# ctu-vras/monoforce

Measured on AMD Instinct MI355X. Metric: rollout-steps/sec (batch x horizon) on 256x256 terrain, higher is better.
Workload: dtype f32; 1 GPU; c3: B=1024/GPU x T=500 x N=4 contact points, 256x256 grid (res 0.05 m), one shared terrain+friction map (the same on every rank), integrator=odeint-euler (reference default), forward+backward; BASE...; rollouts_per_gpu=1024, rollouts_total=1024, horizon=500, contact_points=4, parallelism=rollout-sharded x1

## Files before the change

include/monoforce_hip.h:

```cpp
#ifndef MONOFORCE_HIP_H
#define MONOFORCE_HIP_H

#include <stddef.h>
#include <stdint.h>

#ifdef __cplusplus
extern "C" {
#endif

enum {
  MF_OK = 0,
  MF_ERR_INVALID = 1,
  MF_ERR_UNSUPPORTED = 2,
  MF_ERR_LAUNCH = 3
};

enum {
  MF_INTEG_DYNAMICS = 0,
  MF_INTEG_ODEINT_EULER = 1
};

enum {
  MF_LAYOUT_BATCH_MAJOR = 0,
  MF_LAYOUT_TIME_MAJOR = 1
};

enum {
  MF_MATH_EXACT = 0,
  MF_MATH_FAST = 1
};

enum { MF_LANES_COMPONENT = 16 };

typedef struct MfRolloutDesc {
  int32_t B;
  int32_t T;
  int32_t N;
  int32_t H, W;
  int32_t n_tracks;
  int32_t integrator;
  int32_t layout;
  int32_t map_shared;
  int32_t block;
  int32_t skip_snap;
  int32_t points_per_lane;
  int32_t math_mode;
  int32_t force_stride;
  int32_t grad_copies;
  int32_t has_joints;
  int32_t pose_stride;
  int32_t cost_project;
  int32_t default_state;
  int32_t controls_stride_b, controls_stride_t;
  double mass, gravity, stiffness, damping, omega_max;
  double grid_res, d_max;
  double dt;
  double robot_size_y;
  double Iinv[9];
  double joint_xyz[12];
} MfRolloutDesc;

#define MF_LOSS_VALUE_IN_BACKWARD 1
typedef struct MfRolloutLoss {
  int32_t T2;
  int32_t flags;
  const void* gt;
  const int32_t* near;
  const void* w;
  const int32_t* row_stamp;
  const void* row_w;
  void* partial;
  uint32_t* ticket;
  void* loss;
  const void* gloss;
  const void* Xs;
} MfRolloutLoss;

typedef struct MfRolloutFwdBufs {
  const void* z;
  const void* mu;
  const void* controls;
  const void* ts;
  const void* points;
  const int32_t* part;
  void* x0;
  const void* xd0;
  const void* R0;
  const void* w0;
  void* Xs;
  void* Xds;
  void* Rs;
  void* Omegas;
  void* Fs;
  void* Ff;
  void* Xraw;
  const void* joint_angles;
  void* cost_rows;
  void* path_cost;
  void* zmu_scratch;
  const void* zmu;
  void* rec;
  const MfRolloutLoss* loss;
} MfRolloutFwdBufs;

int mf_rollout_loss_fusable(const MfRolloutDesc* desc);

int mf_rollout_bwd_window(const MfRolloutDesc* desc);

long long mf_rollout_record_bytes(const MfRolloutDesc* desc);
int mf_rollout_fwd_stages_zmu(const MfRolloutDesc* desc);
long long mf_rollout_record_bytes_f64(const MfRolloutDesc* desc);

int mf_rollout_force_stride(const MfRolloutDesc* desc);
int mf_rollout_fwd_f32(const MfRolloutDesc* desc, const MfRolloutFwdBufs* bufs, void* hip_stream);
int mf_rollout_fwd_f64(const MfRolloutDesc* desc, const MfRolloutFwdBufs* bufs, void* hip_stream);

int mf_rollout_default_state_f32(int32_t B, int32_t T, const float* controls, float* x0, float* xd0, float* R0, float* w0, void* hip_stream);
int mf_rollout_default_state_f64(int32_t B, int32_t T, const double* controls, double* x0, double* xd0, double* R0, double* w0, void* hip_stream);

typedef struct MfRolloutBwdBufs {
  const void* z;
  const void* mu;
  const void* controls;
  const void* ts;
  const void* points;
  const int32_t* part;
  const void* x_init;
  const void* xd0;
  const void* R0;
  const void* w0;
  const void* Xraw;
  const void* Xds;
  const void* Rs;
  const void* Omegas;
  const void* gXs;
  const void* gXds;
  const void* gRs;
  const void* gOmegas;
  const void* gFs;
  const void* gFf;
  const void* zeros;
  void* gz;
  void* gmu;
  void* gcontrols;
  void* gx0;
  void* gxd0;
  void* gR0;
  void* gw0;
  const void* joint_angles;
  void* gjoint_angles;
  const void* rec;
  const MfRolloutLoss* loss;
  void* zmu_scratch;
  const void* zmu;
} MfRolloutBwdBufs;

int mf_rollout_bwd_wants_gcontrols(const MfRolloutDesc* desc);
int mf_rollout_bwd_f32(const MfRolloutDesc* desc, const MfRolloutBwdBufs* bufs, void* hip_stream);
int mf_rollout_bwd_f64(const MfRolloutDesc* desc, const MfRolloutBwdBufs* bufs, void* hip_stream);

typedef struct MfSplatDesc {
  int32_t B;
  int32_t n_per_sample;
  int32_t C;
  int32_t nx, ny, nz;
  float off[3];
  float dx[3];
  int32_t lift_D;
  int32_t lift_hw;
} MfSplatDesc;

size_t mf_bev_splat_workspace_bytes(const MfSplatDesc* desc);
int mf_bev_splat_prepare(const MfSplatDesc* desc, const float* geom , void* workspace, void* hip_stream);
int mf_bev_splat_prepare_cameras(const MfSplatDesc* desc, const float* frustum, int32_t pts_per_cam, const float* cams,
                                 void* workspace, void* hip_stream);
int mf_bev_splat_prepare_rig(const MfSplatDesc* desc, const float* frustum, int32_t pts_per_cam, const float* rots, const float* trans,
                             const float* intrins, const float* post_rots, const float* post_trans, void* workspace, void* hip_stream);
int mf_bev_splat_fwd_f32(const MfSplatDesc* desc, const float* x, const void* workspace, float* out, void* hip_stream);
int mf_bev_splat_fwd_f64(const MfSplatDesc* desc, const double* x, const void* workspace, double* out, void* hip_stream);
int mf_bev_splat_bwd_f32(const MfSplatDesc* desc, const float* gout, const void* workspace, float* gx, void* hip_stream);
int mf_bev_splat_bwd_f64(const MfSplatDesc* desc, const double* gout, const void* workspace, double* gx, void* hip_stream);

int mf_bev_lift_splat_fwd_f32(const MfSplatDesc* desc, const float* depth, const float* ctx, const void* workspace, float* out, void* hip_stream);
int mf_bev_lift_splat_fwd_f64(const MfSplatDesc* desc, const double* depth, const double* ctx, const void* workspace, double* out, void* hip_stream);
int mf_bev_lift_splat_bwd_f32(const MfSplatDesc* desc, const float* depth, const float* ctx, const void* workspace, const float* gout,
                              float* rows_scratch, float* g_depth, float* g_ctx, void* hip_stream);
int mf_bev_lift_splat_bwd_f64(const MfSplatDesc* desc, const double* depth, const double* ctx, const void* workspace, const double* gout,
                              double* rows_scratch, double* g_depth, double* g_ctx, void* hip_stream);

typedef struct MfLossDesc {
  int32_t B, T1, T2;
  int32_t reserved;
  int64_t x_stride_b, x_stride_t;
  double gamma;
} MfLossDesc;
int mf_physics_loss_fwd_f32(const MfLossDesc* desc, const float* Xs, const float* Xgt, const float* gt_ts, const int32_t* nearest, float* partial, void* hip_stream);
int mf_physics_loss_fwd_f64(const MfLossDesc* desc, const double* Xs, const double* Xgt, const double* gt_ts, const int32_t* nearest, double* partial, void* hip_stream);
int mf_physics_loss_bwd_f32(const MfLossDesc* desc, const float* Xs, const float* Xgt, const float* gt_ts, const int32_t* nearest, const float* gloss, float* gXs, void* hip_stream);
int mf_physics_loss_bwd_f64(const MfLossDesc* desc, const double* Xs, const double* Xgt, const double* gt_ts, const int32_t* nearest, const double* gloss, double* gXs, void* hip_stream);
int mf_nearest_steps_f32(int32_t B, int32_t T1, int32_t T2, const float* pred_ts, long long pred_stride_b, const float* gt_ts, long long gt_stride_b, int32_t* nearest, void* hip_stream);
int mf_nearest_steps_f64(int32_t B, int32_t T1, int32_t T2, const double* pred_ts, long long pred_stride_b, const double* gt_ts, long long gt_stride_b, int32_t* nearest, void* hip_stream);
int mf_physics_loss_value_f32(const MfLossDesc* desc, const float* Xs, const float* Xgt, const float* gt_ts, const int32_t* nearest, float* partial, uint32_t* ticket, float* loss, float* zero_fill, long long zero_count, void* hip_stream);
int mf_physics_loss_value_f64(const MfLossDesc* desc, const double* Xs, const double* Xgt, const double* gt_ts, const int32_t* nearest, double* partial, uint32_t* ticket, double* loss, double* zero_fill, long long zero_count, void* hip_stream);
int mf_reduce_grad_copies_f32(float* pool, int n_maps, int copies, long long n, float* out, void* hip_stream);
int mf_reduce_grad_copies_f64(double* pool, int n_maps, int copies, long long n, double* out, void* hip_stream);

typedef struct MfStageDesc {
  int32_t B, H, W, k;
} MfStageDesc;
int mf_terrain_stage_fwd_f32(const MfStageDesc* desc, const float* geom, const float* diff, const float* friction, float* terrain,
                             float* z, float* mu, float* zmu, void* hip_stream);
int mf_terrain_stage_bwd_f32(const MfStageDesc* desc, const float* g_terrain, const float* gz, const float* gmu, float* g_geom,
                             float* g_diff, float* g_friction, void* hip_stream);

typedef struct MfHeightmapDesc {
  int32_t n_points, nx, ny;
  float d_max, h_min, h_max;
  float r_min;
  float inv_res;
} MfHeightmapDesc;
int mf_estimate_heightmap_f32(const MfHeightmapDesc* desc, const float* points, const float* x_bins, const float* y_bins,
                              int32_t* scratch, float* hm, void* hip_stream);

typedef struct MfInterpDesc {
  int32_t B, N, H, W;
  int32_t map_shared;
  int32_t math_mode;
  double grid_res, d_max;
} MfInterpDesc;
int mf_interpolate_grid_f32(const MfInterpDesc* desc, const float* grid, const float* xq, const float* yq, float* z_out, float* n_out,
                            int32_t* cells_out, float* frac_out, void* hip_stream);
int mf_interpolate_grid_f64(const MfInterpDesc* desc, const double* grid, const double* xq, const double* yq, double* z_out, double* n_out,
                            int32_t* cells_out, double* frac_out, void* hip_stream);

typedef struct MfMppiDesc {
  int32_t B, T;
  int32_t keep_nominal, reserved;
  int64_t row_stride_b, row_stride_t;
  int64_t x_stride_b;
  float sigma[2], lo[2], hi[2];
  float w_incl, w_force, w_goal, lambda;
} MfMppiDesc;
int mf_mppi_perturb_f32(const MfMppiDesc* desc, const float* nominal , const float* noise ,
                        float* controls , void* hip_stream);
int mf_path_costs_f32(const MfMppiDesc* desc, const float* cost_rows, const float* force_cost, const float* x_last, const float* goal,
                      float* costs, float* terms, void* hip_stream);
long long mf_mppi_scratch_bytes(const MfMppiDesc* desc);
int mf_mppi_update_f32(const MfMppiDesc* desc, const float* costs, const float* controls, const float* nominal_in, float* weights,
                       float* nominal_out, int32_t* best, int32_t* n_valid, void* scratch, long long scratch_bytes, void* hip_stream);

const char* mf_last_error(void);
const char* mf_last_launch(void);
const char* mf_version(void);
int mf_sizeof(const char* struct_name);

#ifdef __cplusplus
}
#endif
#endif
```

monoforce_amd/_lib.py:

```python
import ctypes as C
import os
import threading

_HERE = os.path.dirname(os.path.abspath(__file__))
LIB_PATH = os.path.join(_HERE, 'csrc', 'libmonoforce_hip.so')

MF_INTEG_DYNAMICS, MF_INTEG_ODEINT_EULER = 0, 1
MF_LAYOUT_BATCH_MAJOR, MF_LAYOUT_TIME_MAJOR = 0, 1
MF_LOSS_VALUE_IN_BACKWARD = 1
MF_MATH_EXACT, MF_MATH_FAST = 0, 1
MF_LANES_COMPONENT = 16


class MfRolloutDesc(C.Structure):
    _fields_ = [('B', C.c_int32), ('T', C.c_int32), ('N', C.c_int32), ('H', C.c_int32), ('W', C.c_int32),
                ('n_tracks', C.c_int32), ('integrator', C.c_int32), ('layout', C.c_int32), ('map_shared', C.c_int32),
                ('block', C.c_int32), ('skip_snap', C.c_int32), ('points_per_lane', C.c_int32), ('math_mode', C.c_int32), ('force_stride', C.c_int32), ('grad_copies', C.c_int32), ('has_joints', C.c_int32), ('pose_stride', C.c_int32), ('cost_project', C.c_int32), ('default_state', C.c_int32), ('controls_stride_b', C.c_int32), ('controls_stride_t', C.c_int32),
                ('mass', C.c_double), ('gravity', C.c_double), ('stiffness', C.c_double), ('damping', C.c_double),
                ('omega_max', C.c_double), ('grid_res', C.c_double), ('d_max', C.c_double), ('dt', C.c_double),
                ('robot_size_y', C.c_double), ('Iinv', C.c_double * 9), ('joint_xyz', C.c_double * 12)]


class MfRolloutLoss(C.Structure):
    _fields_ = [('T2', C.c_int32), ('flags', C.c_int32)] + [(n, C.c_void_p) for n in ('gt', 'near', 'w', 'row_stamp', 'row_w', 'partial', 'ticket', 'loss', 'gloss', 'Xs')]


class MfRolloutFwdBufs(C.Structure):
    _fields_ = [(n, C.c_void_p) for n in ('z', 'mu', 'controls', 'ts', 'points', 'part', 'x0', 'xd0', 'R0', 'w0',
                                          'Xs', 'Xds', 'Rs', 'Omegas', 'Fs', 'Ff', 'Xraw', 'joint_angles', 'cost_rows', 'path_cost',
                                          'zmu_scratch', 'zmu', 'rec', 'loss')]


class MfRolloutBwdBufs(C.Structure):
    _fields_ = [(n, C.c_void_p) for n in ('z', 'mu', 'controls', 'ts', 'points', 'part', 'x_init', 'xd0', 'R0', 'w0',
                                          'Xraw', 'Xds', 'Rs', 'Omegas',
                                          'gXs', 'gXds', 'gRs', 'gOmegas', 'gFs', 'gFf', 'zeros',
                                          'gz', 'gmu', 'gcontrols', 'gx0', 'gxd0', 'gR0', 'gw0', 'joint_angles', 'gjoint_angles', 'rec', 'loss',
                                          'zmu_scratch', 'zmu')]


class MfLossDesc(C.Structure):
    _fields_ = [('B', C.c_int32), ('T1', C.c_int32), ('T2', C.c_int32), ('reserved', C.c_int32),
                ('x_stride_b', C.c_int64), ('x_stride_t', C.c_int64), ('gamma', C.c_double)]


class MfSplatDesc(C.Structure):
    _fields_ = [('B', C.c_int32), ('n_per_sample', C.c_int32), ('C', C.c_int32),
                ('nx', C.c_int32), ('ny', C.c_int32), ('nz', C.c_int32),
                ('off', C.c_float * 3), ('dx', C.c_float * 3), ('lift_D', C.c_int32), ('lift_hw', C.c_int32)]


class MfStageDesc(C.Structure):
    _fields_ = [('B', C.c_int32), ('H', C.c_int32), ('W', C.c_int32), ('k', C.c_int32)]


class MfInterpDesc(C.Structure):
    _fields_ = [('B', C.c_int32), ('N', C.c_int32), ('H', C.c_int32), ('W', C.c_int32), ('map_shared', C.c_int32), ('math_mode', C.c_int32),
                ('grid_res', C.c_double), ('d_max', C.c_double)]


class MfHeightmapDesc(C.Structure):
    _fields_ = [('n_points', C.c_int32), ('nx', C.c_int32), ('ny', C.c_int32), ('d_max', C.c_float), ('h_min', C.c_float),
                ('h_max', C.c_float), ('r_min', C.c_float), ('inv_res', C.c_float)]


class MfMppiDesc(C.Structure):
    _fields_ = [('B', C.c_int32), ('T', C.c_int32), ('keep_nominal', C.c_int32), ('reserved', C.c_int32),
                ('row_stride_b', C.c_int64), ('row_stride_t', C.c_int64), ('x_stride_b', C.c_int64),
                ('sigma', C.c_float * 2), ('lo', C.c_float * 2), ('hi', C.c_float * 2),
                ('w_incl', C.c_float), ('w_force', C.c_float), ('w_goal', C.c_float), ('lam', C.c_float)]


SYMBOLS = ['mf_rollout_force_stride', 'mf_rollout_fwd_f32', 'mf_rollout_fwd_f64', 'mf_rollout_default_state_f32', 'mf_rollout_default_state_f64', 'mf_rollout_bwd_f32', 'mf_rollout_bwd_f64', 'mf_rollout_bwd_wants_gcontrols', 'mf_rollout_record_bytes', 'mf_rollout_record_bytes_f64', 'mf_rollout_fwd_stages_zmu', 'mf_rollout_loss_fusable', 'mf_rollout_bwd_window', 'mf_bev_splat_workspace_bytes', 'mf_bev_splat_prepare', 'mf_bev_splat_prepare_cameras', 'mf_bev_splat_prepare_rig',
           'mf_bev_splat_fwd_f32', 'mf_bev_splat_fwd_f64', 'mf_bev_splat_bwd_f32', 'mf_bev_splat_bwd_f64',
           'mf_bev_lift_splat_fwd_f32', 'mf_bev_lift_splat_fwd_f64', 'mf_bev_lift_splat_bwd_f32', 'mf_bev_lift_splat_bwd_f64',
           'mf_physics_loss_fwd_f32', 'mf_physics_loss_fwd_f64', 'mf_physics_loss_bwd_f32', 'mf_physics_loss_bwd_f64', 'mf_physics_loss_value_f32', 'mf_physics_loss_value_f64', 'mf_nearest_steps_f32', 'mf_nearest_steps_f64', 'mf_reduce_grad_copies_f32', 'mf_reduce_grad_copies_f64', 'mf_estimate_heightmap_f32', 'mf_interpolate_grid_f32', 'mf_interpolate_grid_f64', 'mf_terrain_stage_fwd_f32', 'mf_terrain_stage_bwd_f32', 'mf_mppi_perturb_f32', 'mf_path_costs_f32', 'mf_mppi_scratch_bytes', 'mf_mppi_update_f32', 'mf_last_error', 'mf_last_launch', 'mf_version', 'mf_sizeof']

_lib = None
_lock = threading.Lock()


def lib():
    global _lib
    if _lib is None:
        with _lock:
            if _lib is None:
                if not os.path.exists(LIB_PATH):
                    raise RuntimeError(
                        f'{LIB_PATH} is missing: build the HIP extension first (make -C monoforce_amd/csrc). '
                        'monoforce_amd has no CPU fallback.')
                import torch
                L = C.CDLL(os.environ.get('MONOFORCE_HIP_LIB', LIB_PATH))
                L.mf_last_error.restype = C.c_char_p
                L.mf_version.restype = C.c_char_p
                L.mf_last_launch.restype = C.c_char_p
                for name in SYMBOLS:
                    fn = getattr(L, name)
                    if name.startswith(('mf_rollout', 'mf_bev', 'mf_physics', 'mf_estimate', 'mf_terrain', 'mf_reduce', 'mf_interpolate', 'mf_nearest', 'mf_mppi', 'mf_path')):
                        fn.restype = C.c_int
                L.mf_bev_splat_workspace_bytes.restype = C.c_size_t
                L.mf_rollout_record_bytes.restype = C.c_longlong
                L.mf_rollout_record_bytes_f64.restype = C.c_longlong
                L.mf_mppi_scratch_bytes.restype = C.c_longlong
                _lib = L
    return _lib


ON_ERROR = []


def check(rc, what):
    if rc != 0:
        for fn in list(ON_ERROR):
            fn()
        raise RuntimeError(f'{what} failed (code {rc}): {lib().mf_last_error().decode()}')


def ptr(t):
    return None if t is None else C.c_void_p(t.data_ptr())


def require_hip_tensor(t, name):
    if not t.is_cuda:
        raise RuntimeError(f'{name} is on {t.device}: monoforce_amd computes on the MI355X HIP path only '
                           '(no CPU fallback); move inputs to "cuda".')
```

monoforce_amd/csrc/physics_loss.hip:

```cpp
#include "mf_common.h"

namespace mf {

__device__ __forceinline__ void atomic_add_s(float* p, float v) { unsafeAtomicAdd(p, v); }
__device__ __forceinline__ void atomic_add_s(double* p, double v) { unsafeAtomicAdd(p, v); }

template <typename S>
__global__ void __launch_bounds__(256) physics_loss_fwd_kernel(const S* __restrict__ Xs, long long sb, long long st,
                                                              const S* __restrict__ Xgt, const S* __restrict__ gt_ts,
                                                              const int* __restrict__ nearest, int B, int T2, S gamma,
                                                              S* __restrict__ partial) {
  __shared__ S wave_sum[4];
  const int i = blockIdx.x * blockDim.x + threadIdx.x;
  S acc = (S)0;
  if (i < B * T2) {
    const int b = i / T2;
    const S w = (S)1 / ((S)1 + gamma * gt_ts[i]);
    const S* x = Xs + b * sb + (long long)nearest[i] * st;
    const S* g = Xgt + (size_t)i * 3;
#pragma unroll
    for (int c = 0; c < 3; ++c) { const S d = x[c] * w - g[c] * w; acc += d * d; }
  }
#pragma unroll
  for (int d = 32; d >= 1; d >>= 1) acc += __shfl_xor(acc, d, 64);
  if ((threadIdx.x & 63) == 0) wave_sum[threadIdx.x >> 6] = acc;
  __syncthreads();
  if (threadIdx.x == 0) partial[blockIdx.x] = (wave_sum[0] + wave_sum[1]) + (wave_sum[2] + wave_sum[3]);
}

template <typename S>
__global__ void __launch_bounds__(256) physics_loss_value_kernel(const S* __restrict__ Xs, long long sb, long long st,
                                                                const S* __restrict__ Xgt, const S* __restrict__ gt_ts,
                                                                const int* __restrict__ nearest, int B, int T2, S gamma,
                                                                S* __restrict__ partial, unsigned* __restrict__ ticket, S inv_count,
                                                                S* __restrict__ loss, S* __restrict__ zero_fill, long long zero_count) {
  __shared__ S wave_sum[4];
  __shared__ bool last;
  const int i = blockIdx.x * blockDim.x + threadIdx.x;
  {
    const long long head = min(zero_count, (long long)(((16u - (unsigned)((uintptr_t)zero_fill & 15u)) & 15u) / sizeof(S)));
    const long long n16 = (zero_count - head) * (long long)sizeof(S) / 16, tail0 = head + n16 * (16 / (long long)sizeof(S));
    int4* z16 = reinterpret_cast<int4*>(zero_fill + head);
    for (long long k = i; k < n16; k += (long long)gridDim.x * blockDim.x) z16[k] = make_int4(0, 0, 0, 0);
    if (i < head) zero_fill[i] = (S)0;
    if (tail0 + i < zero_count) zero_fill[tail0 + i] = (S)0;
  }
  S acc = (S)0;
  if (i < B * T2) {
    const int k = i, b = i / T2;
    const S w = (S)1 / ((S)1 + gamma * gt_ts[k]);
    const S* x = Xs + b * sb + (long long)nearest[k] * st;
    const S* g = Xgt + (size_t)k * 3;
#pragma unroll
    for (int c = 0; c < 3; ++c) { const S d = x[c] * w - g[c] * w; acc += d * d; }
  }
#pragma unroll
  for (int d = 32; d >= 1; d >>= 1) acc += __shfl_xor(acc, d, 64);
  if ((threadIdx.x & 63) == 0) wave_sum[threadIdx.x >> 6] = acc;
  __syncthreads();
  if (threadIdx.x == 0) {
    partial[blockIdx.x] = (wave_sum[0] + wave_sum[1]) + (wave_sum[2] + wave_sum[3]);
    __threadfence();
    last = atomicAdd(ticket, 1u) == gridDim.x - 1;
  }
  __syncthreads();
  if (!last) return;
  __threadfence();
  S tot = (S)0;
  for (unsigned k = threadIdx.x; k < gridDim.x; k += 256) tot += __builtin_nontemporal_load(partial + k);
#pragma unroll
  for (int d = 32; d >= 1; d >>= 1) tot += __shfl_xor(tot, d, 64);
  if ((threadIdx.x & 63) == 0) wave_sum[threadIdx.x >> 6] = tot;
  __syncthreads();
  if (threadIdx.x == 0) {
    loss[0] = ((wave_sum[0] + wave_sum[1]) + (wave_sum[2] + wave_sum[3])) * inv_count;
    *ticket = 0u;
  }
}

template <typename S>
__global__ void __launch_bounds__(256) reduce_grad_copies_kernel(S* __restrict__ pool, int copies, long long n, S* __restrict__ out) {
  const long long i = (long long)blockIdx.x * blockDim.x + threadIdx.x;
  if (i >= n) return;
  S* p = pool + (long long)blockIdx.y * copies * n + i;
  S acc = (S)0;
  for (int c = 0; c < copies; ++c) { acc += p[(long long)c * n]; p[(long long)c * n] = (S)0; }
  out[(long long)blockIdx.y * n + i] = acc;
}

template <typename S>
__global__ void __launch_bounds__(256) physics_loss_bwd_kernel(const S* __restrict__ Xs, long long sb, long long st,
                                                              const S* __restrict__ Xgt, const S* __restrict__ gt_ts,
                                                              const int* __restrict__ nearest, int B, int T2, S gamma,
                                                              const S* __restrict__ gloss, S inv_count, S* __restrict__ gXs) {
  const int t = blockIdx.x * blockDim.x + threadIdx.x;
  if (t >= B * T2) return;
  const bool jm = sb < st;
  const int b = jm ? t % B : t / T2, j = jm ? t / B : t % T2;
  const int i = b * T2 + j;
  const S scale = (S)2 * gloss[0] * inv_count;
  const S w = (S)1 / ((S)1 + gamma * gt_ts[i]);
  const int nr = nearest[i];
  const long long o = b * sb + (long long)nr * st;
  const S* g = Xgt + (size_t)i * 3;
  bool shared = false;
  for (int k = 0; k < T2; ++k) shared |= (k != j) & (nearest[b * T2 + k] == nr);
#pragma unroll
  for (int c = 0; c < 3; ++c) {
    const S v = scale * w * (Xs[o + c] * w - g[c] * w);
    if (shared) atomic_add_s(gXs + o + c, v); else gXs[o + c] = v;
  }
}

template <typename S>
static int loss_fwd(const MfLossDesc* d, const S* Xs, const S* Xgt, const S* gt_ts, const int* nearest, S* partial, hipStream_t st) {
  MF_REQUIRE(d && Xs && Xgt && gt_ts && nearest && partial, MF_ERR_INVALID, "physics_loss_fwd: null argument");
  MF_REQUIRE(d->B > 0 && d->T1 > 0 && d->T2 > 0, MF_ERR_INVALID, "physics_loss_fwd: B, T1, T2 must be positive");
  hipLaunchKernelGGL((physics_loss_fwd_kernel<S>), dim3((d->B * d->T2 + 255) / 256), dim3(256), 0, st, Xs, (long long)d->x_stride_b,
                     (long long)d->x_stride_t, Xgt, gt_ts, nearest, d->B, d->T2, (S)d->gamma, partial);
  hipError_t e = hipGetLastError();
  MF_REQUIRE(e == hipSuccess, MF_ERR_LAUNCH, std::string("physics_loss_fwd launch: ") + hipGetErrorString(e));
  return MF_OK;
}

template <typename S>
static int loss_value(const MfLossDesc* d, const S* Xs, const S* Xgt, const S* gt_ts, const int* nearest, S* partial, unsigned* ticket,
                      S* loss, S* zero_fill, long long zero_count, hipStream_t st) {
  MF_REQUIRE(d && Xs && Xgt && gt_ts && nearest && partial && ticket && loss, MF_ERR_INVALID, "physics_loss_value: null argument");
  MF_REQUIRE(d->B > 0 && d->T1 > 0 && d->T2 > 0, MF_ERR_INVALID, "physics_loss_value: B, T1, T2 must be positive");
  MF_REQUIRE(zero_count >= 0 && (zero_fill || zero_count == 0), MF_ERR_INVALID, "physics_loss_value: zero_count without zero_fill");
  const double count = (double)d->B * d->T2 * 3;
  hipLaunchKernelGGL((physics_loss_value_kernel<S>), dim3((d->B * d->T2 + 255) / 256), dim3(256), 0, st, Xs, (long long)d->x_stride_b,
                     (long long)d->x_stride_t, Xgt, gt_ts, nearest, d->B, d->T2, (S)d->gamma, partial, ticket, (S)(1.0 / count), loss, zero_fill, zero_count);
  hipError_t e = hipGetLastError();
  MF_REQUIRE(e == hipSuccess, MF_ERR_LAUNCH, std::string("physics_loss_value launch: ") + hipGetErrorString(e));
  return MF_OK;
}

template <typename S>
static int reduce_copies(S* pool, int n_maps, int copies, long long n, S* out, hipStream_t st) {
  MF_REQUIRE(pool && out, MF_ERR_INVALID, "reduce_grad_copies: null argument");
  MF_REQUIRE(n_maps > 0 && n_maps < 65536 && copies > 0 && n > 0, MF_ERR_INVALID, "reduce_grad_copies: n_maps, copies, n must be positive");
  hipLaunchKernelGGL((reduce_grad_copies_kernel<S>), dim3((unsigned)((n + 255) / 256), (unsigned)n_maps), dim3(256), 0, st, pool, copies, n, out);
  hipError_t e = hipGetLastError();
  MF_REQUIRE(e == hipSuccess, MF_ERR_LAUNCH, std::string("reduce_grad_copies launch: ") + hipGetErrorString(e));
  return MF_OK;
}

template <typename S>
static int loss_bwd(const MfLossDesc* d, const S* Xs, const S* Xgt, const S* gt_ts, const int* nearest, const S* gloss, S* gXs,
                    hipStream_t st) {
  MF_REQUIRE(d && Xs && Xgt && gt_ts && nearest && gloss && gXs, MF_ERR_INVALID, "physics_loss_bwd: null argument");
  MF_REQUIRE(d->B > 0 && d->T1 > 0 && d->T2 > 0, MF_ERR_INVALID, "physics_loss_bwd: B, T1, T2 must be positive");
  const double count = (double)d->B * d->T2 * 3;
  hipLaunchKernelGGL((physics_loss_bwd_kernel<S>), dim3((d->B * d->T2 + 255) / 256), dim3(256), 0, st, Xs, (long long)d->x_stride_b,
                     (long long)d->x_stride_t, Xgt, gt_ts, nearest, d->B, d->T2, (S)d->gamma, gloss, (S)(1.0 / count), gXs);
  hipError_t e = hipGetLastError();
  MF_REQUIRE(e == hipSuccess, MF_ERR_LAUNCH, std::string("physics_loss_bwd launch: ") + hipGetErrorString(e));
  return MF_OK;
}

}

namespace mf {
template <typename S>
__global__ void __launch_bounds__(256) nearest_steps_kernel(const S* __restrict__ pred_ts, long long pred_sb, const S* __restrict__ gt_ts, long long gt_sb,
                                                           int B, int T1, int T2, int* __restrict__ out) {
  const int i = blockIdx.x * blockDim.x + threadIdx.x;
  if (i >= B * T2) return;
  const int b = i / T2, j = i - b * T2;
  const S g = gt_ts[b * gt_sb + j];
  const S* p = pred_ts + b * pred_sb;
  S best = (S)INFINITY;
  int arg = 0;
  bool any = false;
  int t = 0;
  for (; t + 8 <= T1; t += 8) {
    S v[8];
#pragma unroll
    for (int k = 0; k < 8; ++k) v[k] = p[t + k];
#pragma unroll
    for (int k = 0; k < 8; ++k) {
      const S d = fabs(v[k] - g);
      if (d < best || (!any && d == d)) { best = d; arg = t + k; any = true; }
    }
  }
  for (; t < T1; ++t) {
    const S d = fabs(p[t] - g);
    if (d < best || (!any && d == d)) { best = d; arg = t; any = true; }
  }
  out[i] = arg;
}
template <typename S>
static int nearest_steps(int B, int T1, int T2, const S* pred_ts, long long pred_sb, const S* gt_ts, long long gt_sb, int32_t* out, hipStream_t st) {
  MF_REQUIRE(B > 0 && T1 > 0 && T2 > 0 && pred_ts && gt_ts && out && pred_sb >= 0 && gt_sb >= 0, MF_ERR_INVALID, "nearest_steps: bad argument");
  const long long n = (long long)B * T2;
  MF_REQUIRE(n < (1ll << 31), MF_ERR_UNSUPPORTED, "nearest_steps: B * T2 must be below 2^31");
  hipLaunchKernelGGL((nearest_steps_kernel<S>), dim3((unsigned)((n + 255) / 256)), dim3(256), 0, st, pred_ts, pred_sb, gt_ts, gt_sb, B, T1, T2, out);
  hipError_t e = hipGetLastError();
  MF_REQUIRE(e == hipSuccess, MF_ERR_LAUNCH, std::string("nearest_steps launch: ") + hipGetErrorString(e));
  return MF_OK;
}
}
extern "C" int mf_nearest_steps_f32(int32_t B, int32_t T1, int32_t T2, const float* pred_ts, long long pred_stride_b, const float* gt_ts, long long gt_stride_b,
                                    int32_t* nearest, void* s) { return mf::nearest_steps<float>(B, T1, T2, pred_ts, pred_stride_b, gt_ts, gt_stride_b, nearest, (hipStream_t)s); }
extern "C" int mf_nearest_steps_f64(int32_t B, int32_t T1, int32_t T2, const double* pred_ts, long long pred_stride_b, const double* gt_ts, long long gt_stride_b,
                                    int32_t* nearest, void* s) { return mf::nearest_steps<double>(B, T1, T2, pred_ts, pred_stride_b, gt_ts, gt_stride_b, nearest, (hipStream_t)s); }
extern "C" int mf_physics_loss_fwd_f32(const MfLossDesc* d, const float* Xs, const float* Xgt, const float* gt_ts, const int32_t* nearest,
                                       float* partial, void* s) { return mf::loss_fwd<float>(d, Xs, Xgt, gt_ts, nearest, partial, (hipStream_t)s); }
extern "C" int mf_physics_loss_fwd_f64(const MfLossDesc* d, const double* Xs, const double* Xgt, const double* gt_ts, const int32_t* nearest,
                                       double* partial, void* s) { return mf::loss_fwd<double>(d, Xs, Xgt, gt_ts, nearest, partial, (hipStream_t)s); }
extern "C" int mf_physics_loss_bwd_f32(const MfLossDesc* d, const float* Xs, const float* Xgt, const float* gt_ts, const int32_t* nearest,
                                       const float* gloss, float* gXs, void* s) { return mf::loss_bwd<float>(d, Xs, Xgt, gt_ts, nearest, gloss, gXs, (hipStream_t)s); }
extern "C" int mf_physics_loss_bwd_f64(const MfLossDesc* d, const double* Xs, const double* Xgt, const double* gt_ts, const int32_t* nearest,
                                       const double* gloss, double* gXs, void* s) { return mf::loss_bwd<double>(d, Xs, Xgt, gt_ts, nearest, gloss, gXs, (hipStream_t)s); }
extern "C" int mf_physics_loss_value_f32(const MfLossDesc* d, const float* Xs, const float* Xgt, const float* gt_ts, const int32_t* nearest,
                                         float* partial, uint32_t* ticket, float* loss, float* zero_fill, long long zero_count, void* s) { return mf::loss_value<float>(d, Xs, Xgt, gt_ts, nearest, partial, ticket, loss, zero_fill, zero_count, (hipStream_t)s); }
extern "C" int mf_physics_loss_value_f64(const MfLossDesc* d, const double* Xs, const double* Xgt, const double* gt_ts, const int32_t* nearest,
                                         double* partial, uint32_t* ticket, double* loss, double* zero_fill, long long zero_count, void* s) { return mf::loss_value<double>(d, Xs, Xgt, gt_ts, nearest, partial, ticket, loss, zero_fill, zero_count, (hipStream_t)s); }
extern "C" int mf_reduce_grad_copies_f32(float* pool, int n_maps, int copies, long long n, float* out, void* s) { return mf::reduce_copies<float>(pool, n_maps, copies, n, out, (hipStream_t)s); }
extern "C" int mf_reduce_grad_copies_f64(double* pool, int n_maps, int copies, long long n, double* out, void* s) { return mf::reduce_copies<double>(pool, n_maps, copies, n, out, (hipStream_t)s); }
```

monoforce_amd/csrc/rollout_bwd.hip:

```cpp
#include "rollout_bwd_cp_kernel.h"
#include "rollout_bwd_mw_kernel.h"

namespace mf {
template <typename S>
__global__ void __launch_bounds__(256) interleave_maps_bwd_kernel(const S* __restrict__ z, const S* __restrict__ mu, int n, cp::Pk2<S>* __restrict__ out) {
  const int i = blockIdx.x * blockDim.x + threadIdx.x;
  if (i < n) out[i] = cp::Pk2<S>{z[i], mu[i]};
}

long long mw_record_bytes(const MfRolloutDesc* d, int scalar_bytes);

static bool xs_bwd_off() { static const bool off = getenv("MF_BWD_XS") && atoi(getenv("MF_BWD_XS")) == 0; return off; }
static long long xs_bwd_min_waves() {
  static const long long v = getenv("MF_BWD_XS_MIN_WAVES") ? atoll(getenv("MF_BWD_XS_MIN_WAVES")) : device_simds() / 2;
  return v;
}
static bool xs_bwd_shape(const MfRolloutDesc* d, const LaneMap& m) {
  return !xs_bwd_off() && m.PPL == 1 && m.G <= 64 && (long long)d->B * m.G >= xs_bwd_min_waves() * 64;
}
bool cp_loss_one_wave(const MfRolloutDesc* d, int scalar_bytes) {
  static const bool off = getenv("MF_CP_LOSS_ONE_WAVE") && atoi(getenv("MF_CP_LOSS_ONE_WAVE")) == 0;
  if (off || !d || d->layout != MF_LAYOUT_TIME_MAJOR || d->has_joints || cp_loss_fusable(d)) return false;
  if (scalar_bytes != 4 && d->points_per_lane != MF_LANES_COMPONENT) return false;
  if (cp_record_bytes(d, scalar_bytes) > 0 || ((long long)d->B * 16 + 63) / 64 <= (long long)device_simds()) return false;
  MfRolloutBwdBufs none{};
  return use_component_parallel_bwd(d, &none, scalar_bytes);
}
bool xs_loss_fusable(const MfRolloutDesc* d) {
  static const bool off = getenv("MF_BWD_XS_LOSS") && atoi(getenv("MF_BWD_XS_LOSS")) == 0;
  if (off || !d || d->B <= 0 || d->T <= 0 || d->N <= 0 || d->N > 64 || d->has_joints) return false;
  if (d->math_mode != MF_MATH_FAST || d->layout != MF_LAYOUT_TIME_MAJOR) return false;
  if (d->integrator != MF_INTEG_ODEINT_EULER && d->integrator != MF_INTEG_DYNAMICS) return false;
  if (d->points_per_lane == MF_LANES_COMPONENT || d->points_per_lane == 4) return false;
  MfRolloutBwdBufs none{};
  if (use_component_parallel_bwd(d, &none, 4)) return false;
  if (mw_record_bytes(d, 4) > 0) return false;
  return xs_bwd_shape(d, choose_lane_map(d->B, d->N, d->points_per_lane));
}

static bool xs_win_off() { static const bool off = getenv("MF_BWD_WIN") && atoi(getenv("MF_BWD_WIN")) == 0; return off; }
static bool xs_win_shape(const MfRolloutDesc* d, const LaneMap& m) {
  return !xs_win_off() && d->map_shared && m.G == 4 && d->H == d->W && (d->H & (d->H - 1)) == 0;
}
bool xs_bwd_window(const MfRolloutDesc* d) {
  if (!d || d->B <= 0 || d->N <= 0 || d->N > 4 || d->has_joints || d->math_mode != MF_MATH_FAST) return false;
  if (d->points_per_lane == MF_LANES_COMPONENT || d->points_per_lane == 4) return false;
  MfRolloutBwdBufs none{};
  if (use_component_parallel_bwd(d, &none, 4)) return false;
  const LaneMap m = choose_lane_map(d->B, d->N, d->points_per_lane);
  return xs_bwd_shape(d, m) && xs_win_shape(d, m);
}

template <typename S>
static int rollout_bwd(const MfRolloutDesc* d, const MfRolloutBwdBufs* p, void* stream) {
  MF_REQUIRE(d && p, MF_ERR_INVALID, "rollout_bwd: null descriptor");
  MF_REQUIRE(d->B > 0 && d->N > 0 && d->H > 1 && d->W > 0 && d->T >= 1, MF_ERR_INVALID, "rollout_bwd: B, T, N, H, W must be positive");
  MF_REQUIRE(d->n_tracks == 2 || d->n_tracks == 4, MF_ERR_INVALID, "n_tracks must be 2 or 4");
  MF_REQUIRE(d->integrator == MF_INTEG_DYNAMICS || d->integrator == MF_INTEG_ODEINT_EULER, MF_ERR_INVALID,
             "rollout_bwd: unknown integrator");
  MF_REQUIRE(p->z && p->controls && p->ts && p->points && p->part && p->x_init && p->xd0 && p->R0 && p->w0, MF_ERR_INVALID,
             "rollout_bwd: null input buffer");
  MF_REQUIRE(p->Xraw && p->Xds && p->Rs && p->Omegas, MF_ERR_INVALID, "rollout_bwd: null saved-state buffer");
  MF_REQUIRE(p->gz && p->gxd0 && p->gR0 && p->gw0, MF_ERR_INVALID, "rollout_bwd: null gradient output buffer");
  MF_REQUIRE(d->N <= 512, MF_ERR_UNSUPPORTED, "rollout_bwd: more than 512 contact points");
  MF_REQUIRE(d->H < (1 << 23), MF_ERR_UNSUPPORTED, "rollout_bwd: grid too large (H must be below 2^23)");
  MF_REQUIRE(d->H >= 2, MF_ERR_INVALID, "rollout_bwd: the grid needs at least 2 x 2 cells");
  MF_REQUIRE(d->controls_stride_b == 0 && d->controls_stride_t == 0, MF_ERR_UNSUPPORTED, "rollout_bwd: controls must be contiguous [B][T][2]");
  MF_REQUIRE(d->map_shared || (long long)d->B * d->H * d->W * (long long)sizeof(S) < (1ll << 32), MF_ERR_UNSUPPORTED,
             "rollout_bwd: per-rollout maps of 4 GiB or more in total (use a shared map or split the batch)");
  MF_REQUIRE((long long)(d->grad_copies > 1 ? d->grad_copies : 1) * d->H * d->W * (long long)sizeof(S) < (1ll << 32), MF_ERR_UNSUPPORTED,
             "rollout_bwd: gradient copies of 4 GiB or more in total");
  int block = d->block ? d->block : 64;
  MF_REQUIRE(block == 64 || block == 128 || block == 256, MF_ERR_INVALID, "rollout_bwd: block must be 64, 128 or 256");

  RolloutBwdArgs<S> a;
  a.B = d->B; a.T = d->T; a.N = d->N; a.H = d->H; a.W = d->W;
  a.n_tracks = d->n_tracks; a.layout = d->layout; a.map_shared = d->map_shared; a.skip_snap = d->skip_snap;
  a.grad_copies = d->grad_copies > 1 ? d->grad_copies : 1;
  a.mass = (S)d->mass; a.inv_mass = (S)(1.0 / d->mass); a.inv_res = (S)(1.0 / (double)(S)d->grid_res); a.mg = (S)(d->mass * d->gravity); a.k = (S)d->stiffness; a.damp = (S)d->damping;
  a.omega_max = (S)d->omega_max; a.res = (S)d->grid_res; a.d_max = (S)d->d_max; a.dt = (S)d->dt;
  a.half_ly = (S)(d->robot_size_y / 2.0);
  a.sink = (S)(d->mass * d->gravity / (d->stiffness + 1e-6));
  for (int i = 0; i < 9; ++i) a.Iinv[i] = (S)d->Iinv[i];
  for (int i = 0; i < 12; ++i) a.joint_xyz[i] = (S)d->joint_xyz[i];
  a.joint_angles = (const S*)p->joint_angles;
  a.gjoint = (S*)p->gjoint_angles;
  a.rec = nullptr;
  a.zmu = nullptr;
  a.loss_T2 = 0; a.loss_gt = nullptr; a.loss_row_stamp = nullptr; a.loss_row_w = nullptr; a.loss_gloss = nullptr; a.loss_inv_count = (S)0;
  a.loss_partial = nullptr; a.loss_ticket = nullptr; a.loss_out = nullptr; a.loss_near = nullptr; a.loss_w = nullptr;
  MF_REQUIRE(!p->gjoint_angles || p->joint_angles, MF_ERR_INVALID, "rollout_bwd: gjoint_angles without joint_angles");
  MF_REQUIRE(!d->has_joints == !p->joint_angles, MF_ERR_INVALID, "rollout_bwd: joint_angles must be given exactly when desc->has_joints is set");
  MF_REQUIRE(!p->joint_angles || d->n_tracks == 4, MF_ERR_INVALID, "rollout_bwd: joint angles need the 4 driving parts of robot 'marv'");
  a.z = (const S*)p->z; a.mu = (const S*)p->mu; a.controls = (const S*)p->controls; a.ts = (const S*)p->ts;
  a.points = (const S*)p->points; a.part = p->part;
  a.x_init = (const S*)p->x_init; a.xd0 = (const S*)p->xd0; a.R0 = (const S*)p->R0; a.w0 = (const S*)p->w0;
  a.Xraw = (const S*)p->Xraw; a.Xds = (const S*)p->Xds; a.Rs = (const S*)p->Rs; a.Om = (const S*)p->Omegas;
  if (p->loss) {
    const MfRolloutLoss* L = p->loss;
    const bool loss_cp = (sizeof(S) == 4 || d->points_per_lane == MF_LANES_COMPONENT) && cp_loss_fusable(d) && p->rec && !p->joint_angles;
    const bool loss_xs = !loss_cp && sizeof(S) == 4 && xs_loss_fusable(d) && !p->joint_angles;
    const bool loss_cp1 = !loss_cp && !loss_xs && cp_loss_one_wave(d, (int)sizeof(S)) && !p->joint_angles && !(L->flags & MF_LOSS_VALUE_IN_BACKWARD);
    MF_REQUIRE(!(loss_cp1 || loss_xs) || (L->near && L->w), MF_ERR_INVALID, "rollout_bwd: this fused loss reads MfRolloutLoss.near and .w");
    MF_REQUIRE(loss_cp || loss_xs || loss_cp1, MF_ERR_UNSUPPORTED,
               "rollout_bwd: this launch cannot carry the fused physics loss (mf_rollout_loss_fusable: 1 = the streaming component-parallel backward, "
               "the forward's record required; 2 = the saturated positions-only kernels)");
    MF_REQUIRE((long long)d->B * L->T2 * 3 * (long long)sizeof(S) < (1ll << 32), MF_ERR_UNSUPPORTED, "rollout_bwd: ground truth of 4 GiB or more");
    MF_REQUIRE(!p->gXs && !p->gXds && !p->gRs && !p->gOmegas && !p->gFs && !p->gFf, MF_ERR_INVALID,
               "rollout_bwd: with a fused loss the six upstream gradients must be NULL");
    MF_REQUIRE(L->T2 > 0 && L->gt && L->row_stamp && L->row_w && L->gloss && L->Xs, MF_ERR_INVALID, "rollout_bwd: incomplete MfRolloutLoss");
    a.loss_T2 = L->T2; a.loss_gt = (const S*)L->gt; a.loss_row_stamp = L->row_stamp; a.loss_row_w = (const S*)L->row_w; a.loss_gloss = (const S*)L->gloss;
    a.loss_inv_count = (S)(1.0 / ((double)d->B * L->T2 * 3));
    a.loss_near = L->near; a.loss_w = (const S*)L->w;
    if (L->flags & MF_LOSS_VALUE_IN_BACKWARD) {
      MF_REQUIRE(L->partial && L->ticket && L->loss, MF_ERR_INVALID, "rollout_bwd: MF_LOSS_VALUE_IN_BACKWARD needs MfRolloutLoss.partial / ticket / loss");
      a.loss_partial = (S*)L->partial; a.loss_ticket = L->ticket; a.loss_out = (S*)L->loss;
    }
  }
  const bool any_null = !p->gXs || !p->gXds || !p->gRs || !p->gOmegas || !p->gFs || !p->gFf;
  MF_REQUIRE(!any_null || p->zeros, MF_ERR_INVALID,
             "rollout_bwd: an upstream gradient is NULL but `zeros` (>= max(9, 3) zero scalars) was not provided");
  const S* zr = (const S*)p->zeros;
  a.gXs = p->gXs ? (const S*)p->gXs : zr;       a.sXs = p->gXs ? 3 : 0;
  if (p->loss) { a.gXs = (const S*)p->loss->Xs; a.sXs = 3; }
  a.gXds = p->gXds ? (const S*)p->gXds : zr;    a.sXds = p->gXds ? 3 : 0;
  a.gOm = p->gOmegas ? (const S*)p->gOmegas : zr; a.sOm = p->gOmegas ? 3 : 0;
  a.gRs = p->gRs ? (const S*)p->gRs : zr;       a.sRs = p->gRs ? 9 : 0;
  a.gFs = p->gFs ? (const S*)p->gFs : zr;       a.sFs = p->gFs ? 3 : 0;
  a.gFf = p->gFf ? (const S*)p->gFf : zr;       a.sFf = p->gFf ? 3 : 0;
  a.gz = (S*)p->gz; a.gmu = (S*)p->gmu; a.gcontrols = (S*)p->gcontrols;
  a.gc_sb = 2 * d->T; a.gc_st = 2;
  if (!p->gcontrols) { a.gcontrols = (S*)p->gw0; a.gc_sb = 3; a.gc_st = 0; }
  a.gx0 = (S*)p->gx0; a.gxd0 = (S*)p->gxd0; a.gR0 = (S*)p->gR0; a.gw0 = (S*)p->gw0;

  hipStream_t st = (hipStream_t)stream;
  if (p->joint_angles) {
    const LaneMap mj = choose_lane_map(d->B, d->N, 0);
    if (sizeof(S) == 4 && d->math_mode == MF_MATH_FAST)
      return launch_rollout_bwd_joints_fast_f32(*reinterpret_cast<const RolloutBwdArgs<float>*>(&a), mj, d->integrator, block, st);
    if (sizeof(S) == 4) return launch_rollout_bwd_joints_f32(*reinterpret_cast<const RolloutBwdArgs<float>*>(&a), mj, d->integrator, block, st);
    return launch_rollout_bwd_joints_f64(*reinterpret_cast<const RolloutBwdArgs<double>*>(&a), mj, d->integrator, block, st);
  }
  const bool cp = (sizeof(S) == 4 || d->points_per_lane == MF_LANES_COMPONENT) && use_component_parallel_bwd(d, p, (int)sizeof(S));
  if (cp) {
    a.gcontrols = (S*)p->gcontrols;
    if (p->rec && cp_record_bytes(d, (int)sizeof(S)) > 0) {
      MF_REQUIRE(((uintptr_t)p->rec & 15) == 0, MF_ERR_INVALID, "rollout_bwd: rec must be 16-byte aligned");
      a.rec = (const S*)p->rec;
    }
    const bool xs_only = (p->gXs || p->loss) && !p->gXds && !p->gRs && !p->gOmegas && !p->gFs && !p->gFf;
    if constexpr (sizeof(S) == 4) {
      if ((p->zmu || p->zmu_scratch) && cp_bwd_wants_zmu(d, a.rec != nullptr, p->mu != nullptr)) {
        MF_REQUIRE((((uintptr_t)p->zmu_scratch | (uintptr_t)p->zmu) & 7) == 0, MF_ERR_INVALID, "rollout_bwd: zmu_scratch / zmu must be 8-byte aligned");
        if (p->zmu) a.zmu = (const S*)p->zmu;
        else {
          const int n = d->H * d->W;
          hipLaunchKernelGGL((interleave_maps_bwd_kernel<S>), dim3((n + 255) / 256), dim3(256), 0, st, a.z, a.mu, n, (cp::Pk2<S>*)p->zmu_scratch);
          a.zmu = (const S*)p->zmu_scratch;
        }
      }
      return launch_rollout_bwd_cp_f32(a, d->integrator, xs_only, st);
    }
    else return launch_rollout_bwd_cp_f64(a, d->integrator, xs_only, st);
  }
  const LaneMap m = choose_lane_map(d->B, d->N, d->points_per_lane == MF_LANES_COMPONENT ? 0 : d->points_per_lane);
  if ((sizeof(S) == 4 || d->points_per_lane == MF_LANES_COMPONENT) && use_multiwave_bwd(d, p)) {
    MF_REQUIRE(((uintptr_t)p->rec & (4 * sizeof(S) - 1)) == 0, MF_ERR_INVALID, "rollout_bwd: rec must be aligned to its quads");
    a.rec = (const S*)p->rec;
    a.gcontrols = (S*)p->gcontrols;
    const bool xs_only = !p->gXds && !p->gRs && !p->gOmegas && !p->gFs && !p->gFf;
    if constexpr (sizeof(S) == 4) return launch_rollout_bwd_mw_f32(a, m.G, d->integrator, xs_only, st);
    else return launch_rollout_bwd_mw_f64(a, m.G, d->integrator, xs_only, st);
  }
  if (sizeof(S) == 4 && d->math_mode == MF_MATH_FAST) {
    const RolloutBwdArgs<float>& af = *reinterpret_cast<const RolloutBwdArgs<float>*>(&a);
    static const bool xs_zmu_off = getenv("MF_BWD_XS_ZMU") && atoi(getenv("MF_BWD_XS_ZMU")) == 0;
    const bool xs_only = (p->gXs || p->loss) && !p->gXds && !p->gRs && !p->gOmegas && !p->gFs && !p->gFf;
    const bool fused = p->loss != nullptr;
    if (xs_only && xs_bwd_shape(d, m)) {
      RolloutBwdArgs<float> ax = af;
      bool zmu = false;
      if (!xs_zmu_off && d->map_shared && p->mu && (p->zmu || p->zmu_scratch) && (long long)d->H * d->W * 8 < (1ll << 31)) {
        MF_REQUIRE((((uintptr_t)p->zmu_scratch | (uintptr_t)p->zmu) & 7) == 0, MF_ERR_INVALID, "rollout_bwd: zmu_scratch / zmu must be 8-byte aligned");
        if (p->zmu) ax.zmu = (const float*)p->zmu;
        else {
          const int n = d->H * d->W;
          hipLaunchKernelGGL((interleave_maps_bwd_kernel<float>), dim3((n + 255) / 256), dim3(256), 0, st, ax.z, ax.mu, n, (cp::Pk2<float>*)p->zmu_scratch);
          ax.zmu = (const float*)p->zmu_scratch;
        }
        zmu = true;
      }
      if (xs_win_shape(d, m)) {
        const long long waves = ((long long)d->B * m.G + 63) / 64;
        const bool two = waves >= 2ll * device_simds();
        if (fused) return launch_rollout_bwd_xs_win_loss_fast_f32(ax, m, d->integrator, two ? 512 : 256, zmu, two, st);
        return launch_rollout_bwd_xs_win_fast_f32(ax, m, d->integrator, two ? 512 : 256, zmu, two, st);
      }
      if (fused) return launch_rollout_bwd_xs_loss_fast_f32(ax, m, d->integrator, block, zmu, st);
      return launch_rollout_bwd_xs_fast_f32(ax, m, d->integrator, block, zmu, st);
    }
    MF_REQUIRE(!fused, MF_ERR_UNSUPPORTED, "rollout_bwd: this launch cannot carry the fused physics loss (mf_rollout_loss_fusable)");
    static const bool xs_ppl_off = getenv("MF_BWD_XS_PPL") && atoi(getenv("MF_BWD_XS_PPL")) == 0;
    if (!xs_ppl_off && !xs_bwd_off() && xs_only && !fused && m.G == 64 && (m.PPL == 2 || m.PPL == 4 || m.PPL == 8) && (long long)d->B >= xs_bwd_min_waves())
      return launch_rollout_bwd_xs_ppl_fast_f32(af, m, d->integrator, block, st);
    if ((long long)d->B * m.G >= 3ll * device_cus() / 4 * 64) return launch_rollout_bwd_carry_fast_f32(af, m, d->integrator, block, st);
    return launch_rollout_bwd_fast_f32(af, m, d->integrator, block, st);
  }
  MF_REQUIRE(!p->loss, MF_ERR_UNSUPPORTED, "rollout_bwd: this launch cannot carry the fused physics loss (mf_rollout_loss_fusable)");
  return launch_rollout_bwd<S, false>(a, m, d->integrator, block, st);
}

}

extern "C" int mf_rollout_loss_fusable(const MfRolloutDesc* d) {
  return mf::cp_loss_fusable(d) ? 1 : (mf::xs_loss_fusable(d) ? 2 : (mf::cp_loss_one_wave(d, 4) ? 3 : 0));
}
extern "C" int mf_rollout_bwd_window(const MfRolloutDesc* d) { return mf::xs_bwd_window(d) ? 1 : 0; }
extern "C" int mf_rollout_bwd_f32(const MfRolloutDesc* d, const MfRolloutBwdBufs* p, void* s) {
  return mf::rollout_bwd<float>(d, p, s);
}
extern "C" int mf_rollout_bwd_f64(const MfRolloutDesc* d, const MfRolloutBwdBufs* p, void* s) {
  return mf::rollout_bwd<double>(d, p, s);
}
```

monoforce_amd/csrc/rollout_bwd_cp_fast.hip:

```cpp
#include "rollout_bwd_cp_kernel.h"
#include "rollout_fwd_cp_kernel.h"

namespace mf {

static long long cp_bwd_max_waves() {
  static const long long v = getenv("MF_CP_BWD_MAX_WAVES") ? atoll(getenv("MF_CP_BWD_MAX_WAVES")) : -1;
  return v >= 0 ? v : 2 * device_simds();
}

static bool cp_bwd_covers(const MfRolloutDesc* d, bool joints, int scalar_bytes = 4) {
  if (d->math_mode != MF_MATH_FAST || d->N > 4 || joints) return false;
  if (d->points_per_lane != 0 && d->points_per_lane != MF_LANES_COMPONENT) return false;
  const long long waves = ((long long)d->B + 3) / 4;
  if (d->points_per_lane == 0 && waves > cp_bwd_max_waves()) return false;
  const long long row = (long long)d->N * 3 > 9 ? (long long)d->N * 3 : 9;
  if ((long long)d->T * d->B * row * scalar_bytes >= (1ll << 32)) return false;
  return true;
}
bool use_component_parallel_bwd(const MfRolloutDesc* d, const MfRolloutBwdBufs* p, int scalar_bytes) { return cp_bwd_covers(d, p->joint_angles != nullptr, scalar_bytes); }

long long cp_record_bytes(const MfRolloutDesc* d, int scalar_bytes) {
  static const long long max_waves_env = getenv("MF_CP_RECORD_MAX_WAVES") ? atoll(getenv("MF_CP_RECORD_MAX_WAVES")) : -1;
  const long long max_waves = max_waves_env >= 0 ? max_waves_env : device_simds();
  if (!d || d->B <= 0 || d->T <= 0) return 0;
  MfRolloutFwdBufs f{};
  static const bool dyn = getenv("MF_CP_RECORD_DYNAMICS") && atoi(getenv("MF_CP_RECORD_DYNAMICS")) != 0;
  static const bool one_wave = getenv("MF_CP_BWD_MODE") && atoi(getenv("MF_CP_BWD_MODE")) == kCpSaved;
  if (d->has_joints) return 0;
  if (!use_component_parallel(d, &f, scalar_bytes) || !cp_bwd_covers(d, false, scalar_bytes)) return 0;
  const long long waves = ((long long)d->B + 3) / 4;
  if (waves > max_waves) return 0;
  if (d->integrator != MF_INTEG_ODEINT_EULER && !dyn && (one_wave || waves > (long long)cp_stream_max_grid(d->integrator))) return 0;
  const long long bytes = (long long)d->T * d->B * 16 * 4 * scalar_bytes;
  if (bytes >= (1ll << 32)) return 0;
  return bytes;
}

bool cp_loss_fusable(const MfRolloutDesc* d) {
  static const bool one_wave = getenv("MF_CP_BWD_MODE") && atoi(getenv("MF_CP_BWD_MODE")) == kCpSaved;
  if (!d || d->layout != MF_LAYOUT_TIME_MAJOR || one_wave) return false;
  if (d->integrator != MF_INTEG_ODEINT_EULER && d->integrator != MF_INTEG_DYNAMICS) return false;
  if (cp_record_bytes(d, 4) <= 0) return false;
  const long long grid = ((long long)d->B * 16 + 63) / 64;
  return grid <= (long long)cp_stream_max_grid(d->integrator);
}
bool cp_bwd_wants_zmu(const MfRolloutDesc* d, bool has_rec, bool has_mu) {
  static const bool off = getenv("MF_CP_BWD_ZMU") && atoi(getenv("MF_CP_BWD_ZMU")) == 0;
  static const int forced = getenv("MF_CP_BWD_MODE") ? atoi(getenv("MF_CP_BWD_MODE")) : -1;
  if (off || !d || !d->map_shared || !has_rec || !has_mu || d->integrator != MF_INTEG_ODEINT_EULER || d->math_mode != MF_MATH_FAST) return false;
  if ((long long)d->H * d->W * 8 >= (1ll << 31)) return false;
  const long long grid = ((long long)d->B * 16 + 63) / 64;
  return forced == kCpSaved || grid > (long long)cp_stream_max_grid(d->integrator);
}
bool cp_loss_in_forward(const MfRolloutDesc* d) { return cp_loss_fusable(d) && d->integrator == MF_INTEG_ODEINT_EULER; }

}
extern "C" int mf_rollout_bwd_wants_gcontrols(const MfRolloutDesc* d) { (void)d; return 0; }
namespace mf { long long mw_record_bytes(const MfRolloutDesc* d, int scalar_bytes); }
extern "C" long long mf_rollout_record_bytes(const MfRolloutDesc* d) {
  const long long cp = mf::cp_record_bytes(d, 4);
  return cp > 0 ? cp : mf::mw_record_bytes(d, 4);
}
extern "C" long long mf_rollout_record_bytes_f64(const MfRolloutDesc* d) {
  if (!d || d->points_per_lane != MF_LANES_COMPONENT) return 0;
  const long long cp = mf::cp_record_bytes(d, 8);
  return cp > 0 ? cp : mf::mw_record_bytes(d, 8);
}
namespace mf {

int launch_rollout_bwd_cp_f32(const RolloutBwdArgs<float>& a, int integ, bool xs_only, hipStream_t st) {
  if (integ == MF_INTEG_DYNAMICS) return launch_rollout_bwd_cp_dynamics_f32(a, xs_only, st);
  return launch_rollout_bwd_cp_variant<float, MF_INTEG_ODEINT_EULER>(a, xs_only, st);
}

}
```

monoforce_amd/csrc/rollout_bwd_cp_kernel.h:

```cpp
#pragma once
#include "rollout_bwd_kernel.h"
#include "rollout_cp_common.h"
#include <type_traits>

namespace mf {

enum { kCpEarly = 0, kCpLate = 1, kCpSaved = 2, kCpStream = 3 };
#ifdef MF_STREAM_PROFILE
extern __device__ unsigned long long mf_stream_prof[32];
#define MF_PROF_T(v) const unsigned long long v = __builtin_readcyclecounter()
#define MF_PROF_RT(v) const unsigned long long v = __builtin_amdgcn_s_memrealtime()
#define MF_PROF_ACC(name) unsigned long long name = 0
#define MF_PROF_SUM(name, t0) name += __builtin_readcyclecounter() - (t0)
#define MF_PROF_OUT(slot, val) do { if (lane == 0) atomicAdd(&mf_stream_prof[slot], (unsigned long long)(val)); } while (0)
#define MF_PROF_ADD(slot, t0) MF_PROF_OUT(slot, __builtin_readcyclecounter() - (t0))
#define MF_PROF_MAX(slot, val) do { if (lane == 0) atomicMax(&mf_stream_prof[slot], (unsigned long long)(val)); } while (0)
#define MF_PROF_DRAIN() asm volatile("s_waitcnt vmcnt(0) lgkmcnt(0)" ::: "memory")
#else
#define MF_PROF_T(v)
#define MF_PROF_RT(v)
#define MF_PROF_ACC(name)
#define MF_PROF_SUM(name, t0)
#define MF_PROF_OUT(slot, val)
#define MF_PROF_ADD(slot, t0)
// ... 112 lines not shown
  const S* const o_gt = ONE1 ? a.loss_gt + ((size_t)b * (size_t)a.loss_T2) * 3u + (unsigned)cc : nullptr;
  int o_zero = 0;
  int o_j = 0, o_near_cur = 0, o_near_prev = 0;
  S o_w_cur = zero, o_w_prev = zero;
  if constexpr (ONE1) {
    asm volatile("v_mov_b32 %0, 0" : "=v"(o_zero));
    o_j = a.loss_T2 - 1 + o_zero;
    o_near_cur = o_near[o_j]; o_near_prev = o_near[max(o_j - 1, 0)];
    o_w_cur = o_w[o_j]; o_w_prev = o_w[max(o_j - 1, 0)];
  }
  auto load_upstream = [&](int orow, UpIn& u) {
    const unsigned uo = __builtin_amdgcn_readfirstlane((unsigned)orow);
    if constexpr (ONE1) {
      const bool dec = (o_near_cur > (int)uo) & (o_j >= 0);
      o_j -= dec ? 1 : 0;
      o_near_cur = dec ? o_near_prev : o_near_cur;
      o_w_cur = dec ? o_w_prev : o_w_cur;
      const int jp = max(o_j - 1, 0);
      o_near_prev = o_near[jp]; o_w_prev = o_w[jp];
      u.lw = ((o_near_cur == (int)uo) & (o_j >= 0)) ? o_w_cur : -one;
      u.lg = o_gt[(size_t)(unsigned)max(o_j, 0) * 3u];
    }
    u.gXs = bload1<S>(rgXs, u_xs, uo * sg_xs);
    if constexpr (!XS_ONLY) {
      u.gXds = bload1<S>(rgXds, u_xds, uo * sg_xds); u.gOm = bload1<S>(rgOm, u_om, uo * sg_om);
      bload3(rgRs, u_r, uo * sg_r, &u.gR0, &u.gR1, &u.gR2);
      u.gFs = bload1<S>(rgFs, u_fs, uo * sg_fs); u.gFf = bload1<S>(rgFf, u_ff, uo * sg_ff);
    }
  };
  const S first = p == 0 ? one : zero;
  auto add_upstream_masked = [&](const UpIn& u) {
    lx += u.gXs;
    lR2 = mf_fma(u.gXs, a.sink, lR2);
    if constexpr (!XS_ONLY) {
      lxd += u.gXds;
      lR0 += u.gR0; lR1 += u.gR1; lR2 += u.gR2;
      lw += u.gOm;
    }
  };
  auto add_upstream_state = [&](const UpIn& u) {
    UpIn m = u;
    S gXs_row = u.gXs;
    if constexpr (ONE1) {
      const Msk smask = u.lw > zero ? ~(Msk)0 : (Msk)0;
      gXs_row = bfi(smask, cp_loss_grad(one1_scale, u.gXs, u.lg, u.lw), zero);
    }
    m.gXs = first * gXs_row;
    if constexpr (!XS_ONLY) { m.gXds = first * u.gXds; m.gR0 = first * u.gR0; m.gR1 = first * u.gR1; m.gR2 = first * u.gR2; m.gOm = first * u.gOm; }
    add_upstream_masked(m);
  };

  if constexpr (GCTRL && ODE) bstore2(rGctrl, v_ctrl, (unsigned)(a.T - 1) * kC, zero, zero);

  unsigned acc_idx = 0u, st_idx = 0u;
  S acc_z = zero, acc_m = zero, st_z = zero, st_m = zero;
  bool st_pending = false;
  auto emit = [&](unsigned idx, S vz, S vm) {
    if constexpr (WIN) {
      if (win_emit(win, win_flat0, win_shift, (unsigned)(a.H - 1), idx, vz, vm, want_gmu)) return;
    }
#ifdef MF_STREAM_NO_ATOMIC
    asm volatile("" :: "v"(vz), "v"(vm), "v"(idx));
    return;
#endif
    atomic_add(at32(gzmap, goff + idx), vz);
    if (want_gmu) atomic_add(at32(gmumap, goff + idx), vm);
  };
  auto flush_stash = [&]() {
    if (st_pending) emit(st_idx, st_z, st_m);
    st_pending = false;
  };

  unsigned gctrl_pending = (unsigned)(a.T - 1) * kC;
  S gv_pending = zero, gwc_pending = zero;

  struct Rec {
    S x, xd, cv, cw, r, pc, fr, mc;
    S R0, R1, R2, w, r1, r2, w1, w2, vp, e, il, coln2, tv, h;
    S wq, wa, wb, zc, mcv, mub, nrm, inl, cj, inv_csum, A, F0, F1, Fr, Nn, cmdv, s, sn, stv, Gf, f1, f2, wraw;
    int idx;
  };
  auto recompute_gather = [&](const StateIn& st, Rec& k) {
    k.x = st.x; k.xd = st.xd; k.w = st.w; k.cv = st.cv; k.cw = st.cw;
    k.R0 = st.R0; k.R1 = st.R1; k.R2 = st.R2;
    k.h = ODE ? st.t1 - st.t0 : a.dt;
    k.r = cp_body_r(P0, P1, P2, st.R0, st.R1, st.R2);
    k.pc = k.r + st.x;
    const S lim = S(262144.0);
    const S uq = M::cell_coord(k.pc, a.d_max, a.res, a.inv_res);
    const int ui = (int)M::clamp(uq, -lim, lim);
    k.fr = uq - (S)ui;
    const int base = dppi<kB1>(ui) + __mul24(a.H, dppi<kB0>(ui));
    k.idx = min(max(base + cell_off, 0), last);
    k.zc = ld32(zmap, moff + (unsigned)k.idx);
    k.mc = ld32(mumap, moff + (unsigned)k.idx);
  };
  auto recompute = [&](Rec& k) {
    const S xd = k.xd, w = k.w, r = k.r, pc = k.pc, fr = k.fr;
    k.wa = mf_fma(wa_s, dpp<kB0>(fr), wa_o); k.wb = mf_fma(wb_s, dpp<kB1>(fr), wb_o);
    k.wq = k.wa * k.wb;
    k.r1 = dpp<kRot1>(r); k.r2 = dpp<kRot2>(r);
    k.w1 = dpp<kRot1>(w); k.w2 = dpp<kRot2>(w);
    k.vp = cp_vel(xd, w, r);
    k.coln2 = dot3(k.R0, k.R0);
    k.il = M::inv_len(k.coln2);
    k.e = k.R0 * k.il;
    k.tv = cp_track(tv_v, tv_w, k.cv, k.cw);
    const S zq = dot4(k.wq, k.zc);
    k.mcv = has_mu ? k.mc : one;
    k.mub = dot4(k.wq, k.mcv);
    const S dz = k.zc - dpp<kB0>(k.zc);
    const S u = mf_fma(dpp<kN12>(dz), n_mul, n_add);
    k.inl = M::inv_len(dot3(u, u));
    k.nrm = u * k.inl;
    const S dh = dpp<kB2>(pc) - zq;
    S cj = M::sigmoid_m10(dh);
    k.cj = act ? cj : zero;
    k.inv_csum = M::div(one, sum_points(k.cj));
    const S vn = dot3(k.vp, k.nrm);
    k.A = cp_normal_force(a.k, dh, a.damp, vn);
    k.F0 = -(k.A * k.nrm);
    k.F1 = cp_spring(k.A, k.nrm, k.cj, k.inv_csum);
    k.Fr = M::clamp(k.F1, -mg, mg);
    k.Nn = M::sqrt(dot3(k.Fr, k.Fr));
    k.cmdv = cp_cmd(k.tv, k.e, k.vp);
    k.s = k.mub * k.cmdv;
    k.sn = dot3(k.s, k.nrm);
    k.stv = cp_tangent(k.s, k.sn, k.nrm);
    k.Gf = k.Nn * k.stv;
    const S Ff = M::clamp(k.Gf, -mg, mg);
    const S f = k.Fr + Ff;
    k.f1 = dpp<kRot1>(f); k.f2 = dpp<kRot2>(f);
    const S Tsum = sum_points(unrot(cross_pre(r, f)));
    k.wraw = cp_wraw(I0, I1, I2, Tsum);
  };

  auto vjp = [&](int n, const Rec& k, const UpIn& up) {
    const S h = k.h, w1 = k.w1, w2 = k.w2, r1 = k.r1, r2 = k.r2, nrm = k.nrm, cj = k.cj, inv_csum = k.inv_csum;
    S gFr_up = zero, gFf_up = zero, gxdd, gwd;
    if constexpr (ODE) {
      if constexpr (!XS_ONLY) {
        laFs += act ? up.gFs : zero;
        laFf += act ? up.gFf : zero;
        gFr_up = h * laFs; gFf_up = h * laFf;
      }
      gxdd = h * sum_points(lxd); gwd = h * sum_points(lw);
      lxd = mf_fma(h, lx, lxd);
      const S g0 = h * lR0, g1 = h * lR1, g2 = h * lR2;
      const S g01 = dpp<kRot1>(g0), g02 = dpp<kRot2>(g0), g11 = dpp<kRot1>(g1), g12 = dpp<kRot2>(g1), g21 = dpp<kRot1>(g2), g22 = dpp<kRot2>(g2);
      lw += (dpp<kRot1>(k.R0) * g02 - dpp<kRot2>(k.R0) * g01) + (dpp<kRot1>(k.R1) * g12 - dpp<kRot2>(k.R1) * g11) + (dpp<kRot1>(k.R2) * g22 - dpp<kRot2>(k.R2) * g21);
      lR0 += g01 * w2 - g02 * w1;
      lR1 += g11 * w2 - g12 * w1;
      lR2 += g21 * w2 - g22 * w1;
    } else {
      if constexpr (!XS_ONLY) { gFr_up = act ? up.gFs : zero; gFf_up = act ? up.gFf : zero; }
      const S wd = M::clamp(k.wraw, -a.omega_max, a.omega_max);
      const S wn = mf_fma(wd, h, k.w);
      const S th2 = dot3(wn, wn);
      const S idn = M::inv_len(th2);
      const S kv = wn * idn;
      const S th = M::sqrt(th2);
      S sn_, oc;
      M::sincos_small(th * h, &sn_, &oc);
      const S kk = dot3(kv, kv);
      const S kv1 = dpp<kRot1>(kv), kv2 = dpp<kRot2>(kv);
      const S ok = oc * kv;
      const S m0 = mf_fma(ok, kv, mf_fma(-oc, kk, one)), m1 = mf_fma(ok, kv1, -(sn_ * kv2)), m2 = mf_fma(ok, kv2, sn_ * kv1);
      const S q0 = dpp<kB0>(kv), q1 = dpp<kB1>(kv), q2 = dpp<kB2>(kv);
      const S Lk = lR0 * q0 + lR1 * q1 + lR2 * q2, Rk = k.R0 * q0 + k.R1 * q1 + k.R2 * q2;
      const S Gk0 = dot3(k.R0, Lk), Gk1 = dot3(k.R1, Lk), Gk2 = dot3(k.R2, Lk);
      const S Gt0 = dot3(Rk, lR0), Gt1 = dot3(Rk, lR1), Gt2 = dot3(Rk, lR2);
      const S trG = sum3(k.R0 * lR0 + k.R1 * lR1 + k.R2 * lR2);
      const S a0 = sum3(k.R1 * lR2 - k.R2 * lR1), a1 = sum3(k.R2 * lR0 - k.R0 * lR2), a2 = sum3(k.R0 * lR1 - k.R1 * lR0);
      const S ga = -(q0 * a0 + q1 * a1 + q2 * a2);
      const S gb = (q0 * Gk0 + q1 * Gk1 + q2 * Gk2) - kk * trG;
      S gth = ga * h * (one - oc) + gb * h * sn_;
      const S ac = mask_or(mask_or(mask_or(zero, a0, lane0), a1, lane1), a2, lane2);
      const S sc = mask_or(mask_or(mask_or(zero, Gk0 + Gt0, lane0), Gk1 + Gt1, lane1), Gk2 + Gt2, lane2);
      const S gk = -(sn_ * ac) - oc * (S(2.0) * trG * kv - sc);
      const S gkw = dot3(gk, wn);
      const S idn2 = th2 >= S(1e-12) ? idn * idn : zero;
      gth = mf_fma(-gkw, idn2, gth);
      const S ith = th2 > zero ? M::div(one, th) : zero;
      lw += mf_fma(gth * ith, wn, gk * idn);
      gwd = h * sum_points(lw);
      lxd = mf_fma(h, lx, lxd);
      gxdd = h * sum_points(lxd);
      const S n0 = lR0 * dpp<kB0>(m0) + lR1 * dpp<kB0>(m1) + lR2 * dpp<kB0>(m2);
      const S n1 = lR0 * dpp<kB1>(m2) + lR1 * dpp<kB1>(m0) + lR2 * dpp<kB1>(m1);
      const S n2 = lR0 * dpp<kB2>(m1) + lR1 * dpp<kB2>(m2) + lR2 * dpp<kB2>(m0);
      lR0 = n0; lR1 = n1; lR2 = n2;
    }
    const S mwd = inside(k.wraw, -a.omega_max, a.omega_max) ? gwd : zero;
    const S gtau = J0 * dpp<kB0>(mwd) + J1 * dpp<kB1>(mwd) + J2 * dpp<kB2>(mwd);
    const S gsum = gxdd * a.inv_mass;
    const S gt1 = dpp<kRot1>(gtau), gt2 = dpp<kRot2>(gtau);
    const S gf = gt1 * r2 - gt2 * r1;
    S gr = k.f1 * gt2 - k.f2 * gt1;
    S gFr = gFr_up + gsum + gf;
    const S gFf_ = gFf_up + gsum + gf;
    const S gG = inside(k.Gf, -mg, mg) ? gFf_ : zero;
    const S gNn = dot3(gG, k.stv);
    const S gst = k.Nn * gG;
    const S gsn = -dot3(gst, nrm);
    S gn = gsn * k.s - k.sn * gst;
    const S gslip = gst + gsn * nrm;
    const S gmuq = dot3(gslip, k.cmdv);
    const S gcmd = k.mub * gslip;
    S gvp = -gcmd;
    const S ge_p = k.tv * gcmd;
    S gv_p = zero, gwc_p = zero;
    if constexpr (GCTRL) {
      const S gtv = dot3(gcmd, k.e);
      gv_p = tv_v * gtv; gwc_p = tv_w * gtv;
    }
    gFr = mf_fma(k.Nn > zero ? gNn * M::div(one, k.Nn) : zero, k.Fr, gFr);
    const S gF1 = inside(k.F1, -mg, mg) ? gFr : zero;
    const S dF = dot3(gF1, k.F0);
    const S gc_p = dF * inv_csum;
    const S gS = sum_points(-(dF * cj) * inv_csum * inv_csum);
    const S gF0 = gF1 * cj * inv_csum;
    const S gA = -dot3(gF0, nrm);
    gn = mf_fma(-k.A, gF0, gn);
    const S gdh_p = a.k * gA;
    const S gvn = a.damp * gA;
    gvp = mf_fma(gvn, nrm, gvp);
    gn = mf_fma(gvn, k.vp, gn);
    const S gcw = gc_p + gS;
    const S gdh = gdh_p + gcw * (-S(10.0)) * cj * (one - cj);
    const S gzq = -gdh;
    const S dotn = dot3(gn, nrm);
    const S gg = -((gn - dotn * nrm) * k.inl) * a.inv_res;
    const S ggp = dpp<0x51>(gg);
    const S nz = mf_fma(gzq, k.wq, cgA * gg + cgB * ggp);
    const S nm = gmuq * k.wq;
    {
      const unsigned ni = (unsigned)k.idx;
      const bool same = !act | (ni == acc_idx);
      st_pending = !same;
      st_idx = acc_idx; st_z = acc_z; st_m = acc_m;
      acc_idx = act ? ni : acc_idx;
      acc_z = same ? acc_z + nz : nz;
      acc_m = same ? acc_m + nm : nm;
    }
    const S vq = gzq * k.zc + gmuq * k.mcv;
    const S gpx = dot4(vq, wa_s * k.wb), gpy = dot4(vq, wb_s * k.wa);
    const S gp = mask_or(mask_or(mask_or(zero, gpx * a.inv_res, lane0), gpy * a.inv_res, lane1), gdh, lane2);
    const S gvp1 = dpp<kRot1>(gvp), gvp2 = dpp<kRot2>(gvp);
    gr += gvp1 * w2 - gvp2 * w1;
    const S gw_p = r1 * gvp2 - r2 * gvp1;
    const S qa = gp + gr;
    lx += gp; lxd += gvp; lw += gw_p;
    lR0 = mf_fma(qa, P0, lR0); lR1 = mf_fma(qa, P1, lR1); lR2 = mf_fma(qa, P2, lR2);
    const S ge = ge_p;
    S gv = zero, gwc = zero;
    if constexpr (GCTRL) { gv = sum_points(gv_p); gwc = sum_points(gwc_p); }
    {
      const S dote = dot3(ge, k.e) * (k.coln2 >= S(1e-12) ? one : zero);
      lR0 = mf_fma(ge - dote * k.e, k.il, lR0);
    }
    gctrl_pending = __builtin_amdgcn_readfirstlane((unsigned)n * kC); gv_pending = gv; gwc_pending = gwc;
  };

  auto body = [&](int n, const Rec& rec, Rec& rec_next, const StateIn& s_prev, StateIn& s_pp, const UpIn& up, UpIn& up_next) {
    add_upstream_state(up);
    load_state(max(n - 2, 0), s_pp);
    load_upstream(ODE ? n : max(n - 1, 0), up_next);
    recompute_gather(s_prev, rec_next);
    if constexpr (!LATE) recompute(rec_next);
    flush_stash();
    if constexpr (GCTRL) bstore2(rGctrl, v_ctrl, gctrl_pending, gv_pending, gwc_pending);
    vjp(n, rec, up);
    if constexpr (LATE) {
      asm("" : "+v"(rec_next.zc), "+v"(rec_next.mc) : "v"(lR0));
      recompute(rec_next);
    }
  };

  auto snap_cell = [&](int& idx, S& wq, S& dx, S& dy) {
    const S Ra = a.R0[b * 9 + cc * 3 + 0], Rb = a.R0[b * 9 + cc * 3 + 1], Rc = a.R0[b * 9 + cc * 3 + 2];
    const S x0c = a.x_init[b * 3 + cc];
    const S pc = (P0 * Ra + P1 * Rb + P2 * Rc) + x0c;
    const S lim = S(262144.0);
    const S uq = M::cell_coord(pc, a.d_max, a.res, a.inv_res);
    const int ui = (int)M::clamp(uq, -lim, lim);
    const S fr = uq - (S)ui;
    const int base = dppi<kB1>(ui) + __mul24(a.H, dppi<kB0>(ui));
    idx = min(max(base + cell_off, 0), last);
    const S wa = mf_fma(wa_s, dpp<kB0>(fr), wa_o), wb = mf_fma(wb_s, dpp<kB1>(fr), wb_o);
    const S zc = ld32(zmap, moff + (unsigned)idx);
    wq = wa * wb;
    dx = dot4(zc, wa_s * wb); dy = dot4(zc, wb_s * wa);
  };
  int snap_idx = 0;
  S snap_wq = zero, snap_dx = zero, snap_dy = zero;

  StateIn sA, sB;
  UpIn uA, uB;
  Rec recA, recB;
  int n = n_steps - 1;
  if constexpr (SAVED) {
    typedef S f4v __attribute__((ext_vector_type(4)));
    struct Saved { f4v q; S zc, mc; int idx; };
    const char* const prec = reinterpret_cast<const char*>(a.rec) + (size_t)tid * kRecBytesPerLane<S>;
    const unsigned rec_step = (unsigned)a.B * 16u * kRecBytesPerLane<S>;
    auto load_saved = [&](int m, Saved& v) {
      v.q = __builtin_nontemporal_load(reinterpret_cast<const f4v*>(prec + (size_t)__builtin_amdgcn_readfirstlane((unsigned)m) * (size_t)rec_step));
    };
    auto gather_cells = [&](Saved& v) {
      const S lim = S(262144.0);
      const int ui = (int)M::clamp(v.q.x, -lim, lim);
      const int base = dppi<kB1>(ui) + __mul24(a.H, dppi<kB0>(ui));
      v.idx = min(max(base + cell_off, 0), last);
#ifdef MF_STREAM_NO_GATHER
      v.zc = S(0.1) * (S)q; v.mc = S(0.8);
      return;
#endif
      if constexpr (ZMU) {
        const Pk2<S> zm = *reinterpret_cast<const Pk2<S>*>(reinterpret_cast<const char*>(a.zmu) + (size_t)((unsigned)v.idx * (unsigned)(2 * sizeof(S))));
        v.zc = zm.a; v.mc = zm.b;
        return;
      }
      v.zc = ld32(zmap, moff + (unsigned)v.idx);
      v.mc = ld32(mumap, moff + (unsigned)v.idx);
    };
    auto rebuild = [&](const StateIn& st, const Saved& v, Rec& k) {
      k.R0 = st.R0; k.R1 = st.R1; k.R2 = st.R2; k.w = st.w;
      k.h = ODE ? st.t1 - st.t0 : a.dt;
      const S r = cp_body_r(P0, P1, P2, st.R0, st.R1, st.R2);
      k.r1 = dpp<kRot1>(r); k.r2 = dpp<kRot2>(r);
      k.w1 = dpp<kRot1>(st.w); k.w2 = dpp<kRot2>(st.w);
      k.vp = cp_vel(st.xd, st.w, r);
      const S lim = S(262144.0);
      const S uq = v.q.x;
      const S fr = uq - (S)(int)M::clamp(uq, -lim, lim);
      k.wa = mf_fma(wa_s, dpp<kB0>(fr), wa_o); k.wb = mf_fma(wb_s, dpp<kB1>(fr), wb_o);
      k.wq = k.wa * k.wb;
      k.cj = v.q.y; k.wraw = v.q.z; k.A = v.q.w;
      k.idx = v.idx; k.zc = v.zc; k.mcv = has_mu ? v.mc : one;
      k.mub = dot4(k.wq, k.mcv);
      const S dz = v.zc - dpp<kB0>(v.zc);
      const S u = mf_fma(dpp<kN12>(dz), n_mul, n_add);
      k.inl = M::inv_len(dot3(u, u));
      k.nrm = u * k.inl;
      k.inv_csum = M::div(one, sum_points(k.cj));
      k.coln2 = dot3(st.R0, st.R0);
      k.il = M::inv_len(k.coln2);
      k.e = st.R0 * k.il;
      k.tv = cp_track(tv_v, tv_w, st.cv, st.cw);
      k.F0 = -(k.A * k.nrm);
      k.F1 = cp_spring(k.A, k.nrm, k.cj, k.inv_csum);
      k.Fr = M::clamp(k.F1, -mg, mg);
      k.Nn = M::sqrt(dot3(k.Fr, k.Fr));
      k.cmdv = cp_cmd(k.tv, k.e, k.vp);
      k.s = k.mub * k.cmdv;
      k.sn = dot3(k.s, k.nrm);
      k.stv = cp_tangent(k.s, k.sn, k.nrm);
      k.Gf = k.Nn * k.stv;
      const S f = k.Fr + M::clamp(k.Gf, -mg, mg);
      k.f1 = dpp<kRot1>(f); k.f2 = dpp<kRot2>(f);
    };
    const bool loss_on = STREAM && a.loss_gt != nullptr;
    const Msk loss_mask = loss_on ? ~(Msk)0 : (Msk)0;
    const S loss_scale = loss_on ? S(2.0) * a.loss_gloss[0] * a.loss_inv_count : zero;
    const S* const loss_gt_lane = loss_on ? a.loss_gt + ((size_t)b * (size_t)a.loss_T2) * 3u + (unsigned)cc : a.z;
    const int* const l_row_stamp = loss_on ? a.loss_row_stamp : reinterpret_cast<const int*>(a.ts);
    const S* const l_row_w = loss_on ? a.loss_row_w : a.ts;
    const int l_T2m1 = loss_on ? a.loss_T2 - 1 : 0;
    if constexpr (STREAM) {
      const unsigned un = (unsigned)max(n, 0);
      unsigned o3 = v3 + un * s3, o9 = v9 + un * s9, oc = v_ctrl + un * kC, orc = un * rec_step;
      constexpr unsigned kUp = ODE ? 1u : 0u;
      unsigned og_xs = u_xs + (un + kUp) * sg_xs, og_xds = u_xds + (un + kUp) * sg_xds, og_om = u_om + (un + kUp) * sg_om;
      unsigned og_r = u_r + (un + kUp) * sg_r, og_fs = u_fs + (un + kUp) * sg_fs, og_ff = u_ff + (un + kUp) * sg_ff;
      int ti = max(n, 0);
      auto request_state = [&](StateIn& d, Saved& v) {
        d.x = zero;
#ifdef MF_STREAM_NO_FETCH
        d.xd = S(0.1); d.w = S(0.01); d.R0 = cc == 0 ? one : zero; d.R1 = cc == 1 ? one : zero; d.R2 = cc == 2 ? one : zero; d.cv = S(0.5); d.cw = S(0.1);
        d.t1 = S(0.01); d.t0 = zero; v.q = f4v{S(100.3), S(0.2), S(0.1), S(50.0)};
        return;
#endif
        if constexpr (ODE) {
          d.xd = bload1<S>(rXds, o3, 0u); d.w = bload1<S>(rOm, o3, 0u);
          bload3(rRs, o9, 0u, &d.R0, &d.R1, &d.R2);
          d.t1 = a.ts[ti + 1]; d.t0 = a.ts[ti];
        } else {
          const bool init = ti == 0;
          const unsigned p3 = init ? o3 : o3 - s3, p9 = init ? o9 : o9 - s9;
          const S xd = bload1<S>(rXds, p3, 0u), w = bload1<S>(rOm, p3, 0u);
          S R0, R1, R2;
          bload3(rRs, p9, 0u, &R0, &R1, &R2);
          d.xd = init ? ini.xd : xd; d.w = init ? ini.w : w;
          d.R0 = init ? ini.R0 : R0; d.R1 = init ? ini.R1 : R1; d.R2 = init ? ini.R2 : R2;
          d.x = bload1<S>(rOm, o3, 0u);
          d.t1 = a.dt; d.t0 = zero;
        }
        bload2(rCtrl, oc, 0u, &d.cv, &d.cw);
        v.q = __builtin_nontemporal_load(reinterpret_cast<const f4v*>(prec + (size_t)orc));
      };
      auto request_up = [&](UpIn& u) {
#ifdef MF_STREAM_NO_FETCH
        u.gXs = S(0.001);
        if constexpr (!XS_ONLY) { u.gXds = u.gOm = u.gR0 = u.gR1 = u.gR2 = u.gFs = u.gFf = S(0.001); }
        return;
#endif
        u.gXs = bload1<S>(rgXs, og_xs, 0u);
        if constexpr (!XS_ONLY) {
          u.gXds = bload1<S>(rgXds, og_xds, 0u); u.gOm = bload1<S>(rgOm, og_om, 0u);
          bload3(rgRs, og_r, 0u, &u.gR0, &u.gR1, &u.gR2);
          u.gFs = bload1<S>(rgFs, og_fs, 0u); u.gFf = bload1<S>(rgFf, og_ff, 0u);
        }
      };
      auto step_back_up = [&]() {
        og_xs -= sg_xs;
        if constexpr (!XS_ONLY) { og_xds -= sg_xds; og_om -= sg_om; og_r -= sg_r; og_fs -= sg_fs; og_ff -= sg_ff; }
      };
      constexpr int kSlots = SLOTS, kPlanesD = ODE ? 0 : 6, kPlanes = (XS_ONLY ? 10 : 12) + kPlanesD;
      constexpr bool kPow2 = (kSlots & (kSlots - 1)) == 0;
      __shared__ f4v ring[kSlots * kPlanes * 64];
      __shared__ int flags[4];
      typedef __attribute__((address_space(3))) volatile int LdsCounter;
      LdsCounter* vflags = (LdsCounter*)flags;
      if (threadIdx.x == 0) { flags[0] = 0; flags[1] = 0; flags[2] = 0; flags[3] = 0; }
      __syncthreads();
      const bool loss_val = loss_on && a.loss_out != nullptr;
      __shared__ S l_part[3 * 16];
      auto loss_share = [&](S acc) {
        if (!loss_val) return;
        const int wv = (int)(threadIdx.x >> 6);
        if (lane < 16) l_part[wv * 16 + lane] = zero;
        if (p == 0 && q < 3) l_part[wv * 16 + (lane >> 4) * 4 + q] = acc;
        asm volatile("" ::: "memory");
        if (lane == 0) __hip_atomic_fetch_add(&flags[2], 1, __ATOMIC_RELAXED, __HIP_MEMORY_SCOPE_WORKGROUP);
      };
      auto loss_value_finish = [&]() {
        if (!loss_val) return;
        while (__builtin_amdgcn_readfirstlane(vflags[2]) != 3) __builtin_amdgcn_s_sleep(1);
        asm volatile("" ::: "memory");
        unsigned last_wg = 0u;
        if (lane == 0) {
          S tot = zero;
#pragma unroll
          for (int r = 0; r < 4; ++r)
#pragma unroll
            for (int v = 0; v < 3; ++v) tot += (l_part[v * 16 + r * 4 + 0] + l_part[v * 16 + r * 4 + 1]) + l_part[v * 16 + r * 4 + 2];
          __builtin_nontemporal_store(tot, a.loss_partial + blockIdx.x);
          __threadfence();
          last_wg = atomicAdd(a.loss_ticket, 1u) == gridDim.x - 1 ? 1u : 0u;
        }
        last_wg = __builtin_amdgcn_readfirstlane(last_wg);
        if (last_wg) {
          __threadfence();
          const int n_act = min(64, (a.B - (int)blockIdx.x * 4) * 16);
          S tot = zero;
          for (unsigned k0 = (unsigned)lane; k0 < gridDim.x; k0 += 8u * (unsigned)n_act) {
            S v[8];
#pragma unroll
            for (int i = 0; i < 8; ++i) {
              const unsigned k2 = k0 + (unsigned)(i * n_act);
              v[i] = __builtin_nontemporal_load(a.loss_partial + min(k2, gridDim.x - 1u));
              v[i] = k2 < gridDim.x ? v[i] : zero;
            }
#pragma unroll
            for (int i = 0; i < 8; ++i) tot += v[i];
          }
          S sum = zero;
#pragma unroll
          for (int k2 = 0; k2 < 64; ++k2) sum += k2 < n_act ? mf_readlane(tot, k2) : zero;
          if (lane == 0) {
            a.loss_out[0] = sum * a.loss_inv_count;
            *a.loss_ticket = 0u;
          }
        }
      };
      __shared__ S snap_c[4 * 64];
      auto snap_prepare = [&]() {
        if (!a.skip_snap) {
          S wq, dx, dy;
          int idx;
          snap_cell(idx, wq, dx, dy);
          snap_c[lane] = idx_as(zero, idx); snap_c[64 + lane] = wq; snap_c[128 + lane] = dx; snap_c[192 + lane] = dy;
        }
        asm volatile("" ::: "memory");
        vflags[3] = 1;
      };
      if (threadIdx.x >= 64) {
        static_assert(kSlots % BATCH == 0 && (BATCH == 2 || BATCH == 3), "a batch must not wrap around the ring");
        struct Slot { StateIn st; Saved sv; UpIn up; S lg, lw; int sj; };
        unsigned zero_lane = 0u;
        asm("" : "+v"(zero_lane));
        const int fk = __builtin_amdgcn_readfirstlane((int)(threadIdx.x >> 6)) - 1;
        int m = n;
        S l_acc = zero;
        auto fetch = [&](Slot& r) {
          request_state(r.st, r.sv);
          request_up(r.up);
          r.sj = ld32(l_row_stamp, (unsigned)ti + kUp + zero_lane);
          r.lw = ld32(l_row_w, (unsigned)ti + kUp + zero_lane);
          r.lg = zero;
          o3 -= s3; o9 -= s9; oc -= kC; orc -= rec_step; --ti;
          step_back_up();
          --m;
        };
        constexpr unsigned kB = (unsigned)BATCH;
        auto skip3 = [&]() {
          o3 -= kB * s3; o9 -= kB * s9; oc -= kB * kC; orc -= kB * rec_step; ti -= BATCH; m -= BATCH;
          og_xs -= kB * sg_xs;
          if constexpr (!XS_ONLY) { og_xds -= kB * sg_xds; og_om -= kB * sg_om; og_r -= kB * sg_r; og_fs -= kB * sg_fs; og_ff -= kB * sg_ff; }
        };
        MF_PROF_T(t_fetcher);
        MF_PROF_ACC(acc_room); MF_PROF_ACC(acc_pub);
        auto room = [&](int upto) {
          MF_PROF_T(t0);
          while (upto - __builtin_amdgcn_readfirstlane(vflags[1]) > kSlots) __builtin_amdgcn_s_sleep(2);
          asm volatile("" ::: "memory");
          MF_PROF_SUM(acc_room, t0);
        };
        int pub = 0;
        auto publish_written = [&](int upto) {
          asm volatile("" ::: "memory");
          if (__builtin_amdgcn_readfirstlane(vflags[0]) == pub) { vflags[0] = upto; pub = upto; }
        };
        auto publish = [&](int upto) {
          asm volatile("" ::: "memory");
          MF_PROF_T(t0);
          if (pub != upto) {
            while (__builtin_amdgcn_readfirstlane(vflags[0]) != pub) __builtin_amdgcn_s_sleep(1);
            asm volatile("" ::: "memory");
            vflags[0] = upto; pub = upto;
          }
          MF_PROF_SUM(acc_pub, t0);
        };
        auto put = [&](const Slot& r, unsigned slot, int o) {
            Rec k;
            rebuild(r.st, r.sv, k);
            const S mw = inside(k.wraw, -a.omega_max, a.omega_max) ? one : zero;
            const S mG = inside(k.Gf, -mg, mg) ? one : zero;
            const S mF1 = inside(k.F1, -mg, mg) ? one : zero;
            const S invNn = k.Nn > zero ? M::div(one, k.Nn) : zero;
            const S cmask = k.coln2 >= S(1e-12) ? one : zero;
            const S cs = k.cj * k.inv_csum;
            const f4v p0 = f4v{k.R0, k.R1, k.R2, k.h};
            const f4v p1 = f4v{k.w1, k.w2, k.r1, k.r2};
            const f4v p2 = f4v{k.f1, k.f2, mw, mG * k.stv};
            const f4v p3 = f4v{mG * k.Nn, k.nrm, k.s, k.sn};
            const f4v p4 = f4v{k.cmdv, k.mub, k.tv * k.mub, k.Fr * invNn};
            const f4v p5 = f4v{mF1 * cs, mF1 * k.nrm, k.A, -(a.k * cs)};
            const f4v p6 = f4v{-(a.damp * cs), -(k.A * k.inv_csum), k.A * k.cj * k.inv_csum * k.inv_csum, -S(10.0) * k.cj * (one - k.cj)};
            const f4v p7 = f4v{k.vp, -(k.inl * a.inv_res), k.wq, idx_as(zero, k.idx)};
            const f4v p8 = f4v{k.zc, k.mcv, wa_s * k.wb * a.inv_res, wb_s * k.wa * a.inv_res};
            const Msk smask = r.sj >= 0 ? ~(Msk)0 : (Msk)0;
            const S gXs_row = bfi(loss_mask, bfi(smask, cp_loss_grad(loss_scale, r.up.gXs, r.lg, r.lw), zero), r.up.gXs);
            l_acc += bfi(smask, cp_loss_term(r.up.gXs, r.lg, r.lw), zero);
            const f4v p9 = f4v{k.e, k.il, cmask * k.e * k.il, first * gXs_row};
            f4v d0 = {zero, zero, zero, zero}, d1 = d0, d2 = d0, d3 = d0, d4 = d0, d5 = d0;
            if constexpr (!ODE) {
              const S h = a.dt, wn = r.st.x;
              const S th2 = dot3(wn, wn);
              const S idn = M::inv_len(th2);
              const S kv = wn * idn;
              const S th = M::sqrt(th2);
              S sn_, oc;
              M::sincos_small(th * h, &sn_, &oc);
              const S kk = dot3(kv, kv);
              const S kv1 = dpp<kRot1>(kv), kv2 = dpp<kRot2>(kv);
              const S ok = oc * kv;
              const S m0 = mf_fma(ok, kv, mf_fma(-oc, kk, one)), m1 = mf_fma(ok, kv1, -(sn_ * kv2)), m2 = mf_fma(ok, kv2, sn_ * kv1);
              const S q0 = dpp<kB0>(kv), q1 = dpp<kB1>(kv), q2 = dpp<kB2>(kv);
              const S Rk = k.R0 * q0 + k.R1 * q1 + k.R2 * q2;
              const S idn2 = th2 >= S(1e-12) ? idn * idn : zero;
              const S ith = th2 > zero ? M::div(one, th) : zero;
              d0 = f4v{wn, kv, q0, q1};
              d1 = f4v{q2, Rk, kk, sn_};
              d2 = f4v{oc, h * (one - oc), h * sn_, idn};
              d3 = f4v{idn2, ith, dpp<kB0>(m0), dpp<kB0>(m1)};
              d4 = f4v{dpp<kB0>(m2), dpp<kB1>(m2), dpp<kB1>(m0), dpp<kB1>(m1)};
              d5 = f4v{dpp<kB2>(m1), dpp<kB2>(m2), dpp<kB2>(m0), zero};
            }
            room(o + 1);
            f4v* out = ring + slot * (unsigned)(kPlanes * 64) + lane;
            out[0] = p0; out[64] = p1; out[128] = p2; out[192] = p3; out[256] = p4; out[320] = p5; out[384] = p6; out[448] = p7; out[512] = p8; out[576] = p9;
            if constexpr (!XS_ONLY) {
              out[640] = f4v{first * r.up.gXds, first * r.up.gOm, r.up.gFs, r.up.gFf};
              out[704] = f4v{first * r.up.gR0, first * r.up.gR1, first * r.up.gR2, zero};
            }
            if constexpr (!ODE) {
              constexpr int D0 = (XS_ONLY ? 10 : 12) * 64;
              out[D0] = d0; out[D0 + 64] = d1; out[D0 + 128] = d2; out[D0 + 192] = d3; out[D0 + 256] = d4; out[D0 + 320] = d5;
            }
            publish_written(o + 1);
#ifdef MF_STREAM_PROFILE
            if (o == 0) MF_PROF_ADD(18, t_k0);
#endif
          };
        int ord = BATCH * fk;
        unsigned sbase = kB * (unsigned)fk;
        auto fetch3 = [&](Slot (&s)[BATCH]) {
#pragma unroll
          for (int i = 0; i < BATCH; ++i) fetch(s[i]);
          skip3();
        };
        auto gather1 = [&](Slot& r) {
          gather_cells(r.sv);
          r.lg = loss_gt_lane[(size_t)(unsigned)min(max(r.sj, 0), l_T2m1) * 3u];
        };
        auto gather3 = [&](Slot (&s)[BATCH]) {
#pragma unroll
          for (int i = 0; i < BATCH; ++i) gather1(s[i]);
        };
        auto put3 = [&](const Slot (&s)[BATCH]) {
          pub = ord;
#pragma unroll
          for (int i = 0; i < BATCH; ++i) put(s[i], sbase + (unsigned)i, ord + i);
          publish(ord + BATCH);
          ord += 2 * BATCH;
          if constexpr (kSlots != 2 * BATCH) sbase = sbase + 2u * kB >= (unsigned)kSlots ? sbase + 2u * kB - (unsigned)kSlots : sbase + 2u * kB;
        };
        Slot A[BATCH], B[BATCH], C[BATCH];
        const int n_full = (n + 1) / BATCH;
        int full = (n_full - fk + 1) / 2;
        if (fk == 1) skip3();
        if (full >= 2) {
          fetch3(A); fetch3(B); gather3(A);
          full -= 2;
          while (full >= 3) {
            fetch3(C); gather3(B); put3(A);
            fetch3(A); gather3(C); put3(B);
            fetch3(B); gather3(A); put3(C);
            full -= 3;
          }
          if (full == 0) { gather3(B); put3(A); put3(B); }
          else if (full == 1) { fetch3(C); gather3(B); put3(A); gather3(C); put3(B); put3(C); }
          else { fetch3(C); gather3(B); put3(A); fetch3(A); gather3(C); put3(B); gather3(A); put3(C); put3(A); }
        } else if (full == 1) { fetch3(A); gather3(A); put3(A); }
        if (fk == (n_full & 1)) {
          int o = BATCH * n_full;
          unsigned sl = sbase;
          while (m >= 0) {
            Slot r0;
            fetch(r0);
            gather1(r0);
            pub = o;
            put(r0, sl, o);
            publish(o + 1);
            ++sl; ++o;
          }
        }
        MF_PROF_ADD(2 + 4 * fk, t_fetcher);
        MF_PROF_OUT(0 + 4 * fk, acc_room); MF_PROF_OUT(1 + 4 * fk, acc_pub);
        loss_share(l_acc);
        if (fk == 0) {
          MF_PROF_T(t_lf);
          loss_value_finish();
          MF_PROF_DRAIN();
          MF_PROF_ADD(21, t_lf);
#ifdef MF_STREAM_PROFILE
          MF_PROF_MAX(17, __builtin_readcyclecounter() - t_lf);
          MF_PROF_MAX(14, __builtin_amdgcn_s_memrealtime());
#endif
        } else {
          snap_prepare();
        }
        return;
      }
        int consumed = 0, seen = 0;
        unsigned rslot = 0u;
        UpIn uZ;
        load_upstream(0, uZ);
        S l_row0 = zero;
        if (loss_on && ODE) {
          const S g0 = loss_gt_lane[(size_t)max(a.loss_row_stamp[0], 0) * 3u], w0 = a.loss_row_w[0];
          const bool stamped = a.loss_row_stamp[0] >= 0;
          l_row0 = stamped ? cp_loss_term(uZ.gXs, g0, w0) : zero;
          uZ.gXs = stamped ? cp_loss_grad(loss_scale, uZ.gXs, g0, w0) : zero;
        }
        loss_share(l_row0);
        struct Coef {
          S R0, R1, R2, h, w1, w2, r1, r2, f1, f2, mw;
          S stvG, NnG, nrm, s, sn;
          S cmdv, mub, tvm, FrN;
          S csm, nm1, A, kcs;
          S dcs, Aic, Acc, dcj;
          S vp, inlr, wq, zc, mcv, wsb, wsa;
          S e, il, eci;
          int idx;
          S wn, kv, q0, q1, q2, Rk, kk, sn_, oc, cga, cgb, idn, idn2, ith;
          S M00, M01, M02, M10, M11, M12, M20, M21, M22;
        };
        MF_PROF_T(t_compute);
        MF_PROF_ACC(acc_wait);
#ifdef MF_STREAM_PROFILE
        unsigned long long acc_wait_early = 0, acc_wait_late = 0, n_waited = 0;
#endif
        auto ensure = [&](int k) {
          MF_PROF_T(t0);
          int have = __builtin_amdgcn_readfirstlane(seen);
          while (have < consumed + k) have = __builtin_amdgcn_readfirstlane(vflags[0]);
          asm volatile("" ::: "memory");
          MF_PROF_SUM(acc_wait, t0);
#ifdef MF_STREAM_PROFILE
          const unsigned long long dt = __builtin_readcyclecounter() - t0;
          if (consumed < 30) acc_wait_early += dt;
          if (consumed >= n_steps - 30) acc_wait_late += dt;
          n_waited += __builtin_amdgcn_readfirstlane(seen) < consumed + k ? 1u : 0u;
#endif
        };
        auto grab = [&](Coef& c, UpIn& up) {
          const f4v* o = ring + (kPow2 ? (unsigned)(consumed & (kSlots - 1)) : rslot) * (unsigned)(kPlanes * 64) + lane;
          if constexpr (!kPow2) rslot = rslot + 1u == (unsigned)kSlots ? 0u : rslot + 1u;
          const f4v c0 = o[0], c1 = o[64], c2 = o[128], c3 = o[192], c4 = o[256], c5 = o[320], c6 = o[384], c7 = o[448], c8 = o[512], c9 = o[576];
          const S idx_bits = c7.w;
          c.R0 = c0.x; c.R1 = c0.y; c.R2 = c0.z; c.h = c0.w;
          c.w1 = c1.x; c.w2 = c1.y; c.r1 = c1.z; c.r2 = c1.w;
          c.f1 = c2.x; c.f2 = c2.y; c.mw = c2.z; c.stvG = c2.w;
          c.NnG = c3.x; c.nrm = c3.y; c.s = c3.z; c.sn = c3.w;
          c.cmdv = c4.x; c.mub = c4.y; c.tvm = c4.z; c.FrN = c4.w;
          c.csm = c5.x; c.nm1 = c5.y; c.A = c5.z; c.kcs = c5.w;
          c.dcs = c6.x; c.Aic = c6.y; c.Acc = c6.z; c.dcj = c6.w;
          c.vp = c7.x; c.inlr = c7.y; c.wq = c7.z; c.idx = idx_of(idx_bits);
          c.zc = c8.x; c.mcv = c8.y; c.wsb = c8.z; c.wsa = c8.w;
          c.e = c9.x; c.il = c9.y; c.eci = c9.z; up.gXs = c9.w;
          if constexpr (!XS_ONLY) {
            const f4v g0 = o[640];
            const S* g1 = reinterpret_cast<const S*>(o + 704);
            up.gXds = g0.x; up.gOm = g0.y; up.gFs = g0.z; up.gFf = g0.w; up.gR0 = g1[0]; up.gR1 = g1[1]; up.gR2 = g1[2];
          }
          if constexpr (!ODE) {
            constexpr int D0 = (XS_ONLY ? 10 : 12) * 64;
            const f4v e0 = o[D0], e1 = o[D0 + 64], e2 = o[D0 + 128], e3 = o[D0 + 192], e4 = o[D0 + 256];
            const S* e5 = reinterpret_cast<const S*>(o + D0 + 320);
            c.wn = e0.x; c.kv = e0.y; c.q0 = e0.z; c.q1 = e0.w;
            c.q2 = e1.x; c.Rk = e1.y; c.kk = e1.z; c.sn_ = e1.w;
            c.oc = e2.x; c.cga = e2.y; c.cgb = e2.z; c.idn = e2.w;
            c.idn2 = e3.x; c.ith = e3.y; c.M00 = e3.z; c.M01 = e3.w;
            c.M02 = e4.x; c.M10 = e4.y; c.M11 = e4.z; c.M12 = e4.w;
            c.M20 = e5[0]; c.M21 = e5[1]; c.M22 = e5[2];
          }
          ++consumed;
        };
        auto release = [&]() {
          seen = vflags[0];
          asm volatile("" ::: "memory");
          vflags[1] = consumed;
        };
        auto take = [&](Coef& c, UpIn& up) { ensure(1); grab(c, up); release(); };
        auto chain = [&](int n, const Coef& c, const UpIn& up) {
          const S h = c.h;
          S gFr_up = zero, gFf_up = zero, gxdd, gwd;
          if constexpr (ODE) {
          if constexpr (!XS_ONLY) {
            laFs += act ? up.gFs : zero;
            laFf += act ? up.gFf : zero;
            gFr_up = h * laFs; gFf_up = h * laFf;
          }
          gxdd = h * sum_points(lxd); gwd = h * sum_points(lw);
          lxd = mf_fma(h, lx, lxd);
          const S g0 = h * lR0, g1 = h * lR1, g2 = h * lR2;
          const S g01 = dpp<kRot1>(g0), g02 = dpp<kRot2>(g0), g11 = dpp<kRot1>(g1), g12 = dpp<kRot2>(g1), g21 = dpp<kRot1>(g2), g22 = dpp<kRot2>(g2);
          lw += (dpp<kRot1>(c.R0) * g02 - dpp<kRot2>(c.R0) * g01) + (dpp<kRot1>(c.R1) * g12 - dpp<kRot2>(c.R1) * g11) + (dpp<kRot1>(c.R2) * g22 - dpp<kRot2>(c.R2) * g21);
          lR0 += g01 * c.w2 - g02 * c.w1;
          lR1 += g11 * c.w2 - g12 * c.w1;
          lR2 += g21 * c.w2 - g22 * c.w1;
          } else {
            if constexpr (!XS_ONLY) { gFr_up = act ? up.gFs : zero; gFf_up = act ? up.gFf : zero; }
            const S Lk = lR0 * c.q0 + lR1 * c.q1 + lR2 * c.q2;
            const S Gk0 = dot3(c.R0, Lk), Gk1 = dot3(c.R1, Lk), Gk2 = dot3(c.R2, Lk);
            const S Gt0 = dot3(c.Rk, lR0), Gt1 = dot3(c.Rk, lR1), Gt2 = dot3(c.Rk, lR2);
            const S trG = sum3(c.R0 * lR0 + c.R1 * lR1 + c.R2 * lR2);
            const S a0 = sum3(c.R1 * lR2 - c.R2 * lR1), a1 = sum3(c.R2 * lR0 - c.R0 * lR2), a2 = sum3(c.R0 * lR1 - c.R1 * lR0);
            const S ga = -(c.q0 * a0 + c.q1 * a1 + c.q2 * a2);
            const S gb = (c.q0 * Gk0 + c.q1 * Gk1 + c.q2 * Gk2) - c.kk * trG;
            S gth = ga * c.cga + gb * c.cgb;
            const S ac = mask_or(mask_or(mask_or(zero, a0, lane0), a1, lane1), a2, lane2);
            const S sc = mask_or(mask_or(mask_or(zero, Gk0 + Gt0, lane0), Gk1 + Gt1, lane1), Gk2 + Gt2, lane2);
            const S gk = -(c.sn_ * ac) - c.oc * (S(2.0) * trG * c.kv - sc);
            const S gkw = dot3(gk, c.wn);
            gth = mf_fma(-gkw, c.idn2, gth);
            lw += mf_fma(gth * c.ith, c.wn, gk * c.idn);
            gwd = h * sum_points(lw);
            lxd = mf_fma(h, lx, lxd);
            gxdd = h * sum_points(lxd);
            const S n0 = lR0 * c.M00 + lR1 * c.M01 + lR2 * c.M02;
            const S n1 = lR0 * c.M10 + lR1 * c.M11 + lR2 * c.M12;
            const S n2 = lR0 * c.M20 + lR1 * c.M21 + lR2 * c.M22;
            lR0 = n0; lR1 = n1; lR2 = n2;
          }
          const S mwd = c.mw * gwd;
          const S gtau = J0 * dpp<kB0>(mwd) + J1 * dpp<kB1>(mwd) + J2 * dpp<kB2>(mwd);
          const S gt1 = dpp<kRot1>(gtau), gt2 = dpp<kRot2>(gtau);
          const S gq = mf_fma(gxdd, a.inv_mass, gt1 * c.r2 - gt2 * c.r1);
          S gr = c.f1 * gt2 - c.f2 * gt1;
          S gFr = gFr_up + gq;
          const S gFf_ = gFf_up + gq;
          const S gNn = dot3(gFf_, c.stvG);
          const S gst = c.NnG * gFf_;
          const S gsn = -dot3(gst, c.nrm);
          S gn = gsn * c.s - c.sn * gst;
          const S gslip = mf_fma(gsn, c.nrm, gst);
          const S gmuq = dot3(gslip, c.cmdv);
          const S gcmd = c.mub * gslip;
          S gvp = -gcmd;
          const S ge_p = c.tvm * gslip;
          S gv_p = zero, gwc_p = zero;
          if constexpr (GCTRL) {
            const S gtv = dot3(gcmd, c.e);
            gv_p = tv_v * gtv; gwc_p = tv_w * gtv;
          }
          gFr = mf_fma(gNn, c.FrN, gFr);
          const S gF0 = gFr * c.csm;
          const S d1 = dot3(gFr, c.nm1);
          gn = mf_fma(-c.A, gF0, gn);
          const S gvn = c.dcs * d1;
          gvp = mf_fma(gvn, c.nrm, gvp);
          gn = mf_fma(gvn, c.vp, gn);
          const S gcw = mf_fma(c.Aic, d1, sum_points(c.Acc * d1));
          const S gdh = mf_fma(gcw, c.dcj, c.kcs * d1);
          const S gzq = -gdh;
          const S dotn = dot3(gn, c.nrm);
          const S gg = (gn - dotn * c.nrm) * c.inlr;
          const S ggp = dpp<0x51>(gg);
          const S nz = mf_fma(gzq, c.wq, cgA * gg + cgB * ggp);
          const S nm = gmuq * c.wq;
          {
            const unsigned ni = (unsigned)c.idx;
            const bool same = !act | (ni == acc_idx);
            st_pending = !same;
            st_idx = acc_idx; st_z = acc_z; st_m = acc_m;
            acc_idx = act ? ni : acc_idx;
            acc_z = same ? acc_z + nz : nz;
            acc_m = same ? acc_m + nm : nm;
          }
          const S vq = gzq * c.zc + gmuq * c.mcv;
          const S gpx = dot4(vq, c.wsb), gpy = dot4(vq, c.wsa);
          const S gp = mask_or(mask_or(mask_or(zero, gpx, lane0), gpy, lane1), gdh, lane2);
          const S gvp1 = dpp<kRot1>(gvp), gvp2 = dpp<kRot2>(gvp);
          gr += gvp1 * c.w2 - gvp2 * c.w1;
          const S gw_p = c.r1 * gvp2 - c.r2 * gvp1;
          const S qa = gp + gr;
          lx += gp; lxd += gvp; lw += gw_p;
          lR0 = mf_fma(qa, P0, lR0); lR1 = mf_fma(qa, P1, lR1); lR2 = mf_fma(qa, P2, lR2);
          S gv = zero, gwc = zero;
          if constexpr (GCTRL) { gv = sum_points(gv_p); gwc = sum_points(gwc_p); }
          lR0 = mf_fma(-dot3(ge_p, c.e), c.eci, mf_fma(ge_p, c.il, lR0));
          gctrl_pending = __builtin_amdgcn_readfirstlane((unsigned)n * kC); gv_pending = gv; gwc_pending = gwc;
        };
        auto crunch = [&](int n, const Coef& c, const UpIn& up, Coef& c_next, UpIn& up_next, auto more, auto paired) {
          add_upstream_masked(up);
          if constexpr (decltype(paired)::value == 1) grab(c_next, up_next);
          else if constexpr (decltype(paired)::value == 2) { grab(c_next, up_next); release(); }
          else if constexpr (decltype(more)::value) take(c_next, up_next);
          flush_stash();
          if constexpr (GCTRL) bstore2(rGctrl, v_ctrl, gctrl_pending, gv_pending, gwc_pending);
#ifdef MF_STREAM_NO_VJP
          asm volatile("" :: "v"(c.R0), "v"(c.w1), "v"(c.f1), "v"(c.NnG), "v"(c.cmdv), "v"(c.csm), "v"(c.dcs), "v"(c.vp), "v"(c.zc), "v"(c.e));
#else
          chain(n, c, up);
#endif
        };
        using std::true_type;
        using std::false_type;
        Coef cA, cB;
        if (n_steps > 0) {
          take(cA, uA);
          MF_PROF_ADD(3, t_k0); MF_PROF_OUT(19, acc_wait);
          using single = std::integral_constant<int, 0>;
          for (; n >= 2; n -= 2) {
            ensure(2);
            crunch(n, cA, uA, cB, uB, true_type{}, std::integral_constant<int, 1>{});
            crunch(n - 1, cB, uB, cA, uA, true_type{}, std::integral_constant<int, 2>{});
          }
          if (n == 1) { crunch(1, cA, uA, cB, uB, true_type{}, single{}); crunch(0, cB, uB, cA, uA, false_type{}, single{}); }
          else crunch(0, cA, uA, cB, uB, false_type{}, single{});
        }
        MF_PROF_ADD(9, t_compute);
        MF_PROF_OUT(8, acc_wait);
#ifdef MF_STREAM_PROFILE
        MF_PROF_OUT(22, acc_wait_early); MF_PROF_OUT(23, n_waited); MF_PROF_OUT(24, acc_wait_late);
#endif
        MF_PROF_ADD(20, t_k0);
        MF_PROF_DRAIN();
        MF_PROF_T(t_sw);
        if (!a.skip_snap) {
          while (__builtin_amdgcn_readfirstlane(vflags[3]) == 0) __builtin_amdgcn_s_sleep(1);
          asm volatile("" ::: "memory");
          snap_idx = idx_of(snap_c[lane]); snap_wq = snap_c[64 + lane]; snap_dx = snap_c[128 + lane]; snap_dy = snap_c[192 + lane];
        }
        MF_PROF_DRAIN();
        MF_PROF_ADD(7, t_sw);
        uA = uZ; uB = uZ;
    } else {
      struct Raw { StateIn st; Saved sv; };
      Raw S_[3];
      Rec K_[3];
      UpIn U_[3];
      auto up_row = [&](int m) { return ODE ? max(m + 1, 0) : max(m, 0); };
      auto run = [&](auto rtag, int n) {
        constexpr int R = decltype(rtag)::value, R1 = (R + 1) % 3, R2 = (R + 2) % 3;
        add_upstream_state(U_[R]);
        gather_cells(S_[R1].sv);
#ifndef MF_SAVED_NO_STATE
        load_state(max(n - 3, 0), S_[R].st);
#endif
#ifndef MF_SAVED_NO_REC
        load_saved(max(n - 3, 0), S_[R].sv);
#endif
#ifndef MF_SAVED_NO_UP
        load_upstream(min(up_row(n - 2), a.T - 1), U_[R2]);
#endif
#ifndef MF_SAVED_NO_ATOMIC
        flush_stash();
#endif
        if constexpr (GCTRL) bstore2(rGctrl, v_ctrl, gctrl_pending, gv_pending, gwc_pending);
#ifndef MF_SAVED_NO_VJP
        vjp(n, K_[R], U_[R]);
#endif
#ifndef MF_SAVED_NO_VJP
        asm("" : "+v"(S_[R1].sv.zc), "+v"(S_[R1].sv.mc) : "v"(lR0));
#endif
#ifndef MF_SAVED_NO_REBUILD
        rebuild(S_[R1].st, S_[R1].sv, K_[R1]);
#endif
      };
      const int n0 = max(n, 0);
      load_state(n0, S_[0].st);
      load_saved(n0, S_[0].sv);
      load_upstream(min(up_row(n0), a.T - 1), U_[0]);
      load_state(max(n0 - 1, 0), S_[1].st);
      load_saved(max(n0 - 1, 0), S_[1].sv);
      load_upstream(min(up_row(n0 - 1), a.T - 1), U_[1]);
      load_state(max(n0 - 2, 0), S_[2].st);
      load_saved(max(n0 - 2, 0), S_[2].sv);
      gather_cells(S_[0].sv);
      rebuild(S_[0].st, S_[0].sv, K_[0]);
      __builtin_amdgcn_s_waitcnt(0);
      using std::integral_constant;
      int i = 0;
      for (; i + 2 < n_steps; i += 3) {
        run(integral_constant<int, 0>{}, n0 - i);
        run(integral_constant<int, 1>{}, n0 - i - 1);
        run(integral_constant<int, 2>{}, n0 - i - 2);
      }
      if (i < n_steps) run(integral_constant<int, 0>{}, n0 - i);
      if (i + 1 < n_steps) run(integral_constant<int, 1>{}, n0 - i - 1);
      {
        const int r0 = (n0 + 1) % 3;
        uA = r0 == 0 ? U_[0] : (r0 == 1 ? U_[1] : U_[2]);
        uB = uA;
      }
      n = -1;
    }
  } else {
  load_state(max(n, 0), sA);
  load_upstream(min(max(n, 0) + (ODE ? 1 : 0), a.T - 1), uA);
  load_state(max(n - 1, 0), sB);
  recompute_gather(sA, recA);
  recompute(recA);
  __builtin_amdgcn_s_waitcnt(0);
  for (; n >= 1; n -= 2) {
    body(n, recA, recB, sB, sA, uA, uB);
    body(n - 1, recB, recA, sA, sB, uB, uA);
  }
  if (n == 0) body(0, recA, recB, sB, sA, uA, uB);
  }
  MF_PROF_T(t_e0);
  UpIn up = (n_steps & 1) ? uB : uA;
  flush_stash();
  if constexpr (GCTRL) bstore2(rGctrl, v_ctrl, gctrl_pending, gv_pending, gwc_pending);
  if (act) emit(acc_idx, acc_z, acc_m);
  if constexpr (ODE) {
    if (n_steps == 0) load_upstream(0, up);
    add_upstream_state(up);
  }
  lx = sum_points(lx); lxd = sum_points(lxd); lw = sum_points(lw);
  lR0 = sum_points(lR0); lR1 = sum_points(lR1); lR2 = sum_points(lR2);
  MF_PROF_DRAIN();
  MF_PROF_ADD(10, t_e0);
  MF_PROF_T(t_s0);

  S gx0 = lx;
  if (!a.skip_snap) {
    if constexpr (!STREAM) snap_cell(snap_idx, snap_wq, snap_dx, snap_dy);
    const S g = dpp<kB2>(lx) / (S)a.N;
    if (act) atomic_add(at32(gzmap, goff + (unsigned)snap_idx), g * snap_wq);
    const S gpx = snap_dx * g * a.inv_res, gpy = snap_dy * g * a.inv_res;
    S gpxy = q == 0 ? gpx : (q == 1 ? gpy : zero);
    gpxy = act ? gpxy : zero;
    gx0 = (q < 2 ? lx : zero) + sum_points(gpxy);
    lR0 += sum_points(gpxy * P0); lR1 += sum_points(gpxy * P1); lR2 += sum_points(gpxy * P2);
  }
  if (p == 0) {
    if (a.gx0) a.gx0[b * 3 + cc] = gx0;
    a.gxd0[b * 3 + cc] = lxd;
    a.gw0[b * 3 + cc] = lw;
    a.gR0[b * 9 + cc * 3 + 0] = lR0; a.gR0[b * 9 + cc * 3 + 1] = lR1; a.gR0[b * 9 + cc * 3 + 2] = lR2;
  }
#ifdef MF_STREAM_PROFILE
  if constexpr (STREAM) {
    MF_PROF_DRAIN();
    MF_PROF_ADD(11, t_s0);
    MF_PROF_RT(rt_end);
    MF_PROF_ADD(12, t_k0);
    MF_PROF_MAX(13, __builtin_readcyclecounter() - t_k0);
    MF_PROF_MAX(14, rt_end); MF_PROF_MAX(15, ~rt_k0); MF_PROF_OUT(16, rt_end - rt_k0);
  }
#endif
  if constexpr (WIN) {
    __syncthreads();
    win_close(a, win, wx0, wy0);
  }
}

bool use_component_parallel_bwd(const MfRolloutDesc* d, const MfRolloutBwdBufs* p, int scalar_bytes = 4);
long long cp_record_bytes(const MfRolloutDesc* d, int scalar_bytes);
bool cp_loss_fusable(const MfRolloutDesc* d);
bool cp_bwd_wants_zmu(const MfRolloutDesc* d, bool has_rec, bool has_mu);
int launch_rollout_bwd_cp_f32(const RolloutBwdArgs<float>& a, int integ, bool xs_only, hipStream_t st);
int launch_rollout_bwd_cp_dynamics_f32(const RolloutBwdArgs<float>& a, bool xs_only, hipStream_t st);
void launch_rollout_bwd_cp_stream_f32(const RolloutBwdArgs<float>& a, bool xs_only, unsigned grid, hipStream_t st);
void launch_rollout_bwd_cp_stream_dynamics_f32(const RolloutBwdArgs<float>& a, bool xs_only, unsigned grid, hipStream_t st);

inline unsigned cp_stream_max_grid(int integ = MF_INTEG_ODEINT_EULER) {
  static const int env = getenv("MF_CP_STREAM_MAX_GRID") ? atoi(getenv("MF_CP_STREAM_MAX_GRID")) : -1;
  const unsigned cus = (unsigned)device_cus();
  const unsigned v = env >= 0 ? (unsigned)env : 2u * cus;
  return integ == MF_INTEG_ODEINT_EULER ? v : (v < cus ? v : cus);
}

void launch_rollout_bwd_cp_stream_f64(const RolloutBwdArgs<double>& a, bool xs_only, unsigned grid, hipStream_t st);
int launch_rollout_bwd_cp_f64(const RolloutBwdArgs<double>& a, int integ, bool xs_only, hipStream_t st);
inline void launch_rollout_bwd_cp_stream_any(const RolloutBwdArgs<float>& a, int integ, bool xs_only, unsigned grid, hipStream_t st) {
  if (integ == MF_INTEG_ODEINT_EULER) launch_rollout_bwd_cp_stream_f32(a, xs_only, grid, st); else launch_rollout_bwd_cp_stream_dynamics_f32(a, xs_only, grid, st);
}
inline void launch_rollout_bwd_cp_stream_any(const RolloutBwdArgs<double>& a, int, bool xs_only, unsigned grid, hipStream_t st) {
  launch_rollout_bwd_cp_stream_f64(a, xs_only, grid, st);
}
template <typename S>
inline unsigned cp_stream_max_grid_of(int integ) {
  if (sizeof(S) == 8) return integ == MF_INTEG_ODEINT_EULER ? cp_stream_max_grid(integ) : 0u;
  return cp_stream_max_grid(integ);
}
template <typename S, int INTEG>
int launch_rollout_bwd_cp_variant(const RolloutBwdArgs<S>& a, bool xs_only, hipStream_t st) {
  const long long threads = (long long)a.B * 16;
  const unsigned grid = (unsigned)((threads + 63) / 64);
  const unsigned block = wave_unit_block(grid), wgs = (unsigned)((threads + block - 1) / block);
  const bool gc = a.gcontrols != nullptr;
  static const int forced = getenv("MF_CP_BWD_MODE") ? atoi(getenv("MF_CP_BWD_MODE")) : -1;
  const int saved_mode = grid <= cp_stream_max_grid_of<S>(INTEG) && forced != kCpSaved ? kCpStream : kCpSaved;
  const int mode = a.rec ? saved_mode : (forced >= 0 && forced < kCpSaved ? forced : ((long long)grid <= device_simds() ? kCpLate : kCpEarly));
#define MF_BCP(XS_, GC_, M_) MF_KLAUNCH((rollout_bwd_cp_kernel<S, INTEG, XS_, GC_, M_>), dim3(wgs), dim3(block), 0, st, a)
  constexpr bool kZmu = std::is_same<S, float>::value && INTEG == MF_INTEG_ODEINT_EULER;
#define MF_BCP_Z(XS_, GC_) do { if constexpr (kZmu) { if (a.zmu) { MF_KLAUNCH((rollout_bwd_cp_kernel<S, INTEG, XS_, GC_, kCpSaved, 6, 3, kZmu>), dim3(wgs), dim3(block), 0, st, a); break; } } MF_BCP(XS_, GC_, kCpSaved); } while (0)
  static const bool win_off = getenv("MF_BWD_WIN") && atoi(getenv("MF_BWD_WIN")) == 0;
  constexpr bool kWin = std::is_same<S, float>::value;
  const bool win = kWin && !win_off && mode == kCpEarly && a.map_shared && a.H == a.W && (a.H & (a.H - 1)) == 0 && threads % 512 == 0;
#define MF_BCP_W(XS_, GC_) do { if constexpr (kWin) { if (win) { MF_KLAUNCH((rollout_bwd_cp_kernel<S, INTEG, XS_, GC_, kCpEarly, 6, 3, false, kWin>), dim3((unsigned)(threads / 512)), dim3(512), 0, st, a); break; } } MF_BCP(XS_, GC_, kCpEarly); } while (0)
#define MF_BCP_L(XS_, GC_) do { if (mode == kCpStream) launch_rollout_bwd_cp_stream_any(a, INTEG, xs_only, grid, st); else if (mode == kCpSaved) MF_BCP_Z(XS_, GC_); else if (mode == kCpLate) MF_BCP(XS_, GC_, kCpLate); else MF_BCP_W(XS_, GC_); } while (0)
  bool one1_done = false;
  if constexpr (std::is_same<S, float>::value) {
    if (xs_only && a.loss_gt != nullptr && mode != kCpStream) {
      MF_REQUIRE(mode == kCpEarly, MF_ERR_UNSUPPORTED, "rollout_bwd: only the early-recompute one-wave form carries a fused loss");
      one1_done = true;
#define MF_BCP1(GC_, M_, Z_, W_, G_, B_) MF_KLAUNCH((rollout_bwd_cp_kernel<S, INTEG, true, GC_, M_, 6, 3, Z_, W_, true>), dim3(G_), dim3(B_), 0, st, a)
#define MF_BCP1_L(GC_) do {                                                                                                   \
        if (win) MF_BCP1(GC_, kCpEarly, false, kWin, (unsigned)(threads / 512), 512);                                    \
        else MF_BCP1(GC_, kCpEarly, false, false, wgs, block);                                                                \
      } while (0)
      if (gc) MF_BCP1_L(true); else MF_BCP1_L(false);
#undef MF_BCP1_L
#undef MF_BCP1
    }
  }
  if (!one1_done) {
    MF_REQUIRE(a.loss_gt == nullptr || mode == kCpStream, MF_ERR_UNSUPPORTED, "rollout_bwd: the one-wave fused physics loss exists for float32 positions-only launches");
    if (xs_only) { if (gc) MF_BCP_L(true, true); else MF_BCP_L(true, false); }
    else         { if (gc) MF_BCP_L(false, true); else MF_BCP_L(false, false); }
  }
#undef MF_BCP_L
#undef MF_BCP_W
#undef MF_BCP_Z
#undef MF_BCP
  hipError_t e = hipGetLastError();
  MF_REQUIRE(e == hipSuccess, MF_ERR_LAUNCH, std::string("rollout_bwd (component-parallel) launch: ") + hipGetErrorString(e));
  return MF_OK;
}

}
```

monoforce_amd/csrc/rollout_bwd_kernel.h:

```cpp
#pragma once
#include "rollout_fwd_kernel.h"

namespace mf {

template <typename S>
struct RolloutBwdArgs {
  int B, T, N, H, W, n_tracks, layout, map_shared, skip_snap, grad_copies;
  S mass, inv_mass, mg, k, damp, omega_max, res, inv_res, d_max, dt, half_ly, sink;
  S Iinv[9];
  const S *z, *mu, *controls, *ts, *points;
  const int* part;
  const S *x_init, *xd0, *R0, *w0;
  const S *Xraw, *Xds, *Rs, *Om;
  const S *gXs, *gXds, *gRs, *gOm, *gFs, *gFf;
  int sXs, sXds, sRs, sOm, sFs, sFf;
  S *gz, *gmu, *gcontrols, *gx0, *gxd0, *gR0, *gw0;
  const S* joint_angles;
  S joint_xyz[12];
  S* gjoint;
  const S* rec;
  const S* zmu;
  int loss_T2;
  const S* loss_gt;
  const int* loss_row_stamp;
  const S* loss_row_w;
  const S* loss_gloss;
  S loss_inv_count;
  S* loss_partial;
  unsigned* loss_ticket;
  S* loss_out;
  const int* loss_near;
  const S* loss_w;
  int gc_sb, gc_st;
};

#ifdef MF_NO_ATOMICS
__device__ __forceinline__ void atomic_add(float* p, float v) { if (v == 1.2345e-30f) *p = v; }
#else
__device__ __forceinline__ void atomic_add(float* p, float v) { unsafeAtomicAdd(p, v); }
#endif
__device__ __forceinline__ void atomic_add(double* p, double v) { unsafeAtomicAdd(p, v); }

__device__ __forceinline__ void lds_add(float* p, float v) {
  __builtin_amdgcn_ds_faddf((__attribute__((address_space(3))) float*)p, v, __ATOMIC_RELAXED, __HIP_MEMORY_SCOPE_WORKGROUP, false);
}
__device__ __forceinline__ void lds_add(double* p, double v) { unsafeAtomicAdd(p, v); }
template <typename S>
__device__ __forceinline__ bool inside(S v, S lo, S hi) { return v >= lo && v <= hi; }
template <typename S>
__device__ __forceinline__ S* at32(S* base, unsigned elem) {
  return reinterpret_cast<S*>(reinterpret_cast<char*>(base) + (size_t)(elem * (unsigned)sizeof(S)));
}

#define MF_CROSS(o, a, b)                    \
  do {                                       \
    (o)[0] = (a)[1] * (b)[2] - (a)[2] * (b)[1]; \
    (o)[1] = (a)[2] * (b)[0] - (a)[0] * (b)[2]; \
    (o)[2] = (a)[0] * (b)[1] - (a)[1] * (b)[0]; \
  } while (0)

constexpr int kWinW = 128;
template <typename S, bool FAST>
__device__ __forceinline__ void win_open(const RolloutBwdArgs<S>& a, S* win, int b0, int* wx0, int* wy0) {
  b0 = min(b0, a.B - 1);
  const int cx = (int)mf_clamp(Mth<S, FAST>::cell_coord(a.x_init[b0 * 3 + 0], a.d_max, a.res, a.inv_res), (S)-262144.0, (S)262144.0);
  const int cy = (int)mf_clamp(Mth<S, FAST>::cell_coord(a.x_init[b0 * 3 + 1], a.d_max, a.res, a.inv_res), (S)-262144.0, (S)262144.0);
  *wx0 = __builtin_amdgcn_readfirstlane(max(min(cx - kWinW / 2, a.H - kWinW), 0));
  *wy0 = __builtin_amdgcn_readfirstlane(max(min(cy - kWinW / 2, a.H - kWinW), 0));
  typedef float f4 __attribute__((ext_vector_type(4)));
  for (int i = threadIdx.x; i < 2 * kWinW * kWinW / 4; i += blockDim.x) reinterpret_cast<f4*>(win)[i] = f4{0.f, 0.f, 0.f, 0.f};
}
template <typename S>
__device__ __forceinline__ bool win_emit(S* win, unsigned win_flat0, unsigned win_shift, unsigned h_mask, unsigned idx, S vz, S vm, bool want_gmu) {
  const unsigned d = idx - win_flat0, rx = d >> win_shift, ry = d & h_mask;
  if ((rx < (unsigned)kWinW) & (ry < (unsigned)kWinW)) {
    S* wz = win + (rx * kWinW + ry);
    lds_add(wz, vz);
    if (want_gmu) lds_add(wz + kWinW * kWinW, vm);
    return true;
  }
  return false;
}
template <typename S>
__device__ __forceinline__ void win_close(const RolloutBwdArgs<S>& a, const S* win, int wx0, int wy0) {
  const unsigned HW = (unsigned)a.H * (unsigned)a.W;
  const unsigned coff = (a.map_shared ? (unsigned)(blockIdx.x % a.grad_copies) : 0u) * HW;
  const bool want_gmu = a.gmu != nullptr && a.mu != nullptr;
  for (int i = threadIdx.x; i < kWinW * kWinW; i += blockDim.x) {
    const int ix = wx0 + i / kWinW, iy = wy0 + i % kWinW;
    if (ix < a.H && iy < a.H) {
      const unsigned cell = (unsigned)iy + (unsigned)a.H * (unsigned)ix;
      const S vz = win[i];
      if (vz != (S)0) atomic_add(at32(a.gz, coff + cell), vz);
      if (want_gmu) {
        const S vm = win[kWinW * kWinW + i];
        if (vm != (S)0) atomic_add(at32(a.gmu, coff + cell), vm);
      }
    }
  }
}
template <typename S>
__device__ __forceinline__ S xs_loss_grad(S scale, S xs, S g, S w) {
#pragma clang fp contract(off)
  return scale * w * (xs * w - g * w);
}
template <typename S>
__device__ __forceinline__ S xs_loss_term(S xs, S g, S w) {
#pragma clang fp contract(off)
  const S d = xs * w - g * w;
  return d * d;
}
template <typename S>
__device__ __forceinline__ void xs_loss_value_finish(const RolloutBwdArgs<S>& a, S acc) {
  if (a.loss_out == nullptr) return;
  __shared__ S wave_sum[8];
  __shared__ unsigned last_wg;
  const int nw = (int)((blockDim.x + 63) >> 6), lane = (int)(threadIdx.x & 63), wv = (int)(threadIdx.x >> 6);
#pragma unroll
  for (int d = 32; d >= 1; d >>= 1) acc += __shfl_xor(acc, d, 64);
  if (lane == 0) wave_sum[wv] = acc;
  __syncthreads();
  if (threadIdx.x == 0) {
    S tot = (S)0;
    for (int k = 0; k < nw; ++k) tot += wave_sum[k];
    __builtin_nontemporal_store(tot, a.loss_partial + blockIdx.x);
    __threadfence();
    last_wg = atomicAdd(a.loss_ticket, 1u) == gridDim.x - 1 ? 1u : 0u;
  }
  __syncthreads();
  if (!last_wg) return;
  __threadfence();
  S tot = (S)0;
  for (unsigned k = threadIdx.x; k < gridDim.x; k += blockDim.x) tot += __builtin_nontemporal_load(a.loss_partial + k);
#pragma unroll
  for (int d = 32; d >= 1; d >>= 1) tot += __shfl_xor(tot, d, 64);
  __syncthreads();
  if (lane == 0) wave_sum[wv] = tot;
  __syncthreads();
  if (threadIdx.x == 0) {
    S sum = (S)0;
    for (int k = 0; k < nw; ++k) sum += wave_sum[k];
    a.loss_out[0] = sum * a.loss_inv_count;
    *a.loss_ticket = 0u;
  }
}
template <typename S, int G, int PPL, int INTEG, bool FAST, bool JOINTS, bool CARRY, bool XS_ONLY, bool ZMU, bool WIN, bool LOSS = false>
__device__ __forceinline__ void rollout_bwd_body(const RolloutBwdArgs<S>& a, S* win, const unsigned win_flat0, const unsigned win_shift, S* l_acc = nullptr) {
  using M = Mth<S, FAST>;
  const int tid = blockIdx.x * blockDim.x + threadIdx.x;
  const int b = tid / G;
  const int gl = tid % G;
  if (b >= a.B) return;
  const S one = (S)1, zero = (S)0;
  const int HW = a.H * a.W, last = HW - 1;
  __shared__ S gs_lds[G > 64 ? 2 * (G / 64) * kGroupSumMaxValues : 1];
  GroupSum<G, S> gs;
  gs.lds = gs_lds;
  const unsigned moff = a.map_shared ? 0u : (unsigned)b * (unsigned)HW;
  const S* zmap = a.z;
  const bool has_mu = a.mu != nullptr;
  const S* mumap = has_mu ? a.mu : a.z;
  const unsigned goff = a.map_shared ? (unsigned)(b % a.grad_copies) * (unsigned)HW : (unsigned)b * (unsigned)HW;
  S* gzmap = a.gz;
  const bool want_gmu = a.gmu != nullptr && has_mu;
  S* gmumap = want_gmu ? a.gmu : a.gz;

  S P[PPL][3];
  S P0[PPL][3];
  S Iv[9];
  int part[PPL];
  bool act[PPL];
#pragma unroll
  for (int j = 0; j < PPL; ++j) {
    int i = gl * PPL + j;
    act[j] = i < a.N;
    int ii = act[j] ? i : 0;
    P[j][0] = P0[j][0] = a.points[ii * 3 + 0];
    P[j][1] = P0[j][1] = a.points[ii * 3 + 1];
    P[j][2] = P0[j][2] = a.points[ii * 3 + 2];
    part[j] = act[j] ? a.part[ii] : -1;
  }
#pragma unroll
  for (int c = 0; c < 9; ++c) Iv[c] = a.Iinv[c];

  const size_t row_stride = (a.layout == MF_LAYOUT_TIME_MAJOR) ? (size_t)a.B : 1;
  const size_t row0 = (a.layout == MF_LAYOUT_TIME_MAJOR) ? (size_t)b : (size_t)b * a.T;
  const S* ctrl = a.controls + (size_t)b * a.T * 2;
  S* gctrl = a.gcontrols + (size_t)b * (size_t)a.gc_sb;

  constexpr bool UNSUM = XS_ONLY && G <= 64 && !JOINTS;
  const S up_lane = (!UNSUM || gl == 0) ? one : zero;
  S lx[3] = {zero, zero, zero}, lxd[3] = {zero, zero, zero}, lw[3] = {zero, zero, zero}, lR[9];
#pragma unroll
  for (int c = 0; c < 9; ++c) lR[c] = zero;
  S laFs[PPL][3], laFf[PPL][3];
#pragma unroll
  for (int j = 0; j < PPL; ++j)
#pragma unroll
    for (int c = 0; c < 3; ++c) laFs[j][c] = laFf[j][c] = zero;

  struct StateIn {
    S x[3], xd[3], R[9], w[3];
    S cv, cw, t0, t1;
  };
  struct UpIn {
    S gXs[3], gXds[3], gRs[9], gOm[3];
    S gFs[PPL][3], gFf[PPL][3];
    S lg[3], lw;
    bool stamped;
  };
  static_assert(!LOSS || XS_ONLY, "the fused physics loss is a positions-only upstream");
  const S loss_scale = LOSS ? (S)2 * a.loss_gloss[0] * a.loss_inv_count : zero;
  const S* const loss_gt_b = LOSS ? a.loss_gt + (size_t)b * (size_t)a.loss_T2 * 3u : nullptr;
  S l_val = zero;
  int l_opaque_zero = 0;
  if constexpr (LOSS) asm volatile("v_mov_b32 %0, 0" : "=v"(l_opaque_zero));
  int l_j = LOSS ? a.loss_T2 - 1 + l_opaque_zero : 0;
  int l_row = LOSS ? a.loss_near[l_j] : -1;
  S l_w = LOSS ? a.loss_w[l_j] : zero;
  const S* l_gt = LOSS ? loss_gt_b + (size_t)(unsigned)l_j * 3u : nullptr;
  const int* const l_near_tab = LOSS ? a.loss_near : nullptr;
  const S* const l_w_tab = LOSS ? a.loss_w : nullptr;
  const int n_steps = (INTEG == MF_INTEG_ODEINT_EULER) ? a.T - 1 : a.T;
  struct Ptrs {
    const S *x, *xd, *w, *R, *c, *t, *g1, *g2, *g3, *g4;
    const S* f1[PPL];
    const S* f2[PPL];
    int trow;
  };
  auto make_ptrs = [&](int m, Ptrs& p) {
    const size_t in_row = row0 + (size_t)(INTEG == MF_INTEG_ODEINT_EULER ? m : m - 1) * row_stride;
    const size_t out_row = row0 + (size_t)(INTEG == MF_INTEG_ODEINT_EULER ? min(m + 1, a.T - 1) : m) * row_stride;
    p.x = a.Xraw + in_row * 3; p.xd = a.Xds + in_row * 3; p.w = a.Om + in_row * 3; p.R = a.Rs + in_row * 9;
    p.c = ctrl + (size_t)m * 2; p.t = a.ts + m;
    p.g1 = a.gXs + out_row * a.sXs; p.g2 = a.gXds + out_row * a.sXds; p.g3 = a.gOm + out_row * a.sOm; p.g4 = a.gRs + out_row * a.sRs;
    p.trow = INTEG == MF_INTEG_ODEINT_EULER ? min(m + 1, a.T - 1) : m;
#pragma unroll
    for (int j = 0; j < PPL; ++j) {
      const size_t pt = out_row * a.N + min(gl * PPL + j, a.N - 1);
      p.f1[j] = a.gFs + pt * a.sFs; p.f2[j] = a.gFf + pt * a.sFf;
    }
  };
  const size_t d3 = row_stride * 3, d9 = row_stride * 9;
  const size_t dg1 = row_stride * a.sXs, dg2 = row_stride * a.sXds, dg3 = row_stride * a.sOm, dg4 = row_stride * a.sRs;
  const size_t df1 = row_stride * a.N * a.sFs, df2 = row_stride * a.N * a.sFf;
  auto step_back = [&](Ptrs& p, size_t k) {
    p.x -= k * d3; p.xd -= k * d3; p.w -= k * d3; p.R -= k * d9; p.c -= k * 2; p.t -= k;
    p.g1 -= k * dg1; p.g2 -= k * dg2; p.g3 -= k * dg3; p.g4 -= k * dg4;
    p.trow -= (int)k;
#pragma unroll
    for (int j = 0; j < PPL; ++j) { p.f1[j] -= k * df1; p.f2[j] -= k * df2; }
  };
  auto load_state = [&](const Ptrs& p, int m, StateIn& s) {
    const bool init = (INTEG == MF_INTEG_DYNAMICS) && m == 0;
    const S* sx = init ? a.x_init + b * 3 : p.x;
    const S* sxd = init ? a.xd0 + b * 3 : p.xd;
    const S* sw = init ? a.w0 + b * 3 : p.w;
    const S* sR = init ? a.R0 + b * 9 : p.R;
#pragma unroll
    for (int c = 0; c < 3; ++c) { s.x[c] = sx[c]; s.xd[c] = sxd[c]; s.w[c] = sw[c]; }
#pragma unroll
    for (int c = 0; c < 9; ++c) s.R[c] = sR[c];
    s.cv = p.c[0]; s.cw = p.c[1];
    s.t0 = p.t[0]; s.t1 = p.t[m + 1 < a.T ? 1 : 0];
  };
  auto load_upstream = [&](const Ptrs& p, UpIn& u) {
#pragma unroll
    for (int c = 0; c < 3; ++c) u.gXs[c] = p.g1[c];
    if constexpr (LOSS) {
      u.stamped = (p.trow == l_row) & (l_j >= 0);
      u.lw = l_w;
#pragma unroll
      for (int c = 0; c < 3; ++c) u.lg[c] = l_gt[c];
      l_j -= u.stamped ? 1 : 0;
      l_gt -= (u.stamped & (l_j >= 0)) ? 3 : 0;
      const unsigned jn = (unsigned)max(l_j, 0);
      l_row = l_near_tab[jn];
      l_w = l_w_tab[jn];
    }
    if constexpr (!XS_ONLY) {
#pragma unroll
      for (int c = 0; c < 3; ++c) { u.gXds[c] = p.g2[c]; u.gOm[c] = p.g3[c]; }
#pragma unroll
      for (int c = 0; c < 9; ++c) u.gRs[c] = p.g4[c];
#pragma unroll
      for (int j = 0; j < PPL; ++j)
#pragma unroll
        for (int c = 0; c < 3; ++c) { u.gFs[j][c] = p.f1[j][c]; u.gFf[j][c] = p.f2[j][c]; }
    }
  };
  auto add_upstream_state = [&](const UpIn& u) {
    S g[3] = {u.gXs[0], u.gXs[1], u.gXs[2]};
    if constexpr (LOSS) {
#pragma unroll
      for (int c = 0; c < 3; ++c) g[c] = u.stamped ? xs_loss_grad(loss_scale, u.gXs[c], u.lg[c], u.lw) : zero;
      const S e2 = xs_loss_term(u.gXs[0], u.lg[0], u.lw) + xs_loss_term(u.gXs[1], u.lg[1], u.lw) + xs_loss_term(u.gXs[2], u.lg[2], u.lw);
      l_val += (u.stamped & (gl == 0)) ? e2 : zero;
    }
    if constexpr (UNSUM) {
      const S ms = up_lane * a.sink;
      lx[0] += up_lane * g[0]; lx[1] += up_lane * g[1]; lx[2] += up_lane * g[2];
      lR[2] += g[0] * ms; lR[5] += g[1] * ms; lR[8] += g[2] * ms;
    } else {
    lx[0] += g[0]; lx[1] += g[1]; lx[2] += g[2];
    lR[2] += g[0] * a.sink; lR[5] += g[1] * a.sink; lR[8] += g[2] * a.sink;
    }
    if constexpr (!XS_ONLY) {
      lxd[0] += u.gXds[0]; lxd[1] += u.gXds[1]; lxd[2] += u.gXds[2];
#pragma unroll
      for (int c = 0; c < 9; ++c) lR[c] += u.gRs[c];
      lw[0] += u.gOm[0]; lw[1] += u.gOm[1]; lw[2] += u.gOm[2];
    }
  };

  if (INTEG == MF_INTEG_ODEINT_EULER) {
    if (gl == 0) { gctrl[(a.T - 1) * a.gc_st + 0] = zero; gctrl[(a.T - 1) * a.gc_st + 1] = zero; }
  }

  unsigned acc_idx[PPL][4], st_idx[PPL][4];
  S acc_z[PPL][4], acc_m[PPL][4], st_z[PPL][4], st_m[PPL][4];
  bool st_pending[PPL], st_all[PPL];
  constexpr bool carry_over = CARRY;
#pragma unroll
  for (int j = 0; j < PPL; ++j) {
    st_pending[j] = st_all[j] = false;
#pragma unroll
    for (int q = 0; q < 4; ++q) { acc_idx[j][q] = st_idx[j][q] = 0u; acc_z[j][q] = acc_m[j][q] = st_z[j][q] = st_m[j][q] = zero; }
  }
  auto emit = [&](unsigned idx, S vz, S vm) {
    if constexpr (WIN) {
      if (win_emit(win, win_flat0, win_shift, (unsigned)(a.H - 1), idx, vz, vm, want_gmu)) return;
    }
    atomic_add(at32(gzmap, goff + idx), vz);
    if (want_gmu) atomic_add(at32(gmumap, goff + idx), vm);
  };
  auto flush_stash = [&]() {
// ... 642 lines not shown
```

monoforce_amd/dphysics_bwd.py:

```python
import ctypes as C

import torch

from . import _lib, _timing

import os

GRAD_COPIES = int(os.environ.get('MF_GRAD_COPIES', '32'))
WIN_GRAD_COPIES = int(os.environ.get('MF_GRAD_COPIES_WIN', '64'))


def grad_copies_for(B, N):
    floor = GRAD_COPIES if N <= 4 else max(GRAD_COPIES, min(256, max(64, (B * N) // 512)))
    return max(1, min(max(floor, B // 64), 256, B))


class GradPool:

    def __init__(self, n_maps, copies, n, dt, dev):
        self.n_maps, self.copies, self.n = n_maps, copies, n
        self.buf = torch.zeros(n_maps * copies * n + 16, dtype=dt, device=dev)
        self.busy = False
        self.stream = None
        self.pinned = False
        self.done = None

    def acquire(self):
        cur_s = torch.cuda.current_stream(self.buf.device)
        cur = cur_s.cuda_stream
        capturing = torch.cuda.is_current_stream_capturing()
        self.pinned = self.pinned or capturing
        if self.busy or (self.stream is not None and self.stream != cur):
            if self.done is not None and not capturing:
                cur_s.wait_event(self.done)
            self.buf.zero_()
        self.busy, self.stream = True, cur

    def reduce(self, map_shape):
        from .dphysics import _scalar_suffix
        flat = torch.empty(self.n_maps * self.n + 1, dtype=self.buf.dtype, device=self.buf.device)
        out = flat[:-1].view((self.n_maps,) + tuple(map_shape))
        fn = getattr(_lib.lib(), 'mf_reduce_grad_copies_' + _scalar_suffix(self.buf.dtype))
        with torch.cuda.device(self.buf.device):
            _lib.check(fn(_lib.ptr(self.buf), self.n_maps, self.copies, C.c_longlong(self.n), _lib.ptr(out),
                          C.c_void_p(self.stream)), 'mf_reduce_grad_copies')
        if not torch.cuda.is_current_stream_capturing():
            if self.done is None:
                self.done = torch.cuda.Event()
            self.done.record(torch.cuda.current_stream(self.buf.device))
        self.busy = False
        return out


MAX_IDLE_POOLS = 4


def grad_pool(owner, n_maps, copies, n, dt, dev):
    pools = owner.__dict__.setdefault('_grad_pools', {})
    key = (n_maps, copies, n, dt, dev)
    p = pools.pop(key, None)
    if p is None:
        idle = [k for k, q in pools.items() if not q.pinned and not q.busy]
        for k in idle[:max(len(idle) - (MAX_IDLE_POOLS - 1), 0)]:
            del pools[k]
        p = GradPool(n_maps, copies, n, dt, dev)
    pools[key] = p
    p.acquire()
    return p

def rollout_backward(ctx, gXs, gXds, gRs, gOm, gFs, gFf, gloss=None):
    with torch.cuda.device(ctx.saved_tensors[0].device):
        return _rollout_backward_on_device(ctx, gXs, gXds, gRs, gOm, gFs, gFf, gloss)


def _rollout_backward_on_device(ctx, gXs, gXds, gRs, gOm, gFs, gFf, gloss):
    from .dphysics import _scalar_suffix, _stream_ptr
    controls, x_init, xd0, R0, w0, ts, Xraw, Xds, Rs, Om = ctx.saved_tensors
    desc, keep, mod = ctx.desc, ctx.keep, ctx.mod
    dev, dt = controls.device, controls.dtype
    B, T = desc.B, desc.T
    tm = desc.layout == _lib.MF_LAYOUT_TIME_MAJOR

    def up(g):
        if g is None:
            return None
        g = g.to(dt)
        return (g.transpose(0, 1) if tm else g).contiguous()

    ups = [up(g) for g in (gXs, gXds, gRs, gOm, gFs, gFf)]
    z, mu = keep['z'], keep['mu']
    want_gmu = mu is not None and ctx.needs_input_grad[2]
    if desc.map_shared:
        copies = grad_copies_for(B, desc.N)
        if (WIN_GRAD_COPIES and dt == torch.float32 and (gloss is not None or ups[0] is not None) and all(u is None for u in ups[1:])
                and _lib.lib().mf_rollout_bwd_window(C.byref(desc))):
            copies = min(copies, WIN_GRAD_COPIES)
        desc.grad_copies = copies
        n_maps = 2 if want_gmu else 1
        pool = grad_pool(mod, n_maps, copies, z.numel(), dt, dev)
        maps = pool.buf[:n_maps * copies * z.numel()].view((n_maps, copies) + tuple(z.shape))
        gz, gmu, zero_row = maps[0], (maps[1] if want_gmu else None), pool.buf[-16:]
    else:
        maps = None
        gz = torch.zeros_like(z)
        gmu = torch.zeros_like(mu) if want_gmu else None
        zero_row = torch.zeros(16, dtype=dt, device=dev)
    need_gc = ctx.needs_input_grad[3] or bool(_lib.lib().mf_rollout_bwd_wants_gcontrols(C.byref(desc)))
    gcontrols = torch.empty_like(controls) if need_gc else None
    gxd0, gR0, gw0 = torch.empty_like(xd0), torch.empty_like(R0), torch.empty_like(w0)
    gx0 = torch.empty_like(xd0) if ctx.needs_input_grad[4] else None
    ja = getattr(ctx, 'joint_angles', None)
    gja = torch.zeros_like(ja) if ja is not None and ctx.needs_input_grad[10] else None
    bufs = _lib.MfRolloutBwdBufs(
        z=_lib.ptr(z), mu=_lib.ptr(mu), controls=_lib.ptr(controls), ts=_lib.ptr(ts), points=_lib.ptr(keep['points']),
        part=_lib.ptr(mod._part_dev(dev)), x_init=_lib.ptr(x_init), xd0=_lib.ptr(xd0), R0=_lib.ptr(R0), w0=_lib.ptr(w0),
        Xraw=_lib.ptr(Xraw), Xds=_lib.ptr(Xds), Rs=_lib.ptr(Rs), Omegas=_lib.ptr(Om),
        gXs=_lib.ptr(ups[0]), gXds=_lib.ptr(ups[1]), gRs=_lib.ptr(ups[2]), gOmegas=_lib.ptr(ups[3]),
        gFs=_lib.ptr(ups[4]), gFf=_lib.ptr(ups[5]), zeros=_lib.ptr(zero_row),
        gz=_lib.ptr(gz), gmu=_lib.ptr(gmu), gcontrols=_lib.ptr(gcontrols), gx0=_lib.ptr(gx0),
        gxd0=_lib.ptr(gxd0), gR0=_lib.ptr(gR0), gw0=_lib.ptr(gw0), joint_angles=_lib.ptr(ja), gjoint_angles=_lib.ptr(gja),
        rec=_lib.ptr(getattr(ctx, 'rec', None)), zmu_scratch=_lib.ptr(getattr(ctx, 'zmu', (None, None))[0]), zmu=_lib.ptr(getattr(ctx, 'zmu', (None, None))[1]))
    if gloss is not None:
        spec, X_gt, Xs_rows, loss_out = ctx.loss
        gl = gloss.to(dt).reshape(1).contiguous()
        lstruct = _lib.MfRolloutLoss(T2=spec.T2, gt=_lib.ptr(X_gt), near=_lib.ptr(spec.near), w=_lib.ptr(spec.w), row_stamp=_lib.ptr(spec.row_stamp), row_w=_lib.ptr(spec.row_w),
                                     gloss=_lib.ptr(gl), Xs=_lib.ptr(Xs_rows))
        if loss_out is not None:
            lstruct.flags = _lib.MF_LOSS_VALUE_IN_BACKWARD
            lstruct.partial, lstruct.ticket, lstruct.loss = _lib.ptr(loss_out[1]), _lib.ptr(spec.ticket(dev, torch.cuda.current_stream(dev))), _lib.ptr(loss_out[0])
        bufs.loss = C.cast(C.pointer(lstruct), C.c_void_p)
    fn = getattr(_lib.lib(), 'mf_rollout_bwd_' + _scalar_suffix(dt))
    with torch.cuda.device(dev), _timing.timed('rollout_bwd_kernel', dev):
        _lib.check(fn(C.byref(desc), C.byref(bufs), _stream_ptr(dev)), 'mf_rollout_bwd')
    _timing.note_launch('rollout_bwd_kernel')

    if desc.map_shared:
        summed = pool.reduce(z.shape)
        gz, gmu = summed[0], (summed[1] if want_gmu else None)

    def to_input_shape(g, shape, expanded):
        if g is None:
            return None
        Bm = shape[0]
        if g.dim() == 3:
            if Bm == g.shape[0] and not expanded:
                return g
            gs_ = g.sum(0)
            if Bm == 1:
                return gs_.unsqueeze(0)
            g = gs_
        if Bm == 1:
            return g.unsqueeze(0)
        if Bm & (Bm - 1) == 0:
            return (g / Bm).unsqueeze(0).expand(shape)
        full = torch.zeros(shape, dtype=g.dtype, device=g.device)
        full[0] = g
        return full

    return (None, to_input_shape(gz, ctx.z_shape, ctx.z_expanded) if ctx.needs_input_grad[1] else None,
            to_input_shape(gmu, ctx.mu_shape, ctx.mu_expanded), gcontrols if ctx.needs_input_grad[3] else None, gx0,
            gxd0 if ctx.needs_input_grad[5] else None, gR0 if ctx.needs_input_grad[6] else None,
            gw0 if ctx.needs_input_grad[7] else None, None, None, gja)
```

monoforce_amd/ops.py:

```python
import ctypes as C

import torch

from . import _lib, _timing
from .dphysics_bwd import grad_copies_for, grad_pool


class _PoolOwner:
    pass


_POOL_OWNER = _PoolOwner()

__all__ = ['rollout', 'splat', 'CONST_NAMES']

CONST_NAMES = ('mass', 'gravity', 'stiffness', 'damping', 'grid_res', 'd_max', 'dt', 'omega_max', 'robot_size_y')

_L = torch.library.Library('monoforce', 'DEF')
_L.define('dphys_rollout_fwd(Tensor z, Tensor? mu, Tensor controls, Tensor x0, Tensor xd0, Tensor R0, Tensor w0, Tensor pts, '
          'Tensor part_id, Tensor Iinv, float[] consts, int integrator, bool save_for_bwd) -> (Tensor, Tensor, Tensor, Tensor, Tensor, Tensor, Tensor, Tensor, Tensor)')
_L.define('dphys_rollout_bwd(Tensor z, Tensor? mu, Tensor controls, Tensor x_init, Tensor xd0, Tensor R0, Tensor w0, Tensor pts, '
          'Tensor part_id, Tensor Iinv, float[] consts, int integrator, Tensor Xraw, Tensor Xds, Tensor Rs, Tensor Om, Tensor rec, '
          'Tensor? gXs, Tensor? gXds, Tensor? gRs, Tensor? gOm, Tensor? gFs, Tensor? gFf) -> (Tensor, Tensor, Tensor, Tensor, Tensor, Tensor, Tensor)')
_L.define('bev_splat_plan(Tensor geom, float[] dx, float[] bx, int[] nx) -> Tensor')
_L.define('bev_splat_fwd(Tensor x, Tensor plan, int B, int n_per_sample, float[] dx, float[] bx, int[] nx) -> Tensor')
_L.define('bev_splat_bwd(Tensor grad, Tensor plan, int B, int n_per_sample, int C, float[] dx, float[] bx, int[] nx) -> Tensor')
_L.define('mppi_perturb(Tensor nominal, Tensor noise, float[] sigma, float[] lo, float[] hi, bool keep_nominal) -> Tensor')
_L.define('path_costs(Tensor cost_rows, Tensor? force_cost, Tensor x_last, Tensor goal, float[] weights) -> (Tensor, Tensor)')
_L.define('mppi_update(Tensor costs, Tensor controls, Tensor nominal, float lam) -> (Tensor, Tensor, Tensor, Tensor)')


def _sfx(dtype):
    if dtype == torch.float32:
        return 'f32'
    if dtype == torch.float64:
        return 'f64'
    raise TypeError(f'monoforce ops compute in float32 or float64, got {dtype}')


def _stream(dev):
    return C.c_void_p(torch.cuda.current_stream(dev).cuda_stream)


def _rollout_desc(z, controls, pts, Iinv, consts, integrator):
    assert len(consts) in (len(CONST_NAMES), len(CONST_NAMES) + 1), f'consts = {CONST_NAMES} (+ traj_sim_time)'
    c = dict(zip(CONST_NAMES, (float(v) for v in consts)))
    B, T = controls.shape[:2]
    assert z.dim() == 3 and z.shape[0] in (1, B), 'z must be [B,H,W] or [1,H,W] (one map shared by all rollouts)'
    d = _lib.MfRolloutDesc(B=B, T=T, N=pts.shape[0], H=z.shape[1], W=z.shape[2], n_tracks=2, integrator=int(integrator),
                           layout=_lib.MF_LAYOUT_TIME_MAJOR, map_shared=int(z.shape[0] == 1), math_mode=_lib.MF_MATH_FAST,
                           mass=c['mass'], gravity=c['gravity'], stiffness=c['stiffness'], damping=c['damping'], omega_max=c['omega_max'],
                           grid_res=c['grid_res'], d_max=c['d_max'], dt=c['dt'], robot_size_y=c['robot_size_y'])
    for i, v in enumerate(Iinv.detach().double().flatten().tolist()):
        d.Iinv[i] = v
    return d


_TS = {}


def _time_grid(consts, T, dt, dev):
    step = float(consts[6])
    t_sim = float(consts[9]) if len(consts) > 9 else T * step
    key = (step, t_sim, T, dt, str(dev))
    if key not in _TS:
        _TS[key] = torch.linspace(0, t_sim, max(int(t_sim / step), T), dtype=dt)[:T].to(dev).contiguous()
    return _TS[key]


def _prep(z, mu, controls, pts, part_id, states=()):
    dt = z.dtype
    B = controls.shape[0]
    assert controls.dim() == 3 and controls.shape[2] == 2, f'controls must be [B,T,2], got {tuple(controls.shape)}'
    assert z.dim() == 3 and z.shape[0] in (1, B), f'z must be [B,H,W] or [1,H,W] (one map shared by all {B} rollouts), got {tuple(z.shape)}'
    if mu is not None:
        assert mu.dim() == 3 and tuple(mu.shape[1:]) == tuple(z.shape[1:]), \
            f'mu shape {tuple(mu.shape)} does not match the {z.shape[1]}x{z.shape[2]} height grid'
        assert mu.shape[0] in (1, B), f'mu batch {mu.shape[0]} is neither 1 (shared map) nor the {B} rollouts of controls'
        if mu.shape[0] != z.shape[0]:
            z, mu = z.expand(B, -1, -1), mu.expand(B, -1, -1)
    for name, t in states:
        assert t.shape[0] == B, f'{name} has {t.shape[0]} rows, controls {B} rollouts'
    assert pts.dim() == 2 and pts.shape[1] == 3 and part_id.shape[0] == pts.shape[0], 'pts must be [N,3] with one part id per point'
    cont = lambda t: None if t is None else t.to(dt).contiguous()
    return cont(z), cont(mu), cont(controls), cont(pts), part_id.to(torch.int32).contiguous()


@torch.library.impl(_L, 'dphys_rollout_fwd', 'CUDA')
def _rollout_fwd(z, mu, controls, x0, xd0, R0, w0, pts, part_id, Iinv, consts, integrator, save_for_bwd):
    dev, dt = z.device, z.dtype
    zc, muc, cc, pc, part = _prep(z, mu, controls, pts, part_id, (('x0', x0), ('xd0', xd0), ('R0', R0), ('w0', w0)))
    d = _rollout_desc(zc, cc, pc, Iinv, consts, integrator)
    if dt == torch.float64:
        d.math_mode = _lib.MF_MATH_EXACT
    B, T, N = d.B, d.T, d.N
    x0 = x0.to(dt).contiguous().clone()
    with torch.cuda.device(dev):
        Np = _lib.lib().mf_rollout_force_stride(C.byref(d))
        nrec = int(_lib.lib().mf_rollout_record_bytes(C.byref(d))) // 4 if (save_for_bwd and dt == torch.float32) else 0
    d.force_stride = Np
    new = lambda *tail: torch.empty(T, B, *tail, dtype=dt, device=dev)
    Xs, Xds, Rs, Om, Fs, Ff = new(3), new(3), new(3, 3), new(3), new(Np, 3), new(Np, 3)
    Xraw = new(3) if save_for_bwd else torch.empty(0, dtype=dt, device=dev)
    rec = torch.empty(nrec, dtype=dt, device=dev)
    ts = _time_grid(consts, T, dt, dev)
    bufs = _lib.MfRolloutFwdBufs(z=_lib.ptr(zc), mu=_lib.ptr(muc), controls=_lib.ptr(cc), ts=_lib.ptr(ts), points=_lib.ptr(pc),
                                 part=_lib.ptr(part), x0=_lib.ptr(x0), xd0=_lib.ptr(xd0.to(dt).contiguous()), R0=_lib.ptr(R0.to(dt).contiguous()),
                                 w0=_lib.ptr(w0.to(dt).contiguous()), Xs=_lib.ptr(Xs), Xds=_lib.ptr(Xds), Rs=_lib.ptr(Rs), Omegas=_lib.ptr(Om),
                                 Fs=_lib.ptr(Fs), Ff=_lib.ptr(Ff), Xraw=_lib.ptr(Xraw) if save_for_bwd else None,
                                 rec=_lib.ptr(rec) if nrec else None)
    with torch.cuda.device(dev), _timing.timed('rollout_fwd_kernel', dev):
        _lib.check(getattr(_lib.lib(), 'mf_rollout_fwd_' + _sfx(dt))(C.byref(d), C.byref(bufs), _stream(dev)), 'mf_rollout_fwd')
    tr = lambda t: t.transpose(0, 1)
    return tr(Xs), tr(Xds), tr(Rs), tr(Om), tr(Fs[:, :, :N]), tr(Ff[:, :, :N]), (tr(Xraw) if save_for_bwd else Xraw), x0, rec


@torch.library.impl(_L, 'dphys_rollout_bwd', 'CUDA')
def _rollout_bwd(z, mu, controls, x_init, xd0, R0, w0, pts, part_id, Iinv, consts, integrator, Xraw, Xds, Rs, Om, rec, gXs, gXds, gRs, gOm, gFs, gFf):
    dev, dt = z.device, z.dtype
    zc, muc, cc, pc, part = _prep(z, mu, controls, pts, part_id, (('x_init', x_init), ('xd0', xd0), ('R0', R0), ('w0', w0)))
    d = _rollout_desc(zc, cc, pc, Iinv, consts, integrator)
    if dt == torch.float64:
        d.math_mode = _lib.MF_MATH_EXACT
    B = d.B
    tm = lambda t: None if t is None else t.to(dt).transpose(0, 1).contiguous()
    saved = [tm(t) for t in (Xraw, Xds, Rs, Om)]
    ups = [tm(t) for t in (gXs, gXds, gRs, gOm, gFs, gFf)]
    if d.map_shared:
        copies = grad_copies_for(B, int(d.N))
        d.grad_copies = copies
        n_maps = 2 if muc is not None else 1
        pool = grad_pool(_POOL_OWNER, n_maps, copies, zc[0].numel(), dt, dev)
        maps = pool.buf[:n_maps * copies * zc[0].numel()].view((n_maps, copies) + tuple(zc.shape[1:]))
        gz, gmu, zero_row = maps[0], (maps[1] if muc is not None else None), pool.buf[-16:]
    else:
        gz, gmu = torch.zeros_like(zc), (torch.zeros_like(muc) if muc is not None else None)
        zero_row = torch.zeros(16, dtype=dt, device=dev)
    gcontrols = torch.empty_like(cc)
    gx0, gxd0, gR0, gw0 = (torch.empty(B, 3, dtype=dt, device=dev), torch.empty(B, 3, dtype=dt, device=dev),
                           torch.empty(B, 3, 3, dtype=dt, device=dev), torch.empty(B, 3, dtype=dt, device=dev))
    ts = _time_grid(consts, d.T, dt, dev)
    bufs = _lib.MfRolloutBwdBufs(
        z=_lib.ptr(zc), mu=_lib.ptr(muc), controls=_lib.ptr(cc), ts=_lib.ptr(ts), points=_lib.ptr(pc), part=_lib.ptr(part),
        x_init=_lib.ptr(x_init.to(dt).contiguous()), xd0=_lib.ptr(xd0.to(dt).contiguous()), R0=_lib.ptr(R0.to(dt).contiguous()),
        w0=_lib.ptr(w0.to(dt).contiguous()), Xraw=_lib.ptr(saved[0]), Xds=_lib.ptr(saved[1]), Rs=_lib.ptr(saved[2]), Omegas=_lib.ptr(saved[3]),
        gXs=_lib.ptr(ups[0]), gXds=_lib.ptr(ups[1]), gRs=_lib.ptr(ups[2]), gOmegas=_lib.ptr(ups[3]), gFs=_lib.ptr(ups[4]), gFf=_lib.ptr(ups[5]),
        zeros=_lib.ptr(zero_row), gz=_lib.ptr(gz), gmu=_lib.ptr(gmu), gcontrols=_lib.ptr(gcontrols), gx0=_lib.ptr(gx0), gxd0=_lib.ptr(gxd0),
        gR0=_lib.ptr(gR0), gw0=_lib.ptr(gw0), rec=_lib.ptr(rec) if rec.numel() else None)
    with torch.cuda.device(dev), _timing.timed('rollout_bwd_kernel', dev):
        _lib.check(getattr(_lib.lib(), 'mf_rollout_bwd_' + _sfx(dt))(C.byref(d), C.byref(bufs), _stream(dev)), 'mf_rollout_bwd')
    if d.map_shared:
        summed = pool.reduce(zc.shape[1:])
        gz = summed[0].unsqueeze(0)
        gmu = summed[1].unsqueeze(0) if muc is not None else None
    if gz.shape[0] != z.shape[0]:
        gz = gz.sum(0, keepdim=True)
    if gmu is not None and gmu.shape[0] != mu.shape[0]:
        gmu = gmu.sum(0, keepdim=True)
    if gmu is None:
        gmu = torch.zeros(0, dtype=dt, device=dev)
    return gz, gmu, gcontrols, gx0, gxd0, gR0, gw0


def _rollout_setup(ctx, inputs, output):
    z, mu, controls, x0, xd0, R0, w0, pts, part_id, Iinv, consts, integrator, save_for_bwd = inputs
    ctx.consts, ctx.integrator, ctx.has_mu = list(consts), integrator, mu is not None
    if not save_for_bwd:
        ctx.ok = False
        return
    ctx.ok = True
    Xs, Xds, Rs, Om, Fs, Ff, Xraw, x0s, rec = output
    ctx.save_for_backward(z, mu, controls, x0s, xd0, R0, w0, pts, part_id, Iinv, Xraw, Xds, Rs, Om, rec)
    ctx.set_materialize_grads(False)


def _rollout_backward(ctx, gXs, gXds, gRs, gOm, gFs, gFf, _gXraw, _gx0s, _grec):
    if not ctx.ok:
        raise RuntimeError('monoforce::dphys_rollout_fwd was called with save_for_bwd=False: no gradient available')
    z, mu, controls, x_init, xd0, R0, w0, pts, part_id, Iinv, Xraw, Xds, Rs, Om, rec = ctx.saved_tensors
    gz, gmu, gc, gx0, gxd0, gR0, gw0 = torch.ops.monoforce.dphys_rollout_bwd(
        z, mu, controls, x_init, xd0, R0, w0, pts, part_id, Iinv, ctx.consts, ctx.integrator, Xraw, Xds, Rs, Om, rec, gXs, gXds, gRs, gOm, gFs, gFf)
    return gz, (gmu if ctx.has_mu else None), gc, gx0, gxd0, gR0, gw0, None, None, None, None, None, None


torch.library.register_autograd('monoforce::dphys_rollout_fwd', _rollout_backward, setup_context=_rollout_setup, lib=_L)


@torch.library.register_fake('monoforce::dphys_rollout_fwd', lib=_L)
def _rollout_fwd_fake(z, mu, controls, x0, xd0, R0, w0, pts, part_id, Iinv, consts, integrator, save_for_bwd):
    B, T = controls.shape[:2]
    N = pts.shape[0]
    e = lambda *s: z.new_empty(s)
    return e(B, T, 3), e(B, T, 3), e(B, T, 3, 3), e(B, T, 3), e(B, T, N, 3), e(B, T, N, 3), (e(B, T, 3) if save_for_bwd else e(0)), e(B, 3), e(0)


@torch.library.register_fake('monoforce::dphys_rollout_bwd', lib=_L)
def _rollout_bwd_fake(z, mu, controls, x_init, xd0, R0, w0, pts, part_id, Iinv, consts, integrator, Xraw, Xds, Rs, Om, rec, gXs, gXds, gRs, gOm, gFs, gFf):
    B = controls.shape[0]
    return (torch.empty_like(z), torch.empty_like(mu) if mu is not None else z.new_empty(0), torch.empty_like(controls), z.new_empty(B, 3),
            z.new_empty(B, 3), z.new_empty(B, 3, 3), z.new_empty(B, 3))


def _splat_desc(B, n_per_sample, Cc, dx, bx, nx):
    off = (torch.tensor(bx, dtype=torch.float32) - torch.tensor(dx, dtype=torch.float32) / 2.).tolist()
    return _lib.MfSplatDesc(B=B, n_per_sample=n_per_sample, C=Cc, nx=int(nx[0]), ny=int(nx[1]), nz=int(nx[2]),
                            off=(C.c_float * 3)(*off), dx=(C.c_float * 3)(*[float(v) for v in dx]))


@torch.library.impl(_L, 'bev_splat_plan', 'CUDA')
def _splat_plan(geom, dx, bx, nx):
    B = geom.shape[0]
    g = geom.detach().to(torch.float32).contiguous().view(-1, 3)
    d = _splat_desc(B, g.shape[0] // B, 1, dx, bx, nx)
    nbytes = _lib.lib().mf_bev_splat_workspace_bytes(C.byref(d))
    if nbytes == 0:
        raise RuntimeError('mf_bev_splat_workspace_bytes: ' + _lib.lib().mf_last_error().decode())
    ws = torch.empty(nbytes, dtype=torch.uint8, device=geom.device)
    with torch.cuda.device(geom.device), _timing.timed('splat_prepare', geom.device):
        _lib.check(_lib.lib().mf_bev_splat_prepare(C.byref(d), _lib.ptr(g), _lib.ptr(ws), _stream(geom.device)), 'mf_bev_splat_prepare')
    return ws


@torch.library.impl(_L, 'bev_splat_fwd', 'CUDA')
def _splat_fwd(x, plan, B, n_per_sample, dx, bx, nx):
    Cc = x.shape[-1]
    xf = x.contiguous().view(-1, Cc)
    assert xf.shape[0] == B * n_per_sample, 'features and plan disagree on the number of points'
    d = _splat_desc(B, n_per_sample, Cc, dx, bx, nx)
    out = torch.empty(B, d.nz * Cc, d.nx, d.ny, dtype=xf.dtype, device=xf.device)
    with torch.cuda.device(xf.device), _timing.timed('splat_fwd_kernel', xf.device):
        _lib.check(getattr(_lib.lib(), 'mf_bev_splat_fwd_' + _sfx(xf.dtype))(C.byref(d), _lib.ptr(xf), _lib.ptr(plan), _lib.ptr(out), _stream(xf.device)),
                   'mf_bev_splat_fwd')
    return out


@torch.library.impl(_L, 'bev_splat_bwd', 'CUDA')
def _splat_bwd(grad, plan, B, n_per_sample, Cc, dx, bx, nx):
    g = grad.contiguous()
    d = _splat_desc(B, n_per_sample, Cc, dx, bx, nx)
    gx = torch.empty(B * n_per_sample, Cc, dtype=g.dtype, device=g.device)
    with torch.cuda.device(g.device), _timing.timed('splat_bwd_kernel', g.device):
        _lib.check(getattr(_lib.lib(), 'mf_bev_splat_bwd_' + _sfx(g.dtype))(C.byref(d), _lib.ptr(g), _lib.ptr(plan), _lib.ptr(gx), _stream(g.device)),
                   'mf_bev_splat_bwd')
    return gx


def _splat_setup(ctx, inputs, output):
    x, plan, B, n_per_sample, dx, bx, nx = inputs
    ctx.save_for_backward(plan)
    ctx.args = (B, n_per_sample, x.shape[-1], list(dx), list(bx), list(nx))
    ctx.x_shape = x.shape


def _splat_backward(ctx, grad):
    plan, = ctx.saved_tensors
    B, n, Cc, dx, bx, nx = ctx.args
    return torch.ops.monoforce.bev_splat_bwd(grad, plan, B, n, Cc, dx, bx, nx).view(ctx.x_shape), None, None, None, None, None, None


torch.library.register_autograd('monoforce::bev_splat_fwd', _splat_backward, setup_context=_splat_setup, lib=_L)


@torch.library.register_fake('monoforce::bev_splat_fwd', lib=_L)
def _splat_fwd_fake(x, plan, B, n_per_sample, dx, bx, nx):
    return x.new_empty(B, int(nx[2]) * x.shape[-1], int(nx[0]), int(nx[1]))


@torch.library.register_fake('monoforce::bev_splat_bwd', lib=_L)
def _splat_bwd_fake(grad, plan, B, n_per_sample, Cc, dx, bx, nx):
    return grad.new_empty(B * n_per_sample, Cc)


def _mppi_desc(B, T, sigma=(0., 0.), lo=(0., 0.), hi=(0., 0.), weights=(0., 0., 0.), lam=1.0, keep_nominal=False):
    f2 = lambda v: (C.c_float * 2)(float(v[0]), float(v[1]))
    return _lib.MfMppiDesc(B=int(B), T=int(T), keep_nominal=int(bool(keep_nominal)), sigma=f2(sigma), lo=f2(lo), hi=f2(hi),
                           w_incl=float(weights[0]), w_force=float(weights[1]), w_goal=float(weights[2]), lam=float(lam))


def _f32(t, name):
    _lib.require_hip_tensor(t, name)
    if t.dtype != torch.float32:
        raise TypeError(f'monoforce MPPI ops compute in float32, {name} is {t.dtype}')
    return t


@torch.library.impl(_L, 'mppi_perturb', 'CUDA')
def _mppi_perturb(nominal, noise, sigma, lo, hi, keep_nominal):
    nom, nz = _f32(nominal, 'nominal').contiguous(), _f32(noise, 'noise').contiguous()
    assert nz.dim() == 3 and nz.shape[2] == 2 and tuple(nom.shape) == (nz.shape[1], 2), \
        f'noise must be [B,T,2] and nominal [T,2], got {tuple(nz.shape)} and {tuple(nom.shape)}'
    d = _mppi_desc(nz.shape[0], nz.shape[1], sigma=sigma, lo=lo, hi=hi, keep_nominal=keep_nominal)
    controls = torch.empty_like(nz)
    with torch.cuda.device(nz.device), _timing.timed('mppi_perturb_kernel', nz.device):
        _lib.check(_lib.lib().mf_mppi_perturb_f32(C.byref(d), _lib.ptr(nom), _lib.ptr(nz), _lib.ptr(controls), _stream(nz.device)), 'mf_mppi_perturb')
    return controls


@torch.library.impl(_L, 'path_costs', 'CUDA')
def _path_costs(cost_rows, force_cost, x_last, goal, weights):
    rows = _f32(cost_rows, 'cost_rows')
    assert rows.dim() == 3 and rows.shape[2] == 4, f'cost_rows must be [B,T,4], got {tuple(rows.shape)}'
    B, T = rows.shape[:2]
    if rows.stride(2) != 1:
        rows = rows.contiguous()
    xl = _f32(x_last, 'x_last')
    assert xl.dim() == 2 and xl.shape[0] == B and xl.shape[1] >= 2, f'x_last must be [B,>=2], got {tuple(xl.shape)}'
    if xl.stride(1) != 1:
        xl = xl.contiguous()
    g = _f32(goal, 'goal').contiguous()
    assert g.numel() == 2, 'goal must hold (x, y)'
    assert len(weights) == 3, 'weights = (inclination, force, goal)'
    fc = None if force_cost is None else _f32(force_cost, 'force_cost').contiguous()
    assert fc is None or fc.numel() == B, 'force_cost must be [B]'
    d = _mppi_desc(B, T, weights=weights)
    d.row_stride_b, d.row_stride_t, d.x_stride_b = rows.stride(0), rows.stride(1), xl.stride(0)
    costs, terms = torch.empty(B, dtype=torch.float32, device=rows.device), torch.empty(B, 3, dtype=torch.float32, device=rows.device)
    with torch.cuda.device(rows.device), _timing.timed('path_costs_kernel', rows.device):
        _lib.check(_lib.lib().mf_path_costs_f32(C.byref(d), _lib.ptr(rows), _lib.ptr(fc), _lib.ptr(xl), _lib.ptr(g), _lib.ptr(costs), _lib.ptr(terms),
                                                _stream(rows.device)), 'mf_path_costs')
    return costs, terms


def mppi_update_into(costs, controls, nominal, lam, out):
    c, u, nom = _f32(costs, 'costs').contiguous(), _f32(controls, 'controls').contiguous(), _f32(nominal, 'nominal')
    assert u.dim() == 3 and u.shape[2] == 2 and c.shape == (u.shape[0],) and tuple(nom.shape) == (u.shape[1], 2), \
        f'costs [B], controls [B,T,2], nominal [T,2] expected, got {tuple(c.shape)}, {tuple(u.shape)}, {tuple(nom.shape)}'
    assert nom.is_contiguous() and out.is_contiguous() and out.shape == nom.shape and out.dtype == torch.float32 and out.device == u.device
    B, T = u.shape[:2]
    dev = u.device
    d = _mppi_desc(B, T, lam=lam)
    nbytes = int(_lib.lib().mf_mppi_scratch_bytes(C.byref(d)))
    if nbytes < 0:
        raise RuntimeError('mf_mppi_scratch_bytes: ' + _lib.lib().mf_last_error().decode())
    scratch = torch.empty(nbytes // 4, dtype=torch.float32, device=dev)
    weights = torch.empty(B, dtype=torch.float32, device=dev)
    flags = torch.empty(2, dtype=torch.int32, device=dev)
    best, n_valid = flags[:1], flags[1:]
    with torch.cuda.device(dev), _timing.timed('mppi_update_kernel', dev):
        _lib.check(_lib.lib().mf_mppi_update_f32(C.byref(d), _lib.ptr(c), _lib.ptr(u), _lib.ptr(nom), _lib.ptr(weights), _lib.ptr(out), _lib.ptr(best),
                                                 _lib.ptr(n_valid), _lib.ptr(scratch), C.c_longlong(nbytes), _stream(dev)), 'mf_mppi_update')
    return out, weights, best, n_valid


@torch.library.impl(_L, 'mppi_update', 'CUDA')
def _mppi_update(costs, controls, nominal, lam):
    nom = _f32(nominal, 'nominal').contiguous()
    return mppi_update_into(costs, controls, nom, lam, torch.empty_like(nom))


@torch.library.register_fake('monoforce::mppi_perturb', lib=_L)
def _mppi_perturb_fake(nominal, noise, sigma, lo, hi, keep_nominal):
    return noise.new_empty(noise.shape)


@torch.library.register_fake('monoforce::path_costs', lib=_L)
def _path_costs_fake(cost_rows, force_cost, x_last, goal, weights):
    B = cost_rows.shape[0]
    return cost_rows.new_empty(B), cost_rows.new_empty(B, 3)


@torch.library.register_fake('monoforce::mppi_update', lib=_L)
def _mppi_update_fake(costs, controls, nominal, lam):
    B = controls.shape[0]
    return (nominal.new_empty(nominal.shape), costs.new_empty(B), costs.new_empty(1, dtype=torch.int32), costs.new_empty(1, dtype=torch.int32))


def rollout(dphysics, z_grid, controls, state, friction=None):
    cfg = dphysics.dphys_cfg
    dev, dt = z_grid.device, z_grid.dtype
    x0, xd0, R0, w0 = state
    consts = [float(cfg.robot_mass), float(cfg.gravity), float(dphysics.stiffness), float(dphysics.damping), float(cfg.grid_res),
              float(cfg.d_max), float(cfg.dt), float(cfg.omega_max), float(cfg.robot_size[1]), float(dphysics._ts_T)]
    pts = dphysics._points_dev(dev, dt)
    Iinv = torch.tensor(dphysics._iinv(dt), dtype=torch.float64).view(3, 3)
    need = torch.is_grad_enabled() and any(t is not None and t.requires_grad for t in (z_grid, friction, controls, x0, xd0, R0, w0))
    outs = torch.ops.monoforce.dphys_rollout_fwd(z_grid, friction, controls, x0, xd0, R0, w0, pts, dphysics._part_dev(dev), Iinv, consts,
                                                 1 if cfg.use_odeint else 0, need)
    with torch.no_grad():
        x0.data[..., 2] = outs[7][..., 2].to(x0.dtype)
    return tuple(outs[:4]), tuple(outs[4:6])


def splat(geom, x, dx, bx, nx):
    B = geom.shape[0]
    dxl, bxl, nxl = [float(v) for v in dx], [float(v) for v in bx], [int(v) for v in nx]
    plan = torch.ops.monoforce.bev_splat_plan(geom, dxl, bxl, nxl)
    n = geom.numel() // 3 // B
    return torch.ops.monoforce.bev_splat_fwd(x, plan, B, n, dxl, bxl, nxl)
```

Baseline: 1.380 billion rollout-steps/s.

## Track touched-cell bounding box in backward and reduce grad copies only inside it

The streaming backward kernel now records the min/max grid cells its contact points touch, reduced per wavefront and committed with global atomics into a small box buffer. The gradient-copy reduction kernel reads this box and only sums and re-zeros the copies inside it, writing zeros elsewhere. The last block resets the box through a ticket counter. The reduction is also vectorized to 16-byte loads with several copies in flight. The aim is to avoid reading and clearing all 32 copies of the full 256x256 map when rollouts cover only part of it. The cost is extra shuffles and atomics in the backward kernel, plus a correctness dependence on the box tracking being complete.

```diff
diff --git a/include/monoforce_hip.h b/include/monoforce_hip.h
--- a/include/monoforce_hip.h
+++ b/include/monoforce_hip.h
@@ -153,9 +153,11 @@
   const MfRolloutLoss* loss;
   void* zmu_scratch;
   const void* zmu;
+  int32_t* gbox;
 } MfRolloutBwdBufs;
 
 int mf_rollout_bwd_wants_gcontrols(const MfRolloutDesc* desc);
+int mf_rollout_bwd_tracks_box(const MfRolloutDesc* desc);
 int mf_rollout_bwd_f32(const MfRolloutDesc* desc, const MfRolloutBwdBufs* bufs, void* hip_stream);
 int mf_rollout_bwd_f64(const MfRolloutDesc* desc, const MfRolloutBwdBufs* bufs, void* hip_stream);
 
@@ -204,6 +206,8 @@
 int mf_physics_loss_value_f64(const MfLossDesc* desc, const double* Xs, const double* Xgt, const double* gt_ts, const int32_t* nearest, double* partial, uint32_t* ticket, double* loss, double* zero_fill, long long zero_count, void* hip_stream);
 int mf_reduce_grad_copies_f32(float* pool, int n_maps, int copies, long long n, float* out, void* hip_stream);
 int mf_reduce_grad_copies_f64(double* pool, int n_maps, int copies, long long n, double* out, void* hip_stream);
+int mf_reduce_grad_copies_box_f32(float* pool, int n_maps, int copies, int H, int W, int32_t* gbox, float* out, void* hip_stream);
+int mf_reduce_grad_copies_box_f64(double* pool, int n_maps, int copies, int H, int W, int32_t* gbox, double* out, void* hip_stream);
 
 typedef struct MfStageDesc {
   int32_t B, H, W, k;
diff --git a/monoforce_amd/_lib.py b/monoforce_amd/_lib.py
--- a/monoforce_amd/_lib.py
+++ b/monoforce_amd/_lib.py
@@ -36,7 +36,7 @@
                                           'Xraw', 'Xds', 'Rs', 'Omegas',
                                           'gXs', 'gXds', 'gRs', 'gOmegas', 'gFs', 'gFf', 'zeros',
                                           'gz', 'gmu', 'gcontrols', 'gx0', 'gxd0', 'gR0', 'gw0', 'joint_angles', 'gjoint_angles', 'rec', 'loss',
-                                          'zmu_scratch', 'zmu')]
+                                          'zmu_scratch', 'zmu', 'gbox')]
 
 
 class MfLossDesc(C.Structure):
@@ -71,10 +71,10 @@
                 ('w_incl', C.c_float), ('w_force', C.c_float), ('w_goal', C.c_float), ('lam', C.c_float)]
 
 
-SYMBOLS = ['mf_rollout_force_stride', 'mf_rollout_fwd_f32', 'mf_rollout_fwd_f64', 'mf_rollout_default_state_f32', 'mf_rollout_default_state_f64', 'mf_rollout_bwd_f32', 'mf_rollout_bwd_f64', 'mf_rollout_bwd_wants_gcontrols', 'mf_rollout_record_bytes', 'mf_rollout_record_bytes_f64', 'mf_rollout_fwd_stages_zmu', 'mf_rollout_loss_fusable', 'mf_rollout_bwd_window', 'mf_bev_splat_workspace_bytes', 'mf_bev_splat_prepare', 'mf_bev_splat_prepare_cameras', 'mf_bev_splat_prepare_rig',
+SYMBOLS = ['mf_rollout_force_stride', 'mf_rollout_fwd_f32', 'mf_rollout_fwd_f64', 'mf_rollout_default_state_f32', 'mf_rollout_default_state_f64', 'mf_rollout_bwd_f32', 'mf_rollout_bwd_f64', 'mf_rollout_bwd_wants_gcontrols', 'mf_rollout_record_bytes', 'mf_rollout_record_bytes_f64', 'mf_rollout_fwd_stages_zmu', 'mf_rollout_loss_fusable', 'mf_rollout_bwd_window', 'mf_rollout_bwd_tracks_box', 'mf_bev_splat_workspace_bytes', 'mf_bev_splat_prepare', 'mf_bev_splat_prepare_cameras', 'mf_bev_splat_prepare_rig',
            'mf_bev_splat_fwd_f32', 'mf_bev_splat_fwd_f64', 'mf_bev_splat_bwd_f32', 'mf_bev_splat_bwd_f64',
            'mf_bev_lift_splat_fwd_f32', 'mf_bev_lift_splat_fwd_f64', 'mf_bev_lift_splat_bwd_f32', 'mf_bev_lift_splat_bwd_f64',
-           'mf_physics_loss_fwd_f32', 'mf_physics_loss_fwd_f64', 'mf_physics_loss_bwd_f32', 'mf_physics_loss_bwd_f64', 'mf_physics_loss_value_f32', 'mf_physics_loss_value_f64', 'mf_nearest_steps_f32', 'mf_nearest_steps_f64', 'mf_reduce_grad_copies_f32', 'mf_reduce_grad_copies_f64', 'mf_estimate_heightmap_f32', 'mf_interpolate_grid_f32', 'mf_interpolate_grid_f64', 'mf_terrain_stage_fwd_f32', 'mf_terrain_stage_bwd_f32', 'mf_mppi_perturb_f32', 'mf_path_costs_f32', 'mf_mppi_scratch_bytes', 'mf_mppi_update_f32', 'mf_last_error', 'mf_last_launch', 'mf_version', 'mf_sizeof']
+           'mf_physics_loss_fwd_f32', 'mf_physics_loss_fwd_f64', 'mf_physics_loss_bwd_f32', 'mf_physics_loss_bwd_f64', 'mf_physics_loss_value_f32', 'mf_physics_loss_value_f64', 'mf_nearest_steps_f32', 'mf_nearest_steps_f64', 'mf_reduce_grad_copies_f32', 'mf_reduce_grad_copies_f64', 'mf_reduce_grad_copies_box_f32', 'mf_reduce_grad_copies_box_f64', 'mf_estimate_heightmap_f32', 'mf_interpolate_grid_f32', 'mf_interpolate_grid_f64', 'mf_terrain_stage_fwd_f32', 'mf_terrain_stage_bwd_f32', 'mf_mppi_perturb_f32', 'mf_path_costs_f32', 'mf_mppi_scratch_bytes', 'mf_mppi_update_f32', 'mf_last_error', 'mf_last_launch', 'mf_version', 'mf_sizeof']
 
 _lib = None
 _lock = threading.Lock()
diff --git a/monoforce_amd/csrc/physics_loss.hip b/monoforce_amd/csrc/physics_loss.hip
--- a/monoforce_amd/csrc/physics_loss.hip
+++ b/monoforce_amd/csrc/physics_loss.hip
@@ -78,14 +78,63 @@
   }
 }
 
-template <typename S>
-__global__ void __launch_bounds__(256) reduce_grad_copies_kernel(S* __restrict__ pool, int copies, long long n, S* __restrict__ out) {
-  const long long i = (long long)blockIdx.x * blockDim.x + threadIdx.x;
-  if (i >= n) return;
-  S* p = pool + (long long)blockIdx.y * copies * n + i;
-  S acc = (S)0;
-  for (int c = 0; c < copies; ++c) { acc += p[(long long)c * n]; p[(long long)c * n] = (S)0; }
-  out[(long long)blockIdx.y * n + i] = acc;
+constexpr int kBoxEmptyLo = 1 << 30;
+template <typename S, int VEC> struct alignas(sizeof(S) * VEC) CellVec { S v[VEC]; };
+template <typename S, int VEC, bool BOXED>
+__global__ void __launch_bounds__(128) reduce_grad_copies_kernel(S* __restrict__ pool, int copies, int H, int W, long long n, int* gbox, S* __restrict__ out) {
+  using V = CellVec<S, VEC>;
+  constexpr int kFlight = 8;
+  const long long nv = n / VEC;
+  const long long j = (long long)blockIdx.x * blockDim.x + threadIdx.x;
+  bool in = j < nv;
+  if constexpr (BOXED) {
+    const int x0 = max(gbox[0], 0), y0 = max(gbox[1], 0), x1 = min(gbox[2], W - 1), y1 = min(gbox[3], H - 1);
+    const long long e = j * VEC;
+    const int x = (int)(e / H), y = (int)(e - (long long)x * H);
+    in = in && x >= x0 && x <= x1 && y + VEC > y0 && y <= y1;
+  }
+  if (j < nv) {
+    V acc;
+#pragma unroll
+    for (int k = 0; k < VEC; ++k) acc.v[k] = (S)0;
+    if (in) {
+      V* p = reinterpret_cast<V*>(pool + (long long)blockIdx.y * copies * n) + j;
+      V zero;
+#pragma unroll
+      for (int k = 0; k < VEC; ++k) zero.v[k] = (S)0;
+      int c = 0;
+      for (; c + kFlight <= copies; c += kFlight) {
+        V v[kFlight];
+#pragma unroll
+        for (int u = 0; u < kFlight; ++u) v[u] = p[(long long)(c + u) * nv];
+#pragma unroll
+        for (int u = 0; u < kFlight; ++u) {
+#pragma unroll
+          for (int k = 0; k < VEC; ++k) acc.v[k] += v[u].v[k];
+        }
+#pragma unroll
+        for (int u = 0; u < kFlight; ++u) p[(long long)(c + u) * nv] = zero;
+      }
+      for (; c < copies; ++c) {
+        const V v = p[(long long)c * nv];
+#pragma unroll
+        for (int k = 0; k < VEC; ++k) acc.v[k] += v.v[k];
+        p[(long long)c * nv] = zero;
+      }
+    }
+    reinterpret_cast<V*>(out + (long long)blockIdx.y * n)[j] = acc;
+  }
+  if constexpr (BOXED) {
+    __syncthreads();
+    if (threadIdx.x == 0) {
+      __threadfence();
+      unsigned* ticket = reinterpret_cast<unsigned*>(gbox + 4);
+      if (atomicAdd(ticket, 1u) == gridDim.x * gridDim.y - 1u) {
+        gbox[0] = kBoxEmptyLo; gbox[1] = kBoxEmptyLo; gbox[2] = -1; gbox[3] = -1;
+        *ticket = 0u;
+      }
+    }
+  }
 }
 
 template <typename S>
@@ -141,9 +190,30 @@
 static int reduce_copies(S* pool, int n_maps, int copies, long long n, S* out, hipStream_t st) {
   MF_REQUIRE(pool && out, MF_ERR_INVALID, "reduce_grad_copies: null argument");
   MF_REQUIRE(n_maps > 0 && n_maps < 65536 && copies > 0 && n > 0, MF_ERR_INVALID, "reduce_grad_copies: n_maps, copies, n must be positive");
-  hipLaunchKernelGGL((reduce_grad_copies_kernel<S>), dim3((unsigned)((n + 255) / 256), (unsigned)n_maps), dim3(256), 0, st, pool, copies, n, out);
+  constexpr int kVec = 16 / (int)sizeof(S);
+  MF_REQUIRE((n + 127) / 128 < (1ll << 31), MF_ERR_UNSUPPORTED, "reduce_grad_copies: map too large");
+  if (n % kVec == 0 && n < (1ll << 31) && (((uintptr_t)pool | (uintptr_t)out) & 15) == 0)
+    hipLaunchKernelGGL((reduce_grad_copies_kernel<S, kVec, false>), dim3((unsigned)((n / kVec + 127) / 128), (unsigned)n_maps), dim3(128), 0, st, pool, copies, (int)n, 1, n, (int*)nullptr, out);
+  else
+    hipLaunchKernelGGL((reduce_grad_copies_kernel<S, 1, false>), dim3((unsigned)((n + 127) / 128), (unsigned)n_maps), dim3(128), 0, st, pool, copies, 1, 1, n, (int*)nullptr, out);
   hipError_t e = hipGetLastError();
   MF_REQUIRE(e == hipSuccess, MF_ERR_LAUNCH, std::string("reduce_grad_copies launch: ") + hipGetErrorString(e));
+  return MF_OK;
+}
+
+template <typename S>
+static int reduce_copies_box(S* pool, int n_maps, int copies, int H, int W, int32_t* gbox, S* out, hipStream_t st) {
+  MF_REQUIRE(pool && out && gbox, MF_ERR_INVALID, "reduce_grad_copies_box: null argument");
+  MF_REQUIRE(n_maps > 0 && n_maps < 65536 && copies > 0 && H > 0 && W > 0, MF_ERR_INVALID, "reduce_grad_copies_box: n_maps, copies, H, W must be positive");
+  const long long n = (long long)H * W;
+  MF_REQUIRE(n < (1ll << 31), MF_ERR_UNSUPPORTED, "reduce_grad_copies_box: map too large");
+  constexpr int kVec = 16 / (int)sizeof(S);
+  if (H % kVec == 0 && (((uintptr_t)pool | (uintptr_t)out) & 15) == 0)
+    hipLaunchKernelGGL((reduce_grad_copies_kernel<S, kVec, true>), dim3((unsigned)((n / kVec + 127) / 128), (unsigned)n_maps), dim3(128), 0, st, pool, copies, H, W, n, (int*)gbox, out);
+  else
+    hipLaunchKernelGGL((reduce_grad_copies_kernel<S, 1, true>), dim3((unsigned)((n + 127) / 128), (unsigned)n_maps), dim3(128), 0, st, pool, copies, H, W, n, (int*)gbox, out);
+  hipError_t e = hipGetLastError();
+  MF_REQUIRE(e == hipSuccess, MF_ERR_LAUNCH, std::string("reduce_grad_copies_box launch: ") + hipGetErrorString(e));
   return MF_OK;
 }
 
@@ -220,3 +290,5 @@
                                          double* partial, uint32_t* ticket, double* loss, double* zero_fill, long long zero_count, void* s) { return mf::loss_value<double>(d, Xs, Xgt, gt_ts, nearest, partial, ticket, loss, zero_fill, zero_count, (hipStream_t)s); }
 extern "C" int mf_reduce_grad_copies_f32(float* pool, int n_maps, int copies, long long n, float* out, void* s) { return mf::reduce_copies<float>(pool, n_maps, copies, n, out, (hipStream_t)s); }
 extern "C" int mf_reduce_grad_copies_f64(double* pool, int n_maps, int copies, long long n, double* out, void* s) { return mf::reduce_copies<double>(pool, n_maps, copies, n, out, (hipStream_t)s); }
+extern "C" int mf_reduce_grad_copies_box_f32(float* pool, int n_maps, int copies, int H, int W, int32_t* gbox, float* out, void* s) { return mf::reduce_copies_box<float>(pool, n_maps, copies, H, W, gbox, out, (hipStream_t)s); }
+extern "C" int mf_reduce_grad_copies_box_f64(double* pool, int n_maps, int copies, int H, int W, int32_t* gbox, double* out, void* s) { return mf::reduce_copies_box<double>(pool, n_maps, copies, H, W, gbox, out, (hipStream_t)s); }
diff --git a/monoforce_amd/csrc/rollout_bwd.hip b/monoforce_amd/csrc/rollout_bwd.hip
--- a/monoforce_amd/csrc/rollout_bwd.hip
+++ b/monoforce_amd/csrc/rollout_bwd.hip
@@ -132,6 +132,9 @@
   a.gc_sb = 2 * d->T; a.gc_st = 2;
   if (!p->gcontrols) { a.gcontrols = (S*)p->gw0; a.gc_sb = 3; a.gc_st = 0; }
   a.gx0 = (S*)p->gx0; a.gxd0 = (S*)p->gxd0; a.gR0 = (S*)p->gR0; a.gw0 = (S*)p->gw0;
+  a.gbox = p->gbox;
+  MF_REQUIRE(!p->gbox || (d->map_shared && cp_tracks_box(d, (int)sizeof(S)) && p->rec && !p->joint_angles), MF_ERR_UNSUPPORTED,
+             "rollout_bwd: gbox given to a launch that does not track its cells (mf_rollout_bwd_tracks_box; the forward's record required)");
 
   hipStream_t st = (hipStream_t)stream;
   if (p->joint_angles) {
@@ -216,6 +219,7 @@
   return mf::cp_loss_fusable(d) ? 1 : (mf::xs_loss_fusable(d) ? 2 : (mf::cp_loss_one_wave(d, 4) ? 3 : 0));
 }
 extern "C" int mf_rollout_bwd_window(const MfRolloutDesc* d) { return mf::xs_bwd_window(d) ? 1 : 0; }
+extern "C" int mf_rollout_bwd_tracks_box(const MfRolloutDesc* d) { return d && d->map_shared && mf::cp_tracks_box(d, 4) ? 1 : 0; }
 extern "C" int mf_rollout_bwd_f32(const MfRolloutDesc* d, const MfRolloutBwdBufs* p, void* s) {
   return mf::rollout_bwd<float>(d, p, s);
 }
diff --git a/monoforce_amd/csrc/rollout_bwd_cp_fast.hip b/monoforce_amd/csrc/rollout_bwd_cp_fast.hip
--- a/monoforce_amd/csrc/rollout_bwd_cp_fast.hip
+++ b/monoforce_amd/csrc/rollout_bwd_cp_fast.hip
@@ -44,6 +44,16 @@
   const long long grid = ((long long)d->B * 16 + 63) / 64;
   return grid <= (long long)cp_stream_max_grid(d->integrator);
 }
+bool cp_tracks_box(const MfRolloutDesc* d, int scalar_bytes) {
+  static const bool one_wave = getenv("MF_CP_BWD_MODE") && atoi(getenv("MF_CP_BWD_MODE")) == kCpSaved;
+  if (!d || one_wave || d->has_joints) return false;
+  if (scalar_bytes != 4 && d->points_per_lane != MF_LANES_COMPONENT) return false;
+  if (d->integrator != MF_INTEG_ODEINT_EULER && d->integrator != MF_INTEG_DYNAMICS) return false;
+  if (cp_record_bytes(d, scalar_bytes) <= 0) return false;
+  const long long grid = ((long long)d->B * 16 + 63) / 64;
+  if (scalar_bytes == 8 && d->integrator != MF_INTEG_ODEINT_EULER) return false;
+  return grid <= (long long)cp_stream_max_grid(d->integrator);
+}
 bool cp_bwd_wants_zmu(const MfRolloutDesc* d, bool has_rec, bool has_mu) {
   static const bool off = getenv("MF_CP_BWD_ZMU") && atoi(getenv("MF_CP_BWD_ZMU")) == 0;
   static const int forced = getenv("MF_CP_BWD_MODE") ? atoi(getenv("MF_CP_BWD_MODE")) : -1;
diff --git a/monoforce_amd/csrc/rollout_bwd_cp_kernel.h b/monoforce_amd/csrc/rollout_bwd_cp_kernel.h
--- a/monoforce_amd/csrc/rollout_bwd_cp_kernel.h
+++ b/monoforce_amd/csrc/rollout_bwd_cp_kernel.h
@@ -438,6 +438,7 @@
   if constexpr (SAVED) {
     typedef S f4v __attribute__((ext_vector_type(4)));
     struct Saved { f4v q; S zc, mc; int idx; };
+    int cell_u = 0;
     const char* const prec = reinterpret_cast<const char*>(a.rec) + (size_t)tid * kRecBytesPerLane<S>;
     const unsigned rec_step = (unsigned)a.B * 16u * kRecBytesPerLane<S>;
     auto load_saved = [&](int m, Saved& v) {
@@ -446,6 +447,7 @@
     auto gather_cells = [&](Saved& v) {
       const S lim = S(262144.0);
       const int ui = (int)M::clamp(v.q.x, -lim, lim);
+      cell_u = ui;
       const int base = dppi<kB1>(ui) + __mul24(a.H, dppi<kB0>(ui));
       v.idx = min(max(base + cell_off, 0), last);
 #ifdef MF_STREAM_NO_GATHER
@@ -611,11 +613,13 @@
         }
       };
       __shared__ S snap_c[4 * 64];
+      int snap_cell_idx = -1;
       auto snap_prepare = [&]() {
         if (!a.skip_snap) {
           S wq, dx, dy;
           int idx;
           snap_cell(idx, wq, dx, dy);
+          snap_cell_idx = idx;
           snap_c[lane] = idx_as(zero, idx); snap_c[64 + lane] = wq; snap_c[128 + lane] = dx; snap_c[192 + lane] = dy;
         }
         asm volatile("" ::: "memory");
@@ -737,8 +741,31 @@
           for (int i = 0; i < BATCH; ++i) fetch(s[i]);
           skip3();
         };
+        constexpr int kBoxFar = 1 << 30;
+        int bu_lo = kBoxFar, bu_hi = -kBoxFar;
+        auto box_commit = [&]() {
+          if (a.gbox == nullptr) return;
+          int x0 = dppi<kB0>(bu_lo) + (q & 1), x1 = dppi<kB0>(bu_hi) + (q & 1), y0 = dppi<kB1>(bu_lo) + (q >> 1), y1 = dppi<kB1>(bu_hi) + (q >> 1);
+          if (snap_cell_idx >= 0) {
+            const int sx = snap_cell_idx / a.H, sy = snap_cell_idx - sx * a.H;
+            x0 = min(x0, sx); x1 = max(x1, sx); y0 = min(y0, sy); y1 = max(y1, sy);
+          }
+          const int n_live = min(64, (a.B - (int)blockIdx.x * 4) * 16);
+#pragma unroll
+          for (int d = 32; d >= 1; d >>= 1) {
+            const int ox0 = __shfl_xor(x0, d, 64), ox1 = __shfl_xor(x1, d, 64), oy0 = __shfl_xor(y0, d, 64), oy1 = __shfl_xor(y1, d, 64);
+            const bool live = (lane ^ d) < n_live;
+            x0 = live ? min(x0, ox0) : x0; x1 = live ? max(x1, ox1) : x1; y0 = live ? min(y0, oy0) : y0; y1 = live ? max(y1, oy1) : y1;
+          }
+          if (lane == 0 && x0 <= x1) {
+            const bool off_map = (x0 < 0) | (y0 < 0) | (x1 > a.W - 1) | (y1 > a.H - 1);
+            atomicMin(a.gbox + 0, off_map ? 0 : x0); atomicMin(a.gbox + 1, off_map ? 0 : y0);
+            atomicMax(a.gbox + 2, off_map ? a.W - 1 : x1); atomicMax(a.gbox + 3, off_map ? a.H - 1 : y1);
+          }
+        };
         auto gather1 = [&](Slot& r) {
           gather_cells(r.sv);
+          bu_lo = min(bu_lo, cell_u); bu_hi = max(bu_hi, cell_u);
           r.lg = loss_gt_lane[(size_t)(unsigned)min(max(r.sj, 0), l_T2m1) * 3u];
         };
         auto gather3 = [&](Slot (&s)[BATCH]) {
@@ -787,6 +814,7 @@
         MF_PROF_OUT(0 + 4 * fk, acc_room); MF_PROF_OUT(1 + 4 * fk, acc_pub);
         loss_share(l_acc);
         if (fk == 0) {
+          box_commit();
           MF_PROF_T(t_lf);
           loss_value_finish();
           MF_PROF_DRAIN();
@@ -797,6 +825,7 @@
 #endif
         } else {
           snap_prepare();
+          box_commit();
         }
         return;
       }
@@ -1149,6 +1178,7 @@
 
 bool use_component_parallel_bwd(const MfRolloutDesc* d, const MfRolloutBwdBufs* p, int scalar_bytes = 4);
 long long cp_record_bytes(const MfRolloutDesc* d, int scalar_bytes);
+bool cp_tracks_box(const MfRolloutDesc* d, int scalar_bytes);
 bool cp_loss_fusable(const MfRolloutDesc* d);
 bool cp_bwd_wants_zmu(const MfRolloutDesc* d, bool has_rec, bool has_mu);
 int launch_rollout_bwd_cp_f32(const RolloutBwdArgs<float>& a, int integ, bool xs_only, hipStream_t st);
@@ -1185,6 +1215,7 @@
   static const int forced = getenv("MF_CP_BWD_MODE") ? atoi(getenv("MF_CP_BWD_MODE")) : -1;
   const int saved_mode = grid <= cp_stream_max_grid_of<S>(INTEG) && forced != kCpSaved ? kCpStream : kCpSaved;
   const int mode = a.rec ? saved_mode : (forced >= 0 && forced < kCpSaved ? forced : ((long long)grid <= device_simds() ? kCpLate : kCpEarly));
+  MF_REQUIRE(a.gbox == nullptr || mode == kCpStream, MF_ERR_UNSUPPORTED, "rollout_bwd: only the streaming form tracks the box of touched cells (gbox)");
 #define MF_BCP(XS_, GC_, M_) MF_KLAUNCH((rollout_bwd_cp_kernel<S, INTEG, XS_, GC_, M_>), dim3(wgs), dim3(block), 0, st, a)
   constexpr bool kZmu = std::is_same<S, float>::value && INTEG == MF_INTEG_ODEINT_EULER;
 #define MF_BCP_Z(XS_, GC_) do { if constexpr (kZmu) { if (a.zmu) { MF_KLAUNCH((rollout_bwd_cp_kernel<S, INTEG, XS_, GC_, kCpSaved, 6, 3, kZmu>), dim3(wgs), dim3(block), 0, st, a); break; } } MF_BCP(XS_, GC_, kCpSaved); } while (0)
diff --git a/monoforce_amd/csrc/rollout_bwd_kernel.h b/monoforce_amd/csrc/rollout_bwd_kernel.h
--- a/monoforce_amd/csrc/rollout_bwd_kernel.h
+++ b/monoforce_amd/csrc/rollout_bwd_kernel.h
@@ -32,6 +32,7 @@
   const int* loss_near;
   const S* loss_w;
   int gc_sb, gc_st;
+  int* gbox;
 };
 
 #ifdef MF_NO_ATOMICS
diff --git a/monoforce_amd/dphysics_bwd.py b/monoforce_amd/dphysics_bwd.py
--- a/monoforce_amd/dphysics_bwd.py
+++ b/monoforce_amd/dphysics_bwd.py
@@ -8,6 +8,13 @@
 
 GRAD_COPIES = int(os.environ.get('MF_GRAD_COPIES', '32'))
 WIN_GRAD_COPIES = int(os.environ.get('MF_GRAD_COPIES_WIN', '64'))
+GRAD_BOX = os.environ.get('MF_GRAD_BOX', '1') != '0'
+BOX_EMPTY = (1 << 30, 1 << 30, -1, -1, 0, 0, 0, 0)
+
+
+def tracks_box(desc, dt, rec):
+    return bool(GRAD_BOX and desc.map_shared and dt == torch.float32 and rec is not None and rec.numel()
+                and _lib.lib().mf_rollout_bwd_tracks_box(C.byref(desc)))
 
 
 def grad_copies_for(B, N):
@@ -20,6 +27,8 @@
     def __init__(self, n_maps, copies, n, dt, dev):
         self.n_maps, self.copies, self.n = n_maps, copies, n
         self.buf = torch.zeros(n_maps * copies * n + 16, dtype=dt, device=dev)
+        self.box_empty = torch.tensor(BOX_EMPTY, dtype=torch.int32, device=dev)
+        self.box = self.box_empty.clone()
         self.busy = False
         self.stream = None
         self.pinned = False
@@ -34,16 +43,23 @@
             if self.done is not None and not capturing:
                 cur_s.wait_event(self.done)
             self.buf.zero_()
+            self.box.copy_(self.box_empty)
         self.busy, self.stream = True, cur
 
-    def reduce(self, map_shape):
+    def reduce(self, map_shape, boxed=False):
         from .dphysics import _scalar_suffix
         flat = torch.empty(self.n_maps * self.n + 1, dtype=self.buf.dtype, device=self.buf.device)
         out = flat[:-1].view((self.n_maps,) + tuple(map_shape))
-        fn = getattr(_lib.lib(), 'mf_reduce_grad_copies_' + _scalar_suffix(self.buf.dtype))
+        sfx = _scalar_suffix(self.buf.dtype)
         with torch.cuda.device(self.buf.device):
-            _lib.check(fn(_lib.ptr(self.buf), self.n_maps, self.copies, C.c_longlong(self.n), _lib.ptr(out),
-                          C.c_void_p(self.stream)), 'mf_reduce_grad_copies')
+            if boxed:
+                fn = getattr(_lib.lib(), 'mf_reduce_grad_copies_box_' + sfx)
+                _lib.check(fn(_lib.ptr(self.buf), self.n_maps, self.copies, int(map_shape[-2]), int(map_shape[-1]), _lib.ptr(self.box),
+                              _lib.ptr(out), C.c_void_p(self.stream)), 'mf_reduce_grad_copies_box')
+            else:
+                fn = getattr(_lib.lib(), 'mf_reduce_grad_copies_' + sfx)
+                _lib.check(fn(_lib.ptr(self.buf), self.n_maps, self.copies, C.c_longlong(self.n), _lib.ptr(out),
+                              C.c_void_p(self.stream)), 'mf_reduce_grad_copies')
         if not torch.cuda.is_current_stream_capturing():
             if self.done is None:
                 self.done = torch.cuda.Event()
@@ -101,7 +117,7 @@
         maps = pool.buf[:n_maps * copies * z.numel()].view((n_maps, copies) + tuple(z.shape))
         gz, gmu, zero_row = maps[0], (maps[1] if want_gmu else None), pool.buf[-16:]
     else:
-        maps = None
+        maps = pool = None
         gz = torch.zeros_like(z)
         gmu = torch.zeros_like(mu) if want_gmu else None
         zero_row = torch.zeros(16, dtype=dt, device=dev)
@@ -111,7 +127,9 @@
     gx0 = torch.empty_like(xd0) if ctx.needs_input_grad[4] else None
     ja = getattr(ctx, 'joint_angles', None)
     gja = torch.zeros_like(ja) if ja is not None and ctx.needs_input_grad[10] else None
+    boxed = pool is not None and tracks_box(desc, dt, getattr(ctx, 'rec', None))
     bufs = _lib.MfRolloutBwdBufs(
+        gbox=_lib.ptr(pool.box) if boxed else None,
         z=_lib.ptr(z), mu=_lib.ptr(mu), controls=_lib.ptr(controls), ts=_lib.ptr(ts), points=_lib.ptr(keep['points']),
         part=_lib.ptr(mod._part_dev(dev)), x_init=_lib.ptr(x_init), xd0=_lib.ptr(xd0), R0=_lib.ptr(R0), w0=_lib.ptr(w0),
         Xraw=_lib.ptr(Xraw), Xds=_lib.ptr(Xds), Rs=_lib.ptr(Rs), Omegas=_lib.ptr(Om),
@@ -135,7 +153,7 @@
     _timing.note_launch('rollout_bwd_kernel')
 
     if desc.map_shared:
-        summed = pool.reduce(z.shape)
+        summed = pool.reduce(z.shape, boxed)
         gz, gmu = summed[0], (summed[1] if want_gmu else None)
 
     def to_input_shape(g, shape, expanded):
diff --git a/monoforce_amd/ops.py b/monoforce_amd/ops.py
--- a/monoforce_amd/ops.py
+++ b/monoforce_amd/ops.py
@@ -3,7 +3,7 @@
 import torch
 
 from . import _lib, _timing
-from .dphysics_bwd import grad_copies_for, grad_pool
+from .dphysics_bwd import grad_copies_for, grad_pool, tracks_box
 
 
 class _PoolOwner:
@@ -147,10 +147,13 @@
         gXs=_lib.ptr(ups[0]), gXds=_lib.ptr(ups[1]), gRs=_lib.ptr(ups[2]), gOmegas=_lib.ptr(ups[3]), gFs=_lib.ptr(ups[4]), gFf=_lib.ptr(ups[5]),
         zeros=_lib.ptr(zero_row), gz=_lib.ptr(gz), gmu=_lib.ptr(gmu), gcontrols=_lib.ptr(gcontrols), gx0=_lib.ptr(gx0), gxd0=_lib.ptr(gxd0),
         gR0=_lib.ptr(gR0), gw0=_lib.ptr(gw0), rec=_lib.ptr(rec) if rec.numel() else None)
+    boxed = bool(d.map_shared) and tracks_box(d, dt, rec)
+    if boxed:
+        bufs.gbox = _lib.ptr(pool.box)
     with torch.cuda.device(dev), _timing.timed('rollout_bwd_kernel', dev):
         _lib.check(getattr(_lib.lib(), 'mf_rollout_bwd_' + _sfx(dt))(C.byref(d), C.byref(bufs), _stream(dev)), 'mf_rollout_bwd')
     if d.map_shared:
-        summed = pool.reduce(zc.shape[1:])
+        summed = pool.reduce(zc.shape[1:], boxed)
         gz = summed[0].unsqueeze(0)
         gmu = summed[1].unsqueeze(0) if muc is not None else None
     if gz.shape[0] != z.shape[0]:
```

Measured after the change: 1.333 billion rollout-steps/s. 3.4% lower.
